# Rose-STL-Lab/dyffusion

Measured on AMD Instinct MI355X. Metric: sampled fields/sec (h-step rollout), higher is better.
Workload: dtype bf16; 1 GPU; BASELINE configs[1]: Navier-Stokes 221x42, C=3+2 static ch, unet_simple dim 64 @256^2, DYffusion h=16 cold sampling + refine, interpolator MC dropout p=0.15, hipGraph rollout; rows_per_gpu=80, total_rows=80, net_forwards_per_rollout=60, parallelism=ensemble-sharded dp1

## Files before the change

### dyffusion_amd/_lib.py

```python
import ctypes as C
import os

_HERE = os.path.dirname(os.path.abspath(__file__))
LIB_PATH = os.environ.get("DYF_LIB") or os.path.join(_HERE, "lib", "libdyffusion_hip.so")
LIB_PATH_F16 = os.environ.get("DYF_LIB_F16") or os.path.join(_HERE, "lib", "libdyffusion_hip_f16.so")
DTYPES = {"bf16": 0, "bfloat16": 0, "fp16": 1, "float16": 1, "half": 1}
FP32_NAMES = ("fp32", "float32", "32")
BF16X3_NAMES = ("bf16x3", "48")


def canonical_dtype(dtype) -> str:
    key = str(dtype).lower()
    if key in FP32_NAMES:
        return "fp32"
    if key in BF16X3_NAMES:
        return "bf16x3"
    if key not in DTYPES:
        raise ValueError(f"dtype {dtype!r}: expected one of {sorted(DTYPES) + list(FP32_NAMES) + list(BF16X3_NAMES)}")
    return "fp16" if DTYPES[key] else "bf16"


def storage_dtype(dtype) -> str:
    d = canonical_dtype(dtype)
    return "bf16" if d in ("fp32", "bf16x3") else d
# ... 16 lines not shown
DYF_TRAIN_PRECISION_BF16X3 = 48
DYF_SAMPLE_PRECISION_BF16X3 = 48
DYF_OK, DYF_ERR_INVALID_ARGUMENT, DYF_ERR_UNSUPPORTED, DYF_ERR_HIP, DYF_ERR_STATE = range(5)
NET_FORECASTER, NET_INTERPOLATOR = 0, 1
ARCH_UNET_SIMPLE, ARCH_UNET_RESNET = 0, 1
ARCH_SIMPLE_CONV_NET = 2
FCOND = {"none": 0, "data": 1, "data+noise": 2}


class NetConfig(C.Structure):
    _fields_ = [("arch", C.c_int32), ("in_channels", C.c_int32), ("cond_channels", C.c_int32),
                ("out_channels", C.c_int32), ("dim", C.c_int32), ("with_time_emb", C.c_int32),
                ("upsample_h", C.c_int32), ("upsample_w", C.c_int32), ("dropout", C.c_float),
                ("input_dropout", C.c_float), ("n_mults", C.c_int32), ("dim_mults", C.c_int32 * 6),
                ("block_dropout1", C.c_float), ("attn_dropout", C.c_float), ("groups", C.c_int32),
                ("init_kernel_size", C.c_int32), ("init_padding", C.c_int32), ("outer_nearest", C.c_int32),
                ("keep_spatial_dims", C.c_int32), ("single_conv_layer", C.c_int32), ("learned_sinusoidal_dim", C.c_int32)]


class EngineConfig(C.Structure):
    _fields_ = [("abi_version", C.c_int32), ("device", C.c_int32), ("height", C.c_int32), ("width", C.c_int32),
                ("max_batch", C.c_int32), ("use_graph", C.c_int32), ("enable_mfma", C.c_int32), ("dtype", C.c_int32),
                ("batch_invariant", C.c_int32), ("net", NetConfig * 2)]


class PlanStep(C.Structure):
    _fields_ = [("forecaster_time", C.c_float), ("tau", C.c_float), ("i_next", C.c_float), ("i_cur", C.c_float),
                ("is_last", C.c_int32), ("out_slot", C.c_int32)]


class Plan(C.Structure):
    _fields_ = [("n_steps", C.c_int32), ("steps", C.POINTER(PlanStep)), ("sampling_cold", C.c_int32),
                ("cold_for_last_step", C.c_int32), ("forward_conditioning", C.c_int32), ("n_refine", C.c_int32),
                ("refine_times", C.POINTER(C.c_float)), ("refine_slots", C.POINTER(C.c_int32)),
                ("n_out_slots", C.c_int32), ("interpolator_dropout", C.c_int32), ("forecaster_dropout", C.c_int32)]


class BcArgs(C.Structure):
    _fields_ = [("kind", C.c_int32), ("n_fields", C.c_int32), ("rows", C.c_int32), ("channels", C.c_int32),
                ("height", C.c_int32), ("width", C.c_int32), ("n_meta", C.c_int32), ("row_meta_dev", C.c_void_p),
                ("time_factor_dev", C.c_void_p), ("times_per_meta", C.c_int32), ("fixed_mask_dev", C.c_void_p),
                ("in_velocity_dev", C.c_void_p), ("vertex_y_dev", C.c_void_p), ("boundary_dev", C.c_void_p)]


class ConvEx(C.Structure):
    _fields_ = [("x1_dev", C.c_void_p), ("residual_dev", C.c_void_p), ("y_f32_dev", C.c_void_p), ("mask_dev", C.c_void_p),
                ("c1", C.c_int32), ("coef_div", C.c_int32), ("n_sel", C.c_int32), ("drop_mode", C.c_int32),
                ("drop_p", C.c_float), ("drop_site", C.c_int32), ("drop_row_offset", C.c_uint32), ("drop_forward", C.c_uint32)]


BC_NAVIER_STOKES, BC_SPRING_MESH = 0, 1
COMM_ID_BYTES = 128
TRAIN_BATCH_STATS, TRAIN_DROPOUT = 1, 2


class TrainOp(C.Structure):
    _fields_ = [(k, C.c_int32) for k in ("op", "nb", "h", "w", "c", "c2", "k", "stride", "pad", "groups", "flags")] + [("p", C.c_float)]


TRAIN_OPS = {"conv": 0, "gn_act": 1, "layernorm": 2, "linattn": 3, "attention": 4, "linear": 5, "learned_sinu": 6, "dropout": 7,
             "gelu": 8, "add": 9, "cat": 10, "up2_nearest": 11, "norm_act": 12, "up2_bilinear": 13, "resize": 14, "convt": 15,
             "attention_stream": 16}
TOP_WS, TOP_BIAS, TOP_PRE, TOP_FILM, TOP_SAME = 1, 2, 4, 8, 16
TOP_RUNNING, TOP_MASK, TOP_LEAKY, TOP_RELU, TOP_NEAREST, TOP_GRAD_IN = 32, 64, 128, 256, 512, 1024
TOP_ACT_GELU, TOP_RESIDUAL = 2048, 4096
TOP_SAMPLE = 8192


class SampleOp(C.Structure):
    _fields_ = [(k, C.c_int32) for k in ("op", "nb", "h", "w", "c", "c2", "k", "pad", "groups", "act", "flags", "film_stride", "film_div",
                                         "part_slots", "nsrc")] + [("ch", C.c_int32 * 4), ("drop_mode", C.c_int32), ("drop_p", C.c_float),
                                                                   ("drop_site", C.c_int32), ("drop_row_offset", C.c_uint32), ("drop_forward", C.c_uint32)] + \
               [(k, C.c_int32) for k in ("oh", "ow", "nearest", "src_rows", "iw_store")] + [("tau", C.c_float)]


class SampleTensors(C.Structure):
    _fields_ = [("x", C.c_void_p * 4), ("residual", C.c_void_p), ("film_a", C.c_void_p), ("film_c", C.c_void_p), ("part", C.c_void_p),
                ("mask", C.c_void_p), ("y", C.c_void_p), ("col_map", C.c_void_p), ("y2", C.c_void_p), ("y3", C.c_void_p)]


SAMPLE_OPS = {"gn_act": 0, "layernorm_c": 1, "head": 2, "up2_nearest": 3, "drop16": 4, "stem_conv": 5, "groupnorm_f32": 6, "up2_bilinear": 7,
              "up2_epilogue": 8, "readout": 9, "readout_tables": 10, "stem": 11, "stem16": 12, "rng_begin": 13, "rng_clone": 14, "time_mlp": 15,
              "film": 16, "cold_update": 17, "noisy_condition": 18}
SOP_NO_STATS, SOP_NO_TABLES, SOP_FOLD_RNG, SOP_COUNTERS_ONLY = 1, 2, 4, 8
RNG_STATE_WORDS = 8
ACTS = {"none": 0, "relu": 1, "leaky": 2, "silu": 3, "gelu": 4}


class OptimConfig(C.Structure):
    _fields_ = [("beta1", C.c_double), ("beta2", C.c_double), ("eps", C.c_double), ("weight_decay", C.c_double),
                ("max_grad_norm", C.c_double), ("ema", C.c_int32)]


OPTIM_WEIGHT, OPTIM_GRAD, OPTIM_EXP_AVG, OPTIM_EXP_AVG_SQ, OPTIM_EMA, OPTIM_WEIGHT_FWD = range(6)

_P = C.c_void_p
SYMBOLS = [
    ("dyf_engine_create", C.c_int, [C.POINTER(EngineConfig), C.POINTER(_P)]),
    ("dyf_engine_destroy", None, [_P]),
    ("dyf_last_error", C.c_char_p, [_P]),
    ("dyf_abi_version", C.c_int32, []),
    ("dyf_dtype", C.c_int32, []),
    ("dyf_load_weights", C.c_int, [_P, C.c_int32, C.c_int32, C.POINTER(C.c_char_p), C.POINTER(_P), C.POINTER(_P),
                                   C.POINTER(C.c_int32)]),
    ("dyf_train_load_weights", C.c_int, [_P, C.c_int32, C.c_int32, C.POINTER(C.c_char_p), C.POINTER(_P), C.POINTER(_P),
                                         C.POINTER(C.c_int32)]),
    ("dyf_train_load_weights_dev", C.c_int, [_P, C.c_int32, C.c_int32, C.POINTER(C.c_char_p), C.POINTER(_P), C.POINTER(_P),
                                             C.POINTER(C.c_int32)]),
    ("dyf_train_export_dev", C.c_int, [_P, C.c_int32, C.c_int32, C.POINTER(C.c_char_p), C.POINTER(_P)]),
    ("dyf_net_forward", C.c_int, [_P, C.c_int32, _P, _P, _P, _P, C.c_int32, C.c_int32, C.POINTER(_P), _P]),
    ("dyf_set_plan", C.c_int, [_P, C.POINTER(Plan)]),
    ("dyf_sample", C.c_int, [_P, _P, _P, _P, C.c_int32, C.POINTER(_P), _P, _P]),
    ("dyf_seed", C.c_int, [_P, C.c_uint64]),
    ("dyf_set_row_offset", C.c_int, [_P, C.c_uint32]),
    ("dyf_set_log_intermediates", C.c_int, [_P, C.c_int32]),
    ("dyf_get_log", C.c_int, [_P, C.c_int32, C.c_int32, _P, C.c_int32, _P]),
    ("dyf_set_row_groups", C.c_int, [_P, C.c_int32]),
    ("dyf_row_groups", C.c_int32, [_P]),
    ("dyf_comm_unique_id", C.c_int, [_P]),
    ("dyf_comm_init", C.c_int, [_P, _P, C.c_int32, C.c_int32]),
    ("dyf_comm_destroy", C.c_int, [_P]),
    ("dyf_comm_count", C.c_int, [_P, _P]),
    ("dyf_sample_gather", C.c_int, [_P, _P, _P, _P, C.c_int32, C.c_int32, _P]),
    ("dyf_get_sampler_state", C.c_int, [_P, C.c_int32, _P, C.c_int32, _P]),
    ("dyf_plan_forward_counts", C.c_int, [_P, C.POINTER(C.c_int32), C.POINTER(C.c_int32)]),
    ("dyf_net_flops", C.c_int, [_P, C.c_int32, C.POINTER(C.c_double)]),
    ("dyf_net_flops_executed", C.c_int, [_P, C.c_int32, C.POINTER(C.c_double)]),
    ("dyf_time_conv_layer", C.c_int, [_P, C.c_int32, C.c_int32, C.c_int32, C.c_int32, _P, C.POINTER(C.c_double),
                                      C.POINTER(C.c_double), C.POINTER(C.c_double)]),
    ("dyf_ensemble_metrics", C.c_int, [_P, _P, _P, C.c_int32, C.c_int64, C.POINTER(C.c_double), _P]),
    ("dyf_time_layer_in_rollout", C.c_int, [_P, C.c_int32, C.c_int32, _P, C.POINTER(C.c_double), C.POINTER(C.c_int32)]),
    ("dyf_time_kernel_in_rollout", C.c_int, [_P, C.c_int32, C.c_int32, _P, C.POINTER(C.c_double), C.POINTER(C.c_int32),
                                             C.POINTER(C.c_double), C.POINTER(C.c_double)]),
    ("dyf_op_conv2d", C.c_int, [_P, _P, _P] + [C.c_int32] * 9 + [_P, _P, C.c_int32, C.c_int32, _P, _P]),
    ("dyf_op_conv2d_ex", C.c_int, [_P, _P, _P] + [C.c_int32] * 9 + [_P, _P, C.c_int32, C.c_int32, _P, C.POINTER(ConvEx), _P]),
    ("dyf_op_upconv2d", C.c_int, [_P, _P, _P] + [C.c_int32] * 5 + [_P, _P, C.c_int32, _P, _P]),
    ("dyf_op_linear_attention", C.c_int, [_P, _P, C.c_int32, C.c_int32, _P, _P]),
    ("dyf_op_linear_attention_fused", C.c_int, [_P, _P, _P, C.c_int32, C.c_int32, C.c_int32, _P, _P, _P, _P, _P]),
    ("dyf_op_attention", C.c_int, [_P, _P, C.c_int32, C.c_int32, _P, _P]),
    ("dyf_op_attention_dropout", C.c_int, [_P, _P, C.c_int32, C.c_int32, C.c_float, _P, _P]),
    ("dyf_op_attention_f32", C.c_int, [_P, _P, C.c_int32, C.c_int32, C.c_float, _P, C.c_int32, _P, _P]),
    ("dyf_op_train_f32", C.c_int, [_P, C.POINTER(TrainOp), C.POINTER(_P), C.POINTER(_P), _P, _P, C.POINTER(_P), C.POINTER(_P), _P]),
    ("dyf_op_sample16", C.c_int, [_P, C.POINTER(SampleOp), C.POINTER(SampleTensors), C.POINTER(_P), _P]),
    ("dyf_criterion", C.c_int, [_P, _P, _P, C.c_int64, C.c_int32, _P, _P]),
    ("dyf_train_forward", C.c_int, [_P, C.c_int32, C.c_int32, _P, _P, _P, _P, C.c_int32, C.c_int32, _P]),
    ("dyf_train_backward", C.c_int, [_P, C.c_int32, _P, _P, C.c_int32, _P]),
    ("dyf_train_zero_grads", C.c_int, [_P, C.c_int32]),
    ("dyf_train_set_precision", C.c_int, [_P, C.c_int32]),
    ("dyf_train_precision", C.c_int32, [_P]),
    ("dyf_train_set_deterministic", C.c_int, [_P, C.c_int32]),
    ("dyf_train_deterministic", C.c_int32, [_P]),
    ("dyf_set_sample_precision", C.c_int, [_P, C.c_int32]),
    ("dyf_sample_precision", C.c_int32, [_P]),
    ("dyf_set_attention_dropout", C.c_int, [_P, C.c_int32]),
    ("dyf_attention_dropout", C.c_int32, [_P]),
    ("dyf_train_export", C.c_int, [_P, C.c_int32, C.c_int32, C.POINTER(C.c_char_p), C.POINTER(_P)]),
    ("dyf_optim_create", C.c_int, [_P, C.c_int32, C.POINTER(OptimConfig)]),
    ("dyf_optim_destroy", C.c_int, [_P, C.c_int32]),
    ("dyf_optim_step", C.c_int, [_P, C.c_int32, C.c_double, C.c_double, _P]),
    ("dyf_optim_last", C.c_int, [_P, C.c_int32, C.POINTER(C.c_double), C.POINTER(C.c_int32)]),
    ("dyf_optim_get_step", C.c_int, [_P, C.c_int32, C.POINTER(C.c_int64)]),
    ("dyf_optim_set_step", C.c_int, [_P, C.c_int32, C.c_int64]),
    ("dyf_optim_export", C.c_int, [_P, C.c_int32, C.c_int32, C.c_int32, C.POINTER(C.c_char_p), C.POINTER(_P), C.c_int32]),
    ("dyf_optim_import", C.c_int, [_P, C.c_int32, C.c_int32, C.c_int32, C.POINTER(C.c_char_p), C.POINTER(_P), C.c_int32]),
    ("dyf_optim_swap_ema", C.c_int, [_P, C.c_int32, _P]),
    ("dyf_criterion_grad", C.c_int, [_P, _P, _P, C.c_int64, C.c_int32, C.c_float, _P, _P]),
    ("dyf_train_conv_check", C.c_int, [_P] + [C.c_int32] * 9 + [C.c_uint32, C.POINTER(C.c_float)]),
# ... 61 lines not shown
```

### dyffusion_amd/csrc/conv.h

```cpp
#pragma once
#include "common.h"
#include "gn_fused.h"

#include <string>
#include <vector>

void dyf_form_log_enable(bool on);
std::string dyf_form_log_text();
void dyf_form_set(const char* key, const char* value);
std::string dyf_form_text();
void dyf_prof_arm(const char* name);
void dyf_prof_collect(double* total_ms, double* total_bytes, int* launches);

struct ConvArgs {
    const el16_t* src0;
    const el16_t* src1;
    int c0, c1;
    int pix_pitch0;
    int n, h, w;
    int ho, wo;
    int kh, kw, stride, pad;
    int cout;
    const el16_t* wpk;
    const el16_t* wpk_frag;
    int up2x;
    const el16_t* wpk_up;
    const el16_t* wpk_up_frag;
    const int16_t* up_cols;
    const int16_t* up_cbase;
    const int16_t* up_cidx;
    int up_ntiles, up_npad, up_nvalid0, up_nvalid1;
    int up_mix[3];
    int up_sh_off, up_sh_cb;
    int up_wo_store;
    const float* coef_a;
    const float* coef_c;
    int coef_stride;
    int coef_div;
    int act;
    DropSpec drop;
    int up_nearest;
    const el16_t* residual;
    el16_t* out_el16;
    float* out_f32;
    const el16_t* zero_page;
    float* up_border;
    float* splitk_ws;
    long long splitk_cap;
    int splitk;
    int n_sel;
    float* gn_part;
    int gn_slots;
    GnFuse gnf;
};
inline size_t conv_up_border_floats(int n, int h, int w, int cout) { return (size_t)n * (4 * (size_t)w + 4 * (size_t)h - 4) * cout; }

enum class HaloOrder { None, Halo3_256 , Halo3_64 , S2 ,
                       Enc0Stem  };
struct ConvW {
    const el16_t* wpk = nullptr;
    const el16_t* frag = nullptr;
    const el16_t* halo = nullptr;
    HaloOrder halo_order = HaloOrder::None;
    const el16_t* frag64 = nullptr;
};

hipError_t conv_init();
bool conv_mfma_supported(const ConvArgs& a);
enum class ConvForm { Invalid , None , Direct, Igemm128, Igemm256x64, UpHalo,
                      Halo3, Rows3, Halo5, HaloS2, Enc0Stem, Igemm2, Skinny, Gn16 };
enum class ConvWant { Plain, Stats , GnFused };
struct ConvChoice {
    ConvForm form;
    const el16_t* frag;
    int gn_slots;
    int bm;
};
ConvChoice conv_choose_form(const ConvArgs& a, const ConvW& w, int path, ConvWant want);
hipError_t launch_conv(const ConvArgs& a, const ConvW& w, int path, hipStream_t stream);
hipError_t launch_conv_stats(const ConvArgs& a, const ConvW& w, int path, hipStream_t stream, int* gn_slots);
hipError_t launch_conv_gn_fused(const ConvArgs& a, const ConvW& w, int path, hipStream_t stream, bool* fused);
int conv_gn_fused_max_slots(int h, int w);
bool conv_plain3x3_takes_halo5(const ConvArgs& a, const ConvW& w);

hipError_t launch_conv_direct(const ConvArgs& a, hipStream_t stream);
hipError_t launch_conv_igemm(const ConvArgs& a, hipStream_t stream);
void pack_up2x_weights(const float* w, int cout, int cin, el16_t* out);
hipError_t launch_conv_splitk_finish4(const ConvArgs& a, long long M, hipStream_t stream);
bool conv_up_halo_supported(const ConvArgs& a);
hipError_t conv_up_halo_init();
hipError_t launch_conv_up_halo(const ConvArgs& a, hipStream_t stream);
void pack_up2x_frag(const el16_t* wpk_up, int cout, int cin, el16_t* out);
bool plan_up_sparse_columns(const std::vector<uint8_t>& needed, int w, std::vector<int16_t>& cols, std::vector<int16_t>& cbase,
                            std::vector<int16_t>& cidx, std::vector<int16_t>& col_map, int& ntiles, int& nvalid0, int& nvalid1,
                            int slots = 16);
int conv_halo_rows_slots();
int conv_halo_rows_sparse_halo_w();
int conv_halo_rows_sparse_halo_w_shape(int shape);
bool plan_up_sparse_columns_mixed(const std::vector<uint8_t>& needed, int w, int h, std::vector<int16_t>& cols, std::vector<int16_t>& cbase,
                                  std::vector<int16_t>& cidx, std::vector<int16_t>& col_map, int mix[3], int& nvalid0, int& nvalid1);
bool conv_halo_rows_up_supported(const ConvArgs& a);
bool conv_halo_rows3_supported(const ConvArgs& a);
hipError_t conv_halo_rows_init();
hipError_t launch_conv_halo_rows_up(const ConvArgs& a, hipStream_t stream);
hipError_t launch_conv_halo_rows3(const ConvArgs& a, hipStream_t stream);
bool conv_halo3_supported(const ConvArgs& a);
hipError_t launch_conv_halo3(const ConvArgs& a, hipStream_t stream);
void pack_halo3_frag(const el16_t* wpk, int cout, int cin, el16_t* out);
bool conv_halo_s2_supported(const ConvArgs& a);
hipError_t launch_conv_halo_s2(const ConvArgs& a, hipStream_t stream);
void pack_halo_s2_frag(const el16_t* wpk, int cout, int cin, el16_t* out);
bool conv_halo5_supported(const ConvArgs& a);
int conv_halo5_gn_slots(int h, int w);
hipError_t launch_conv_halo5(const ConvArgs& a, hipStream_t stream);
void pack_halo3_frag64(const el16_t* wpk, int cout, int cin, el16_t* out);
bool conv_gn16_supported(const ConvArgs& a);
int conv_gn16_slots(int h, int w);
hipError_t launch_conv_gn16(const ConvArgs& a, hipStream_t stream);
bool conv_enc0_stem_supported(const ConvArgs& a);
hipError_t conv_enc0_stem_init();
hipError_t launch_conv_enc0_stem(const ConvArgs& a, const el16_t* wfrag, hipStream_t stream);
void pack_enc0_stem_frag(const el16_t* wpk, int cout, el16_t* out);
bool conv_igemm2_supported(const ConvArgs& a);
hipError_t conv_igemm2_init();
hipError_t launch_conv_igemm2(const ConvArgs& a, hipStream_t stream);
void pack_conv_frag(const el16_t* wpk, int cout, int taps, int cin, el16_t* out);
bool conv_igemm2_tile2d(int ho, int wo);
int conv_igemm2_gn_slots(int ho, int wo);
int conv_igemm2_gn_slots_bm128(int ho, int wo);
bool conv_skinny_supported(const ConvArgs& a);
hipError_t launch_conv_skinny(const ConvArgs& a, hipStream_t stream);
```

### dyffusion_amd/csrc/conv_dispatch.hip

```cpp
#include "conv.h"

#include <algorithm>
#include <initializer_list>

namespace {

long long form_rows(const ConvArgs& a) { return a.n_sel > 0 ? a.n_sel : a.n; }
ConvArgs with_up_frag(ConvArgs a, const el16_t* f) { a.wpk_up_frag = f; return a; }
ConvArgs with_frag(ConvArgs a, const ConvW& w) { a.wpk_frag = w.frag; return a; }
const el16_t* halo_of(const ConvW& w, HaloOrder order) { return w.halo_order == order ? w.halo : nullptr; }
bool halo3_on() { return dyf_form_int("DYF_HALO3", 1) != 0; }
bool igemm2_on() { return dyf_form_int("DYF_IGEMM2", 1) != 0; }

bool up_halo_admits(const ConvArgs& a) {
    const int halo_min = dyf_form_int("DYF_HALO_MIN_PLANE", 32);
    return a.up2x && dyf_form_int("DYF_UP_HALO", 1) != 0 && a.h >= halo_min && a.w >= halo_min && conv_up_halo_supported(a);
}

const el16_t* halo3_admits(const ConvArgs& a, const ConvW& w) {
    if (!(!a.up2x && a.kh == 3 && a.kw == 3 && a.cout % 256 == 0 && a.out_f32 == nullptr && a.residual == nullptr) || !halo3_on()) return nullptr;
    const ConvArgs b = with_up_frag(a, halo_of(w, HaloOrder::Halo3_256));
    const long long tiles3 = (form_rows(a) * a.h * a.w / 128) * (a.cout / 256);
    return b.wpk_up_frag && tiles3 >= dyf_form_int("DYF_HALO3_MIN_TILES", 80) && conv_halo3_supported(b) ? b.wpk_up_frag : nullptr;
}

const el16_t* halo5_admits(const ConvArgs& a, const ConvW& w) {
    if (!(!a.up2x && a.kh == 3 && a.kw == 3 && a.stride == 1 && a.cout % 64 == 0 && a.cout % 256 != 0 && a.out_f32 == nullptr)) return nullptr;
    if (dyf_form_int("DYF_HALO5", 1) == 0) return nullptr;
    const ConvArgs b = with_up_frag(a, halo_of(w, HaloOrder::Halo3_64));
    const long long ty = (a.h + 15) / 16, tx = (a.w + 31) / 32;
    const long long tiles5 = form_rows(a) * ty * tx * (a.cout / 64);
    const bool covers = 10ll * a.h * a.w >= 6ll * ty * 16 * tx * 32;
    return b.wpk_up_frag && covers && tiles5 >= dyf_form_int("DYF_HALO5_MIN_TILES", 64) && conv_halo5_supported(b) ? b.wpk_up_frag : nullptr;
}

const el16_t* enc0_stem_admits(const ConvArgs& a, const ConvW& w) {
    return a.pix_pitch0 == 16 && conv_enc0_stem_supported(a) ? halo_of(w, HaloOrder::Enc0Stem) : nullptr;
}

const el16_t* halo_s2_admits(const ConvArgs& a, const ConvW& w) {
    if (!(!a.up2x && a.kh == 4 && a.kw == 4 && a.stride == 2 && a.cout % 128 == 0 && a.c1 == 0 && a.out_f32 == nullptr &&
          a.residual == nullptr && a.pix_pitch0 == 0) || !halo3_on())
        return nullptr;
    const ConvArgs b = with_up_frag(a, halo_of(w, HaloOrder::S2));
    const long long min_tiles3 = dyf_form_int("DYF_HALO_S2_MIN_TILES", dyf_form_int("DYF_HALO3_MIN_TILES", 80));
    const long long pix = form_rows(a) * a.ho * a.wo;
    const long long tiles3 = a.cout % 256 == 0 ? (pix / 128) * (a.cout / 256) : (pix / 256) * (a.cout / 128);
    return b.wpk_up_frag && tiles3 >= min_tiles3 && conv_halo_s2_supported(b) ? b.wpk_up_frag : nullptr;
}

long long igemm2_tiles(const ConvArgs& a) {
    return ((form_rows(a) * a.ho * a.wo + 255) / 256) * (a.cout % 128 == 0 ? a.cout / 128 : a.cout / 64);
}

const el16_t* igemm2_admits(const ConvArgs& a, const ConvW& w) {
    if (!(!a.up2x && igemm2_on() && a.cout % 64 == 0)) return nullptr;
    const ConvArgs b = with_frag(a, w);
    return igemm2_tiles(a) >= dyf_form_int("DYF_IGEMM2_MIN_TILES", 384) && conv_igemm2_supported(b) ? b.wpk_frag : nullptr;
}

const el16_t* skinny_admits(const ConvArgs& a, const ConvW& w) {
    if (!(!a.up2x && a.cout % 128 == 0) || dyf_form_int("DYF_SKINNY", 1) == 0) return nullptr;
    const long long tiles128 = ((form_rows(a) * a.ho * a.wo + 127) / 128) * (a.cout / 128);
    const ConvArgs b = with_frag(a, w);
    return tiles128 <= dyf_form_int("DYF_SKINNY_MAX_TILES", 64) && conv_skinny_supported(b) ? b.wpk_frag : nullptr;
}

const int GN_FUSE_MAX_SLOTS = 64;
bool gn_slots_fit(int slots, int max_slots) { return slots <= GN_FUSE_MAX_SLOTS && slots <= max_slots; }

const el16_t* gn16_admits(const ConvArgs& a, const ConvW& w, bool c256) {
    if (dyf_form_int("DYF_GN16", 1) == 0 || (c256 && dyf_form_int("DYF_GN16_C256", 1) == 0)) return nullptr;
    const ConvArgs b = with_up_frag(a, c256 ? w.frag64 : halo_of(w, HaloOrder::Halo3_64));
    const int slots16 = conv_gn16_slots(a.h, a.w);
    const long long tiles16 = form_rows(a) * slots16 * (a.cout / 64);
    const bool covers16 = 10ll * a.h * a.w >= 6ll * slots16 * 256 || dyf_form_int("DYF_GN16_ANY_PLANE", 0) != 0;
    const bool plane_ok = !c256 || (long long)a.h * a.w <= dyf_form_int("DYF_GN16_C256_MAX_PLANE", 1024);
    return b.wpk_up_frag && covers16 && plane_ok && tiles16 >= dyf_form_int("DYF_GN16_MIN_TILES", 64) &&
                   gn_slots_fit(slots16, a.gnf.max_slots) && conv_gn16_supported(b) ? b.wpk_up_frag : nullptr;
}

const el16_t* igemm2_fused_admits(const ConvArgs& a, const ConvW& w, ConvChoice* c) {
    const GnFuse& G = a.gnf;
    if (!(igemm2_on() && a.cout % 128 == 0)) return nullptr;
    const ConvArgs b = with_frag(a, w);
    if (!conv_igemm2_supported(b)) return nullptr;
    const long long tiles2 = igemm2_tiles(a);
    const long long min_tiles = dyf_form_int("DYF_IGEMM2_MIN_TILES", dyf_form_int("DYF_GN_FUSE_MIN_TILES", 32));
    const bool position_free = conv_igemm2_tile2d(a.ho, a.wo) || (a.ho * a.wo) % 128 == 0;
    if (G.invariant && !position_free) return nullptr;
    const long long bm128_below = dyf_form_int("DYF_IGEMM2_BM128_BELOW", 224);
    const int slots128 = conv_igemm2_gn_slots_bm128(a.ho, a.wo), slots = conv_igemm2_gn_slots(a.ho, a.wo);
    const bool free128 = (a.wo % 16 == 0 && a.ho % 8 == 0) || (a.ho * a.wo) % 64 == 0;
    if (tiles2 >= min_tiles && tiles2 < bm128_below && slots128 > 0 && gn_slots_fit(slots128, G.max_slots) && (!G.invariant || free128))
        c->gn_slots = slots128, c->bm = 128;
    else if (tiles2 >= min_tiles && slots > 0 && gn_slots_fit(slots, G.max_slots))
        c->gn_slots = slots, c->bm = 256;
    else
        return nullptr;
    return b.wpk_frag;
}

ConvChoice choose_plain(const ConvArgs& a, const ConvW& w, bool mfma, bool stats) {
    const ConvChoice invalid{ConvForm::Invalid, nullptr, 0, 0};
    const el16_t* const h5 = mfma && a.residual == nullptr ? halo5_admits(a, w) : nullptr;
    if (a.up_nearest && !(h5 && a.h % 2 == 0 && a.w % 2 == 0 && a.c1 == 0)) return invalid;
    if (!mfma) return a.up2x ? invalid : ConvChoice{ConvForm::Direct, nullptr, 0, 0};
    if (a.up2x && a.up_cols) return conv_up_halo_supported(a) ? ConvChoice{ConvForm::UpHalo, nullptr, 0, 0} : invalid;
    if (up_halo_admits(a)) return {ConvForm::UpHalo, nullptr, 0, 0};
    if (const el16_t* f = halo3_admits(a, w))
        return {dyf_form_int("DYF_HALO_ROWS", 1) != 0 && conv_halo_rows3_supported(a) ? ConvForm::Rows3 : ConvForm::Halo3, f, 0, 0};
    if (h5)
        return {ConvForm::Halo5, h5, stats && a.act == ACT_NONE && a.drop.mode == 0 ? conv_halo5_gn_slots(a.h, a.w) : 0, 0};
    if (const el16_t* f = enc0_stem_admits(a, w)) return {ConvForm::Enc0Stem, f, 0, 0};
    if (const el16_t* f = halo_s2_admits(a, w)) return {ConvForm::HaloS2, f, 0, 0};
    if (const el16_t* f = igemm2_admits(a, w)) return {ConvForm::Igemm2, f, 0, 0};
    if (const el16_t* f = skinny_admits(a, w)) return {ConvForm::Skinny, f, 0, 0};
    return {a.cout % 128 == 0 ? ConvForm::Igemm128 : ConvForm::Igemm256x64, nullptr, 0, 0};
}

ConvChoice choose_gn_fused(const ConvArgs& a, const ConvW& w, bool mfma) {
    ConvChoice c{ConvForm::None, nullptr, 0, 0};
    const GnFuse& G = a.gnf;
    if (!mfma || G.gran == nullptr || G.epoch == nullptr || a.act != ACT_SILU || a.drop.mode == 2 || a.out_el16 == nullptr ||
        a.out_f32 != nullptr || a.up2x)
        return c;
    const int cpg = G.groups > 0 ? a.cout / G.groups : 0;
    if (cpg < 8 || cpg % 8 != 0 || 64 % cpg != 0 || cpg * G.groups != a.cout) return c;
    const bool conv3 = a.kh == 3 && a.kw == 3 && a.stride == 1 && a.pad == 1;
    if (conv3 && a.cout % 64 == 0) {
        if (const el16_t* f = gn16_admits(a, w, a.cout % 256 == 0)) return {ConvForm::Gn16, f, conv_gn16_slots(a.h, a.w), 0};
        const int slots = conv_halo5_gn_slots(a.h, a.w);
        if (const el16_t* f = gn_slots_fit(slots, G.max_slots) ? halo5_admits(a, w) : nullptr) return {ConvForm::Halo5, f, slots, 0};
    }
    if ((c.frag = igemm2_fused_admits(a, w, &c))) c.form = ConvForm::Igemm2;
    return c;
}

hipError_t launch_chosen(ConvArgs& a, const ConvChoice& c, hipStream_t stream) {
    switch (c.form) {
    case ConvForm::Invalid: return hipErrorInvalidValue;
    case ConvForm::None: return hipSuccess;
    case ConvForm::Direct: return launch_conv_direct(a, stream);
    case ConvForm::Igemm128:
    case ConvForm::Igemm256x64: return launch_conv_igemm(a, stream);
    case ConvForm::UpHalo: return launch_conv_up_halo(a, stream);
    case ConvForm::Halo3: a.wpk_up_frag = c.frag; return launch_conv_halo3(a, stream);
    case ConvForm::Rows3: a.wpk_up_frag = c.frag; return launch_conv_halo_rows3(a, stream);
    case ConvForm::Halo5: a.wpk_up_frag = c.frag; return launch_conv_halo5(a, stream);
    case ConvForm::HaloS2: a.wpk_up_frag = c.frag; return launch_conv_halo_s2(a, stream);
    case ConvForm::Gn16: a.wpk_up_frag = c.frag; return launch_conv_gn16(a, stream);
    case ConvForm::Enc0Stem: return launch_conv_enc0_stem(a, c.frag, stream);
    case ConvForm::Igemm2: a.wpk_frag = c.frag; return launch_conv_igemm2(a, stream);
    case ConvForm::Skinny: a.wpk_frag = c.frag; return launch_conv_skinny(a, stream);
    }
    return hipErrorInvalidValue;
}

}

ConvChoice conv_choose_form(const ConvArgs& a, const ConvW& w, int path, ConvWant want) {
    const bool mfma = path == 1 && conv_mfma_supported(a);
    return want == ConvWant::GnFused ? choose_gn_fused(a, w, mfma) : choose_plain(a, w, mfma, want == ConvWant::Stats);
}

bool conv_plain3x3_takes_halo5(const ConvArgs& a, const ConvW& w) {
    return a.gn_part == nullptr && a.gnf.gran == nullptr && conv_choose_form(a, w, 1, ConvWant::Plain).form == ConvForm::Halo5;
}

int conv_gn_fused_max_slots(int h, int w) {
    int best = 0;
    for (int s : {conv_halo5_gn_slots(h, w), conv_gn16_slots(h, w), conv_igemm2_gn_slots(h, w), conv_igemm2_gn_slots_bm128(h, w)})
        if (gn_slots_fit(s, GN_FUSE_MAX_SLOTS)) best = std::max(best, s);
    return best;
}

hipError_t launch_conv(const ConvArgs& a, const ConvW& w, int path, hipStream_t stream) {
    return launch_conv_stats(a, w, path, stream, nullptr);
}

hipError_t launch_conv_stats(const ConvArgs& a_in, const ConvW& w, int path, hipStream_t stream, int* gn_slots) {
    if (gn_slots) *gn_slots = 0;
    ConvArgs a = a_in;
    a.wpk = w.wpk;
    a.gn_part = nullptr;
    a.gn_slots = 0;
    const bool stats = gn_slots != nullptr && a_in.gn_part != nullptr;
    const ConvChoice c = conv_choose_form(a, w, path, stats ? ConvWant::Stats : ConvWant::Plain);
    if (c.gn_slots > 0) {
        a.gn_part = a_in.gn_part;
        a.gn_slots = c.gn_slots;
        *gn_slots = c.gn_slots;
    }
    return launch_chosen(a, c, stream);
}

hipError_t launch_conv_gn_fused(const ConvArgs& a_in, const ConvW& w, int path, hipStream_t stream, bool* fused) {
    ConvArgs a = a_in;
    a.wpk = w.wpk;
    a.gn_part = nullptr;
    a.gn_slots = 0;
    const ConvChoice c = conv_choose_form(a, w, path, ConvWant::GnFused);
    *fused = c.form != ConvForm::None;
    a.gnf.slots = c.gn_slots;
    if (c.bm) a.gnf.bm = c.bm;
    return launch_chosen(a, c, stream);
}
```

### dyffusion_amd/csrc/conv_enc0_stem.hip

```cpp
#include "conv.h"

#include <type_traits>
typedef __attribute__((ext_vector_type(16))) float f32x16;

namespace {
constexpr int E0_KSTEPS = 16;
constexpr int E0_WAVES = 8, E0_THREADS = E0_WAVES * 64;
constexpr int e0_lds_bytes(int nt) { return E0_KSTEPS * nt * 1024 + E0_WAVES * 2 * nt * 32 * 4 + E0_WAVES * 32 * (nt * 64 + 16); }
}

template <int NT>
__global__ __launch_bounds__(512) void conv_enc0_stem_kernel(ConvArgs a, const el16_t* __restrict__ wfrag, int tiles, int tiles_per_wg) {
#if defined(__gfx950__)
    extern __shared__ __attribute__((aligned(16))) unsigned char e0_smem[];
    uint4* wl = (uint4*)e0_smem;
    const int tid = threadIdx.x, lane = tid & 63, wave = __builtin_amdgcn_readfirstlane(tid >> 6), l31 = lane & 31, hi = lane >> 5;
    for (int i = tid; i < E0_KSTEPS * NT * 64; i += E0_THREADS) wl[i] = ((const uint4*)wfrag)[i];
    __syncthreads();
    float* coefl = (float*)(e0_smem + E0_KSTEPS * NT * 1024) + wave * (2 * NT * 32);
    int coef_row = -1;
    constexpr int OROW = NT * 64 + 16;
    unsigned char* ostage = e0_smem + E0_KSTEPS * NT * 1024 + E0_WAVES * 2 * NT * 32 * 4 + wave * (32 * OROW);
    const int segs = a.wo >> 5;
    const int plane = a.ho * a.wo;
    const int t0 = blockIdx.x * tiles_per_wg, t1 = min(t0 + tiles_per_wg, tiles);
    const int cout = NT * 32;

    auto load = [&](int t, uint4 (&xf)[E0_KSTEPS]) {
        const int row = t / segs, seg = t - row * segs;
        const int n = row / a.ho, oy = row - n * a.ho;
        const el16_t* p = a.src0 + ((size_t)(n * a.h + 2 * oy) * a.w + 2 * (seg * 32 + l31)) * 16 + 8 * hi;
#pragma unroll
        for (int kh = 0; kh < 4; ++kh)
#pragma unroll
            for (int kw = 0; kw < 4; ++kw) xf[kh * 4 + kw] = *(const uint4*)(p + ((size_t)kh * a.w + kw) * 16);
        __builtin_amdgcn_sched_barrier(0);
    };

    auto tile = [&](int t, const uint4 (&xf)[E0_KSTEPS], auto act_c, auto mode_c) {
        constexpr int ACT = decltype(act_c)::value, MODE = decltype(mode_c)::value;
        f32x16 acc[NT];
#pragma unroll
        for (int nt = 0; nt < NT; ++nt)
#pragma unroll
            for (int r = 0; r < 16; ++r) acc[nt][r] = 0.0f;
#pragma unroll
        for (int s = 0; s < E0_KSTEPS; ++s) {
            int wlane = lane;
            asm volatile("" : "+v"(wlane));
            const el16x8_t xb = __builtin_bit_cast(el16x8_t, xf[s]);
#pragma unroll
            for (int nt = 0; nt < NT; ++nt)
                acc[nt] = DYF_MFMA_32x32x16(__builtin_bit_cast(el16x8_t, wl[(s * NT + nt) * 64 + wlane]), xb, acc[nt], 0, 0, 0);
        }
        const int m = t * 32 + l31;
        const int n_img = m / plane;
        const uint32_t ob = (uint32_t)m * (uint32_t)cout;
        const RngKey key = drop_row_key(a.drop, n_img);
        const uint32_t row0 = (uint32_t)n_img * (uint32_t)(plane * cout);
        const int crow = __builtin_amdgcn_readfirstlane(a.coef_div > 1 ? n_img / a.coef_div : n_img);
        if (crow != coef_row) {
            coef_row = crow;
            const float ps = drop_prescale<ACT, MODE>(a.drop);
            if (lane < NT * 8) {
                float4 ca = *(const float4*)(a.coef_a + (size_t)crow * a.coef_stride + lane * 4);
                float4 cc = *(const float4*)(a.coef_c + (size_t)crow * a.coef_stride + lane * 4);
                ca.x *= ps; ca.y *= ps; ca.z *= ps; ca.w *= ps;
                cc.x *= ps; cc.y *= ps; cc.z *= ps; cc.w *= ps;
                *(float4*)(coefl + lane * 4) = ca;
                *(float4*)(coefl + NT * 32 + lane * 4) = cc;
            }
        }
#pragma unroll
        for (int nt = 0; nt < NT; ++nt) {
            uint4 o2[2];
#pragma unroll
            for (int g2 = 0; g2 < 2; ++g2) {
                const int cg0 = nt * 32 + 16 * g2;
                const float4 ca0 = *(const float4*)(coefl + cg0 + 4 * hi), ca1 = *(const float4*)(coefl + cg0 + 4 * hi + 8);
                const float4 cc0 = *(const float4*)(coefl + NT * 32 + cg0 + 4 * hi), cc1 = *(const float4*)(coefl + NT * 32 + cg0 + 4 * hi + 8);
                const float ca[8] = {ca0.x, ca0.y, ca0.z, ca0.w, ca1.x, ca1.y, ca1.z, ca1.w};
                const float cc[8] = {cc0.x, cc0.y, cc0.z, cc0.w, cc1.x, cc1.y, cc1.z, cc1.w};
                const uint32_t e0 = ob + cg0 + 4 * hi;
                float v[8];
#pragma unroll
                for (int i = 0; i < 8; ++i) v[i] = fmaf(acc[nt][8 * g2 + i], ca[i], cc[i]);
                act_drop_fixed<4, ACT, MODE, true>(v, e0, row0, a.drop, key);
                act_drop_fixed<4, ACT, MODE, true>(v + 4, e0 + 8, row0, a.drop, key);
                const uint32_t p0 = pack_el16x2(v[0], v[1]), p1 = pack_el16x2(v[2], v[3]);
                const uint32_t q0 = pack_el16x2(v[4], v[5]), q1 = pack_el16x2(v[6], v[7]);
                const auto s0 = __builtin_amdgcn_permlane32_swap(p0, q0, false, false);
                const auto s1 = __builtin_amdgcn_permlane32_swap(p1, q1, false, false);
                o2[g2].x = s0[0]; o2[g2].y = s1[0]; o2[g2].z = s0[1]; o2[g2].w = s1[1];
            }
            *(uint4*)(ostage + l31 * OROW + (nt * 32 + 8 * hi) * 2) = o2[0];
            *(uint4*)(ostage + l31 * OROW + (nt * 32 + 16 + 8 * hi) * 2) = o2[1];
        }
        el16_t* tbase = a.out_el16 + (size_t)t * 32 * cout;
#pragma unroll
        for (int k = 0; k < NT * 2; ++k) {
            const int off = k * 1024 + lane * 16;
            const int px = off / (NT * 64), within = off - px * (NT * 64);
            const uint4 ov = *(const uint4*)(ostage + px * OROW + within);
            *(uint4*)((unsigned char*)tbase + off) = ov;
        }
    };

    auto run = [&](auto act_c, auto mode_c) {
        uint4 xa[E0_KSTEPS], xb[E0_KSTEPS];
        int t = t0 + wave;
        if (t >= t1) return;
        load(t, xa);
        for (; t < t1; t += 2 * E0_WAVES) {
            load(t + E0_WAVES, xb);
            tile(t, xa, act_c, mode_c);
            load(t + 2 * E0_WAVES < t1 ? t + 2 * E0_WAVES : t, xa);
            tile(t + E0_WAVES, xb, act_c, mode_c);
        }
    };
    auto by_mode = [&](auto act_c) {
        if (a.drop.mode == 0) run(act_c, std::integral_constant<int, 0>{});
        else if (a.drop.mode == 1) run(act_c, std::integral_constant<int, 1>{});
        else run(act_c, std::integral_constant<int, 2>{});
    };
    if (a.act == ACT_RELU) by_mode(std::integral_constant<int, ACT_RELU>{});
    else if (a.act == ACT_LEAKY) by_mode(std::integral_constant<int, ACT_LEAKY>{});
    else if (a.act == ACT_SILU) by_mode(std::integral_constant<int, ACT_SILU>{});
    else by_mode(std::integral_constant<int, ACT_NONE>{});
#endif
}

void pack_enc0_stem_frag(const el16_t* wpk, int cout, el16_t* out) {
    const int nt_n = cout / 32;
    for (int s = 0; s < E0_KSTEPS; ++s)
        for (int nt = 0; nt < nt_n; ++nt)
            for (int lane = 0; lane < 64; ++lane)
                for (int j = 0; j < 8; ++j)
                    out[(((size_t)s * nt_n + nt) * 64 + lane) * 8 + j] = wpk[(size_t)(32 * nt + (lane & 31)) * 256 + 16 * s + 8 * (lane >> 5) + j];
}

bool conv_enc0_stem_supported(const ConvArgs& a) {
    const bool on = dyf_form_int("DYF_ENC0_STEM", 1) != 0;
    if (!on || a.pix_pitch0 != 16 || a.c0 != 64 || a.c1 != 0 || a.kh != 4 || a.kw != 1 || a.stride != 2 || a.pad != 0) return false;
    if (a.up2x || a.residual || a.out_f32 || !a.out_el16 || (a.cout != 64 && a.cout != 128)) return false;
    if (a.wo % 32 != 0 || (a.ho * (a.wo / 32)) % 16 != 0 || a.h != 2 * a.ho + 2 || a.w != 2 * a.wo + 2) return false;
    const long long nsel = a.n_sel > 0 ? a.n_sel : a.n;
    if (nsel * a.ho * (a.wo / 32) < 4096) return false;
    return (size_t)a.n * a.ho * a.wo * a.cout < 0xFFFFFFF0ull;
}

hipError_t conv_enc0_stem_init() {
    hipError_t e = hipFuncSetAttribute((const void*)conv_enc0_stem_kernel<4>, hipFuncAttributeMaxDynamicSharedMemorySize, e0_lds_bytes(4));
    if (e == hipSuccess) e = hipFuncSetAttribute((const void*)conv_enc0_stem_kernel<2>, hipFuncAttributeMaxDynamicSharedMemorySize, e0_lds_bytes(2));
    return e;
}

hipError_t launch_conv_enc0_stem(const ConvArgs& a, const el16_t* wfrag, hipStream_t stream) {
    const int tiles = a.n * a.ho * (a.wo / 32);
    int nwg = std::min(256, (tiles + 15) / 16);
    int per = (tiles + nwg - 1) / nwg;
    per = (per + 15) / 16 * 16;
    nwg = (tiles + per - 1) / per;
    dyf_form_note("conv_enc0_stem_kernel", a.n);
    if (a.cout == 128)
        hipLaunchKernelGGL(conv_enc0_stem_kernel<4>, dim3(nwg), dim3(E0_THREADS), e0_lds_bytes(4), stream, a, wfrag, tiles, per);
    else
        hipLaunchKernelGGL(conv_enc0_stem_kernel<2>, dim3(nwg), dim3(E0_THREADS), e0_lds_bytes(2), stream, a, wfrag, tiles, per);
    return hipGetLastError();
}
```

### dyffusion_amd/csrc/engine.hip

```cpp
#include "engine_internal.h"

#include <dlfcn.h>
#include <mutex>
#include <rccl/rccl.h>
#include "unet_kernels.h"
#include "../../include/dyffusion_hip_testing.h"

using namespace dyf;

namespace {

thread_local bool g_creating_group_child = false;

int default_row_groups(const dyf_engine* e) {
    if (e->cfg.net[0].arch != DYF_ARCH_UNET_RESNET || e->cfg.net[1].arch != DYF_ARCH_UNET_RESNET) return 1;
    if (e->cfg.batch_invariant) return 1;
    const long long plane = (long long)e->cfg.height * e->cfg.width;
    if (plane > 128 * 128) return 1;
    const long long pix = plane * e->cfg.max_batch;
    if (pix >= 72ll * 60 * 60) return 3;
    return 1;
}

void layout_blocks(Net& n) {
// ... 5 lines not shown
    int off = 0;
    for (int i = 0; i < 12; ++i) {
        const int* s = i < 6 ? enc[i] : dec[i - 6];
        UBlock& b = n.blk[i];
        b.cin = s[0]; b.cout = s[1]; b.k = s[2]; b.stride = s[3]; b.pad = s[4];
        b.gn = (i == 5);
        b.transposed = i >= 6;
        b.act = i < 6 ? ACT_LEAKY : ACT_RELU;
        b.film_off = off;
        off += b.cout;
    }
    n.total_c = off;
}

std::string layout_geometry(Net& n, int H, int W) {
    n.uh = n.cfg.upsample_h > 0 ? n.cfg.upsample_h : H;
    n.uw = n.cfg.upsample_w > 0 ? n.cfg.upsample_w : W;
    int h = n.uh, w = n.uw;
    for (int i = 0; i < 6; ++i) {
        UBlock& b = n.blk[i];
        b.in_h = h; b.in_w = w;
        b.out_h = (h + 2 * b.pad - b.k) / b.stride + 1;
        b.out_w = (w + 2 * b.pad - b.k) / b.stride + 1;
        if (b.out_h < 1 || b.out_w < 1) return "resampled grid too small for six stride-2 encoder blocks";
        h = b.out_h; w = b.out_w;
    }
    for (int i = 6; i < 12; ++i) {
        UBlock& b = n.blk[i];
        b.in_h = 2 * h; b.in_w = 2 * w;
        b.out_h = b.in_h + 2 * b.pad - b.k + 1;
        b.out_w = b.in_w + 2 * b.pad - b.k + 1;
        h = b.out_h; w = b.out_w;
        if (i < 11) {
            const UBlock& skip = n.blk[10 - i];
            if (skip.out_h != h || skip.out_w != w)
                return "decoder/skip spatial sizes do not match (resampled grid must be divisible by 64)";
        }
    }
    double f = 2.0 * n.uh * n.uw * (double)n.cin_total * n.dim;
    for (int i = 0; i < 12; ++i) {
        const UBlock& b = n.blk[i];
        f += 2.0 * b.out_h * b.out_w * (double)b.cout * b.cin * b.k * b.k;
    }
    f += 2.0 * h * w * (double)n.dim * n.cfg.out_channels * 16;
    if (n.cfg.with_time_emb) {
        f += 2.0 * ((double)n.dim * n.tdim + (double)n.tdim * n.tdim);
        f += 2.0 * (double)n.tdim * 2 * n.total_c;
    }
    n.flops_per_sample = f;
    return "";
}

DropSpec make_drop(const dyf_engine* e, const Net& n, const FwdOpts& o, int layer) {
    DropSpec d{};
    const float p = n.cfg.dropout;
    d.mode = (p > 0.0f) ? o.dropout_mode : 0;
    d.scale = 1.0f / (1.0f - p);
    d.thresh16 = keep_threshold16(p);
    d.salt = rng_layer_salt((uint32_t)layer);
    d.row_keys = e->row_keys;
    d.mask = (d.mode == 2 && o.masks) ? o.masks[layer + (n.cfg.input_dropout > 0.0f ? 1 : 0)] : nullptr;
    if (d.mode == 2 && d.mask == nullptr) d.mode = 0;
    return d;
}

DropSpec make_input_drop(const dyf_engine* e, const Net& n, const FwdOpts& o) {
    DropSpec d{};
    const float p = n.cfg.input_dropout;
    d.mode = (p > 0.0f) ? o.dropout_mode : 0;
    d.scale = 1.0f / (1.0f - p);
    d.thresh16 = keep_threshold16(p);
    d.salt = rng_layer_salt(DYF_INPUT_DROP_SITE);
    d.row_keys = e->row_keys;
    d.mask = (d.mode == 2 && o.masks) ? o.masks[0] : nullptr;
    if (d.mode == 2 && d.mask == nullptr) d.mode = 0;
    return d;
}

dyf_status run_conv(dyf_engine* e, const ConvArgs& a, const ConvW& w, hipStream_t st) {
    HIP_TRY(e, launch_conv(a, w, conv_path(e, a), st));
    return DYF_OK;
}

const ConvW* fused_enc0_args(const dyf_engine* e, const Net& n, ConvArgs& a) {
    a.src0 = e->ws.stem16; a.c0 = 64; a.pix_pitch0 = 16;
    a.h = n.uh + 2; a.w = n.uw + 2;
    a.kh = 4; a.kw = 1; a.stride = 2; a.pad = 0;
    return &n.enc0_fused_w;
}

bool use_fused_up(const dyf_engine* e, const UBlock& b, const ConvArgs& f) {
    return e->cfg.enable_mfma && e->fuse_up2x && b.wpk_up != nullptr && f.h >= e->fuse_min_plane && f.w >= e->fuse_min_plane &&
           conv_mfma_supported(f);
}

ConvArgs block_conv_args(const dyf_engine* e, const Net& n, const UBlock& b, int nb) {
    ConvArgs a{};
    a.n = nb; a.h = b.in_h; a.w = b.in_w; a.ho = b.out_h; a.wo = b.out_w;
    a.kh = b.k; a.kw = b.k; a.stride = b.stride; a.pad = b.pad; a.cout = b.cout;
    a.act = b.act;
    a.zero_page = e->ws.zero_page;
    a.splitk_ws = e->ws.splitk; a.splitk_cap = DYF_SPLITK_FLOATS;
    a.n_sel = e->cfg.batch_invariant ? 2 * e->cfg.max_batch : 0;
    return a;
}

dyf_status net_forward(dyf_engine* e, int which, const Source* srcs, int nsrc, int nb, const FwdOpts& o, float* out_dev,
                       hipStream_t st) {
    Net& n = e->net[which];
    if (n.rn) return rn_forward(e, which, srcs, nsrc, nb, o, out_dev, st);
    if (n.sc) return sc_forward(e, which, srcs, nsrc, nb, o, out_dev, st);
    Workspace& ws = e->ws;
    const int H = e->cfg.height, W = e->cfg.width;
    const bool draws = o.dropout_mode == 1 && (n.cfg.dropout > 0.0f || n.cfg.input_dropout > 0.0f);
    const bool fold_rng = dyf_form_int("DYF_FOLD_RNG_BEGIN", 1) != 0;
    const bool rng_in_stem = draws && fold_rng && n.stem_fused && e->cfg.enable_mfma && e->fuse_stem && n.cfg.input_dropout == 0.0f;
    if (draws && !rng_in_stem)
        HIP_TRY(e, launch_rng_begin_forward(e->rng_state, e->row_keys, nb, o.src_rows > 0 ? o.src_rows : nb, st));
    StemArgs sa{};
    int ctot = 0;
    for (int i = 0; i < nsrc; ++i) {
        sa.src[i] = srcs[i].p;
        sa.ch[i] = srcs[i].ch;
        ctot += srcs[i].ch;
    }
    if (ctot != n.cin_total)
        return fail(e, DYF_ERR_INVALID_ARGUMENT, "channel count of the network inputs does not match its configuration");
    sa.nsrc = nsrc; sa.cin = ctot; sa.n = nb; sa.src_rows = o.src_rows; sa.h = H; sa.w = W; sa.uh = n.uh; sa.uw = n.uw;
    sa.resample = (n.uh != H || n.uw != W) ? 1 : 0;
    sa.nearest = n.cfg.outer_nearest;
    sa.wgt = n.stem_w; sa.bias = n.stem_b; sa.dim = n.dim;
    const bool fused_stem = n.stem_fused && e->cfg.enable_mfma && e->fuse_stem && n.cfg.input_dropout == 0.0f;
    sa.drop = make_input_drop(e, n, o);
    if (rng_in_stem) {
        sa.rng_state = e->rng_state; sa.rng_row_keys = e->row_keys; sa.rng_rows = nb; sa.rng_rows_per_fwd = o.src_rows > 0 ? o.src_rows : nb;
    }
    if (fused_stem) {
        sa.out = ws.stem16;
        HIP_TRY(e, launch_stem16(sa, st));
    } else {
        sa.out = ws.stem;
        HIP_TRY(e, launch_stem(sa, st));
    }
    const el16_t* x = ws.stem;
    for (int i = 0; i < 6; ++i) {
        const UBlock& b = n.blk[i];
        ConvArgs a = block_conv_args(e, n, b, nb);
        a.src0 = x; a.c0 = b.cin; a.src1 = nullptr; a.c1 = 0;
        const ConvW* w = &b.wpk;
        if (i == 0 && fused_stem) w = fused_enc0_args(e, n, a);
        if (!b.gn) {
            a.coef_a = o.coef_a + b.film_off; a.coef_c = o.coef_c + b.film_off; a.coef_stride = o.coef_stride;
            a.coef_div = o.coef_div;
            a.drop = make_drop(e, n, o, i);
            a.out_el16 = ws.enc[i];
            dyf_status s = run_conv(e, a, *w, st);
            if (s != DYF_OK) return s;
        } else {
            a.coef_a = b.static_a; a.coef_c = b.static_c; a.coef_stride = 0;
            a.act = ACT_NONE;
            a.drop = DropSpec{};
            a.out_f32 = ws.enc5_raw;
            dyf_status s = run_conv(e, a, *w, st);
            if (s != DYF_OK) return s;
            GroupNormArgs g{};
            g.x = ws.enc5_raw; g.n = nb; g.hw = b.out_h * b.out_w; g.c = b.cout; g.groups = 8;
            g.gamma = b.gamma; g.beta = b.beta;
            g.film_a = o.coef_a + b.film_off; g.film_c = o.coef_c + b.film_off; g.film_stride = o.coef_stride;
            g.film_div = o.coef_div;
            g.act = b.act; g.drop = make_drop(e, n, o, i); g.out = ws.enc[i];
            HIP_TRY(e, launch_groupnorm(g, st));
        }
        x = ws.enc[i];
    }
    const el16_t* skip = nullptr;
    int skip_c = 0;
    const UBlock* sparse_out = nullptr;
    int lh = n.blk[5].out_h, lw = n.blk[5].out_w;
    for (int i = 6; i < 12; ++i) {
        const UBlock& b = n.blk[i];
        ConvArgs a = block_conv_args(e, n, b, nb);
        a.coef_a = o.coef_a + b.film_off; a.coef_c = o.coef_c + b.film_off; a.coef_stride = o.coef_stride;
        a.coef_div = o.coef_div;
        a.drop = make_drop(e, n, o, i);
        a.out_el16 = ws.dec[i - 6];
        ConvArgs f = a;
        f.src0 = x; f.c0 = b.cin - skip_c; f.src1 = skip; f.c1 = skip_c; f.h = lh; f.w = lw;
        f.up2x = 1; f.wpk_up = b.wpk_up; f.wpk_up_frag = b.wpk_up_frag; f.up_border = ws.up_border;
        f.up_cols = b.up_cols; f.up_cbase = b.up_cbase; f.up_cidx = b.up_cidx; f.up_ntiles = b.up_ntiles; f.up_npad = b.up_npad;
        f.up_nvalid0 = b.up_nvalid0; f.up_nvalid1 = b.up_nvalid1; f.up_wo_store = b.up_wo_store;
        f.up_mix[0] = b.up_mix[0]; f.up_mix[1] = b.up_mix[1]; f.up_mix[2] = b.up_mix[2];
        if (i == 11 && b.up_cols && e->poison_dec5)
            HIP_TRY(e, hipMemsetAsync(ws.dec[5], 0xFF, (size_t)nb * b.out_h * b.out_w * b.cout * sizeof(el16_t), st));
        if (f.up_cols && !(use_fused_up(e, b, f) && conv_up_halo_supported(f))) f.up_cols = nullptr;
        if (f.up_cols) sparse_out = &b;
        const bool prof = e->prof_layer == i && e->prof_ev.size() < 4096;
        hipEvent_t pe0 = nullptr, pe1 = nullptr;
        if (prof) {
            HIP_TRY(e, hipEventCreate(&pe0));
            HIP_TRY(e, hipEventCreate(&pe1));
        }
        const bool commute = dyf_form_int("DYF_DEC_COMMUTE", 1) != 0;
        const bool commuted = commute && b.k == 1 && b.stride == 1 && b.pad == 0 && e->cfg.enable_mfma && (b.cout & 3) == 0 &&
                              (size_t)nb * lh * lw * b.cout * sizeof(float) <= (size_t)nb * b.in_h * b.in_w * b.cin * sizeof(el16_t);
        if (use_fused_up(e, b, f)) {
            if (prof) HIP_TRY(e, hipEventRecord(pe0, st));
            HIP_TRY(e, launch_conv(f, b.wpk, 1, st));
            if (prof) HIP_TRY(e, hipEventRecord(pe1, st));
        } else if (commuted) {
            ConvArgs lo = a;
            lo.src0 = x; lo.c0 = b.cin - skip_c; lo.src1 = skip; lo.c1 = skip_c;
            lo.h = lh; lo.w = lw; lo.ho = lh; lo.wo = lw;
            lo.coef_a = ws.ones_f; lo.coef_c = ws.zeros_f; lo.coef_stride = 0; lo.coef_div = 0;
            lo.act = ACT_NONE; lo.drop = DropSpec{};
            lo.out_el16 = nullptr; lo.out_f32 = (float*)ws.up;
            if (prof) HIP_TRY(e, hipEventRecord(pe0, st));
            dyf_status s = run_conv(e, lo, b.wpk, st);
            if (s != DYF_OK) return s;
            Up2xEpiArgs u{};
            u.lo = (const float*)ws.up; u.n = nb; u.h = lh; u.w = lw; u.c = b.cout;
            u.coef_a = a.coef_a; u.coef_c = a.coef_c; u.coef_stride = a.coef_stride; u.coef_div = a.coef_div;
            u.act = a.act; u.drop = a.drop; u.out = a.out_el16;
            HIP_TRY(e, launch_up2x_epilogue(u, st));
            if (prof) HIP_TRY(e, hipEventRecord(pe1, st));
        } else {
            Up2xArgs u{};
            u.src0 = x; u.c0 = b.cin - skip_c; u.src1 = skip; u.c1 = skip_c; u.n = nb; u.h = lh; u.w = lw; u.out = ws.up;
            HIP_TRY(e, launch_up2x(u, st));
            a.src0 = ws.up; a.c0 = b.cin; a.src1 = nullptr; a.c1 = 0;
            if (prof) HIP_TRY(e, hipEventRecord(pe0, st));
            dyf_status s = run_conv(e, a, b.wpk, st);
            if (s != DYF_OK) return s;
            if (prof) HIP_TRY(e, hipEventRecord(pe1, st));
// ... 332 lines not shown
    if (n.sc) {
        dyf_status ss = sc_load_weights(e, n, sd);
        if (ss != DYF_OK || e->is_group_child) return ss;
        return train_store_params(e, which, sd);
    }
    if (n.rn) {
        dyf_status rs = rn_load_weights(e, n, sd);
        if (rs != DYF_OK) return rs;
        n.loaded = true;
        n.table_of_time.clear();
        n.ntables = 0;
        e->plan.set = false;
        if (e->is_group_child) return DYF_OK;
        return train_store_params(e, which, sd);
    }
    std::string missing;
    auto get = [&](const std::string& key, std::vector<int64_t> want) -> const TensorView* {
        auto it = sd.find(key);
        if (it == sd.end()) {
            if (missing.empty()) missing = "missing tensor '" + key + "' in state_dict";
            return nullptr;
        }
        if (it->second.shape != want) {
            if (missing.empty()) missing = "tensor '" + key + "' has an unexpected shape";
            return nullptr;
        }
        return &it->second;
    };
    auto vec = [](const TensorView* t) { return std::vector<float>(t->data, t->data + t->numel()); };
    const int64_t d = n.dim, td = n.tdim;
#define NEED(var, key, ...)                                              \
    const TensorView* var = get(key, std::vector<int64_t>{__VA_ARGS__}); \
    if (!var) return fail(e, DYF_ERR_INVALID_ARGUMENT, missing)
#define UP(dst, hostvec)                                  \
    do {                                                  \
        dyf_status _s = dev_upload(e, &(dst), (hostvec)); \
        if (_s != DYF_OK) return _s;                      \
    } while (0)

    if (n.cfg.with_time_emb) {
        NEED(w1, "time_emb_mlp.1.weight", td, d);
        NEED(b1, "time_emb_mlp.1.bias", td);
        NEED(w2, "time_emb_mlp.3.weight", td, td);
        NEED(b2, "time_emb_mlp.3.bias", td);
        UP(n.t_w1, vec(w1)); UP(n.t_b1, vec(b1)); UP(n.t_w2, vec(w2)); UP(n.t_b2, vec(b2));
    }
    {
        NEED(sw, "init_conv.weight", d, (int64_t)n.cin_total, 1, 1);
        NEED(sb, "init_conv.bias", d);
        UP(n.stem_w, vec(sw)); UP(n.stem_b, vec(sb));
    }
    std::vector<float> film_w((size_t)2 * n.total_c * n.tdim, 0.0f), film_b((size_t)2 * n.total_c, 0.0f);
    std::vector<float> norm_a(n.total_c, 1.0f), norm_c(n.total_c, 0.0f);
    std::vector<int> blk_of(n.total_c), blk_off(12), blk_cout(12);
    for (int i = 0; i < 12; ++i) {
        UBlock& b = n.blk[i];
        const std::string pre = (i < 6 ? "input_ops." + std::to_string(i) : "output_ops." + std::to_string(i - 6));
        const std::string conv = pre + ".ops." + (b.transposed ? "1" : "0");
        const std::string norm = pre + ".ops." + (b.transposed ? "2" : "1");
        NEED(cw, conv + ".weight", (int64_t)b.cout, (int64_t)b.cin, (int64_t)b.k, (int64_t)b.k);
        NEED(cb, conv + ".bias", (int64_t)b.cout);
        NEED(nw, norm + ".weight", (int64_t)b.cout);
        NEED(nbias, norm + ".bias", (int64_t)b.cout);
        blk_off[i] = b.film_off;
        blk_cout[i] = b.cout;
        for (int c = 0; c < b.cout; ++c) blk_of[b.film_off + c] = i;
        const int taps = b.k * b.k;
        { dyf_status _s = upload_conv_weights(e, &b.wpk, pack_conv(cw->data, b.cout, b.cin, taps), b.cout, taps, b.cin); if (_s != DYF_OK) return _s; }
        if (i == 0 && b.k == 4 && n.cin_total + 1 <= 16 && b.cout % 64 == 0 && n.uh % 2 == 0 && n.uw % 2 == 0) {
            const TensorView* sw = &sd["init_conv.weight"];
            const TensorView* sb = &sd["init_conv.bias"];
            std::vector<el16_t> fw((size_t)b.cout * 16 * 16);
            for (int co = 0; co < b.cout; ++co)
                for (int t = 0; t < 16; ++t)
                    for (int c = 0; c < 16; ++c) {
                        double v = 0.0;
                        if (c <= n.cin_total)
                            for (int d2 = 0; d2 < n.dim; ++d2) {
                                const double we = cw->data[((size_t)co * b.cin + d2) * 16 + t];
                                v += we * (c < n.cin_total ? (double)sw->data[(size_t)d2 * n.cin_total + c] : (double)sb->data[d2]);
                            }
                        fw[((size_t)co * 16 + t) * 16 + c] = f32_to_el16((float)v);
                    }
            { dyf_status _s = upload_conv_weights(e, &n.enc0_fused_w, fw, b.cout, 4, 64, true); if (_s != DYF_OK) return _s; }
            n.stem_fused = true;
        }
        if (b.transposed && b.k == 3) {
            std::vector<el16_t> pu((size_t)4 * b.cout * 16 * b.cin);
            pack_up2x_weights(cw->data, b.cout, b.cin, pu.data());
            UP(b.wpk_up, pu);
            if (b.cin % 64 == 0 && b.cout % 64 == 0) {
                std::vector<el16_t> pf(pu.size());
                pack_up2x_frag(pu.data(), b.cout, b.cin, pf.data());
                UP(b.wpk_up_frag, pf);
            }
            const bool sparse_ok = dyf_form_int("DYF_SPARSE_DEC5", 1) != 0;
            if (i == 11 && b.wpk_up_frag && sparse_ok) {
                const int iw = b.out_w, tw = 2 * iw, ow = e->cfg.width;
                std::vector<uint8_t> needed(iw, 0);
                for (int ox = 0; ox < ow; ++ox) {
                    double src = ((double)ox + 0.5) * ((double)tw / (double)ow) - 0.5;
                    if (src < 0.0) src = 0.0;
                    if (n.cfg.outer_nearest) src = (double)ox * ((double)tw / (double)ow);
                    for (double eps : {-1e-3, 1e-3}) {
                        int v0 = (int)std::floor(std::max(0.0, src + eps));
                        v0 = std::min(v0, tw - 1);
                        for (int v : {v0, std::min(v0 + 1, tw - 1)}) {
                            const int jh = (v + 1) >> 1;
                            for (int j : {jh, jh - 1})
                                if (j >= 0 && j < iw) needed[j] = 1;
                        }
                    }
                }
                std::vector<int16_t> cols, cbase, cidx, cmap;
                int nt = 0, nv0 = 0, nv1 = 0;
                const bool rows_env = dyf_form_int("DYF_HALO_ROWS", 1) != 0;
                int slots = rows_env && (b.out_h / 2) % 4 == 0 ? conv_halo_rows_slots() : 16;
                bool planned = false;
                int mix[3] = {0, 0, 0};
                const bool mixed_env = dyf_form_int("DYF_SPARSE_MIXED", 1) != 0;
                if (n.dim == 64 && n.cfg.out_channels <= 4 && mixed_env && slots == conv_halo_rows_slots() &&
                    plan_up_sparse_columns_mixed(needed, iw / 2, b.out_h / 2, cols, cbase, cidx, cmap, mix, nv0, nv1)) {
                    planned = true;
                    nt = mix[0] + mix[1] + mix[2];
                }
                if (!planned && n.dim == 64 && n.cfg.out_channels <= 4) {
                    mix[0] = mix[1] = mix[2] = 0;
                    planned = plan_up_sparse_columns(needed, iw / 2, cols, cbase, cidx, cmap, nt, nv0, nv1, slots);
                    if (!planned && slots != 16) {
                        slots = 16;
                        planned = plan_up_sparse_columns(needed, iw / 2, cols, cbase, cidx, cmap, nt, nv0, nv1, slots);
                    }
                }
                if (planned) {
                    UP(b.up_cols, cols);
                    UP(b.up_cbase, cbase);
                    UP(b.up_cidx, cidx);
                    UP(b.up_col_map, cmap);
                    b.up_ntiles = nt; b.up_npad = nt * slots; b.up_nvalid0 = nv0; b.up_nvalid1 = nv1;
                    b.up_mix[0] = mix[0]; b.up_mix[1] = mix[1]; b.up_mix[2] = mix[2];
                    if (mix[0] | mix[1] | mix[2]) b.up_npad = 32 * mix[0] + 16 * mix[1] + 4 * mix[2];
                    b.up_wo_store = nv0 + nv1;
                }
            }
        }
        if (!b.gn) {
            NEED(rm, norm + ".running_mean", (int64_t)b.cout);
            NEED(rv, norm + ".running_var", (int64_t)b.cout);
            for (int c = 0; c < b.cout; ++c) {
                const double a = (double)nw->data[c] / std::sqrt((double)rv->data[c] + 1e-5);
                norm_a[b.film_off + c] = (float)a;
                norm_c[b.film_off + c] = (float)((double)nbias->data[c] + ((double)cb->data[c] - (double)rm->data[c]) * a);
            }
        } else {
            UP(b.gamma, vec(nw)); UP(b.beta, vec(nbias));
            UP(b.static_a, std::vector<float>(b.cout, 1.0f));
            UP(b.static_c, vec(cb));
        }
        if (n.cfg.with_time_emb) {
            NEED(fw, pre + ".time_mlp.1.weight", (int64_t)2 * b.cout, td);
            NEED(fb, pre + ".time_mlp.1.bias", (int64_t)2 * b.cout);
            std::copy(fw->data, fw->data + fw->numel(), film_w.begin() + (size_t)2 * b.film_off * n.tdim);
            std::copy(fb->data, fb->data + fb->numel(), film_b.begin() + (size_t)2 * b.film_off);
        }
    }
    UP(n.film_w, film_w); UP(n.film_b, film_b); UP(n.norm_a, norm_a); UP(n.norm_c, norm_c);
    UP(n.blk_of, blk_of); UP(n.blk_off, blk_off); UP(n.blk_cout, blk_cout);
// ... 724 lines not shown
    if (!e || !out_full_dev) return fail(e, DYF_ERR_INVALID_ARGUMENT, "null argument");
    if (!e->comm) return fail(e, DYF_ERR_STATE, "dyf_comm_init has not been called");
    const int world = e->comm_world;
    if (total_rows < 1 || (long long)nb * world < total_rows || nb != (total_rows + world - 1) / world)
        return fail(e, DYF_ERR_INVALID_ARGUMENT, "every rank samples nb = ceil(total_rows / world) rows");
    e->poll_stream = (hipStream_t)stream;
    dyf_status r = sample_into_stack(e, initial_dev, static_dev, nb, nullptr, nullptr, stream);
    if (r != DYF_OK) return r;
    hipStream_t st = (hipStream_t)stream;
    const size_t row = (size_t)e->C * e->cfg.height * e->cfg.width, slots = (size_t)e->plan.hdr.n_out_slots;
    const size_t send = slots * nb * row;
    if (e->gather_recv_floats < send * world) {
        if (e->gather_recv) { HIP_TRY(e, hipDeviceSynchronize()); (void)hipFree(e->gather_recv); e->gather_recv = nullptr; }
        HIP_TRY(e, hipMalloc((void**)&e->gather_recv, send * world * sizeof(float)));
        e->gather_recv_floats = send * world;
    }
    RcclApi& api = rccl_api();
    ncclResult_t nr = api.AllGather(e->s_stack, e->gather_recv, send, ncclFloat, (ncclComm_t)e->comm, st);
    if (nr != ncclSuccess) return fail(e, DYF_ERR_HIP, std::string("ncclAllGather: ") + api.GetErrorString(nr));
    HIP_TRY(e, launch_gather_unpack(e->gather_recv, out_full_dev, world, (int)slots, nb, total_rows, (long long)row, st));
    return DYF_OK;
}

dyf_status dyf_get_sampler_state(dyf_engine* e, int32_t what, float* out_dev, int32_t nb, void* stream) {
    if (!e || !out_dev) return DYF_ERR_INVALID_ARGUMENT;
    if (!e->plan.set || !e->s_x0hat) return fail(e, DYF_ERR_STATE, "no sampling call has been made yet");
    if (nb < 1 || nb > e->cfg.max_batch) return fail(e, DYF_ERR_INVALID_ARGUMENT, "batch size outside [1, max_batch]");
    if (e->last_groups > 0) {
        if (nb != e->last_nb) return fail(e, DYF_ERR_INVALID_ARGUMENT, "batch size differs from the sampling call's");
        const size_t row = (size_t)e->C * e->cfg.height * e->cfg.width;
        for (int g = 0; g < e->last_groups; ++g) {
            dyf_engine* c = e->groups[g];
            dyf_status r = dyf_get_sampler_state(c, what, out_dev + (size_t)g * e->last_per * row,
                                                 std::min(e->last_per, nb - g * e->last_per), stream);
            if (r != DYF_OK) return fail(e, r, "row group: " + c->err);
        }
        return DYF_OK;
    }
    const float* src = nullptr;
    if (what == DYF_STATE_X0_HAT) src = e->s_x0hat;
    else if (what == DYF_STATE_X_S) src = e->s_xs;
    else if (what == DYF_STATE_X_NEXT) src = e->plan.steps.back().i_next >= 0.0f ? e->s_next : e->s_x0hat;
    else return fail(e, DYF_ERR_INVALID_ARGUMENT, "what must be a dyf_sampler_state");
    HIP_TRY(e, hipMemcpyAsync(out_dev, src, (size_t)nb * e->C * e->cfg.height * e->cfg.width * sizeof(float),
                              hipMemcpyDeviceToDevice, (hipStream_t)stream));
    return DYF_OK;
}

dyf_status dyf_set_log_intermediates(dyf_engine* e, int32_t enable) {
    if (!e) return DYF_ERR_INVALID_ARGUMENT;
    e->log_on = enable != 0;
    return DYF_OK;
}

dyf_status dyf_get_log(dyf_engine* e, int32_t step, int32_t what, float* out_dev, int32_t nb, void* stream) {
    if (!e || !out_dev) return DYF_ERR_INVALID_ARGUMENT;
    if (!e->s_log || e->log_has_cur.size() != e->plan.steps.size())
        return fail(e, DYF_ERR_STATE, "no sampling call has been logged (dyf_set_log_intermediates, then dyf_sample)");
    if (step < 0 || step >= (int)e->plan.steps.size() || what < 0 || what > 2 || nb != e->log_nb)
        return fail(e, DYF_ERR_INVALID_ARGUMENT, "step / what / batch size outside the logged call");
    if (what == 2 && !e->log_has_cur[step])
        return fail(e, DYF_ERR_STATE, "x_interpolated_s is not defined at this step (naive sampling, or a first step that is the last)");
    const size_t field = (size_t)nb * e->C * e->cfg.height * e->cfg.width;
    HIP_TRY(e, hipMemcpyAsync(out_dev, e->s_log + ((size_t)step * 3 + what) * field, field * sizeof(float), hipMemcpyDeviceToDevice,
                              (hipStream_t)stream));
    return DYF_OK;
}

dyf_status dyf_time_conv_layer(dyf_engine* e, int32_t which, int32_t layer, int32_t nb, int32_t iters, void* stream,
                               double* avg_ms, double* flops, double* algo_bytes) {
    if (!e || which < 0 || which > 1 || layer < 0 || layer > 11 || iters < 1 || !avg_ms)
        return fail(e, DYF_ERR_INVALID_ARGUMENT, "bad argument to dyf_time_conv_layer");
    Net& n = e->net[which];
    if (!n.loaded) return fail(e, DYF_ERR_STATE, "weights not loaded");
    if (n.rn || n.sc) return fail(e, DYF_ERR_UNSUPPORTED, "dyf_time_conv_layer addresses the 12 UNetBlocks of arch unet_simple");
    if (nb < 1 || nb > e->cfg.max_batch) return fail(e, DYF_ERR_INVALID_ARGUMENT, "batch size outside [1, max_batch]");
    HIP_TRY(e, hipSetDevice(e->cfg.device));
    hipStream_t st = (hipStream_t)stream;
    const UBlock& b = n.blk[layer];
    ConvArgs a = block_conv_args(e, n, b, nb);
    a.src0 = b.transposed ? e->ws.up : (layer == 0 ? e->ws.stem : e->ws.enc[layer - 1]);
    a.c0 = b.cin;
    const ConvW* w = &b.wpk;
    if (layer == 0 && n.stem_fused && e->cfg.enable_mfma && e->fuse_stem && n.cfg.input_dropout == 0.0f) w = fused_enc0_args(e, n, a);
    if (b.transposed && layer > 6) {
        ConvArgs f = a;
        const UBlock& skipb = n.blk[11 - layer];
        f.src0 = e->ws.dec[layer - 7]; f.c0 = b.cin - skipb.cout; f.src1 = e->ws.enc[11 - layer]; f.c1 = skipb.cout;
        f.h = b.in_h / 2; f.w = b.in_w / 2; f.up2x = 1; f.wpk_up = b.wpk_up; f.wpk_up_frag = b.wpk_up_frag; f.up_border = e->ws.up_border;
        f.up_cols = b.up_cols; f.up_cbase = b.up_cbase; f.up_cidx = b.up_cidx; f.up_ntiles = b.up_ntiles; f.up_npad = b.up_npad;
        f.up_nvalid0 = b.up_nvalid0; f.up_nvalid1 = b.up_nvalid1; f.up_wo_store = b.up_wo_store;
        f.up_mix[0] = b.up_mix[0]; f.up_mix[1] = b.up_mix[1]; f.up_mix[2] = b.up_mix[2];
        if (use_fused_up(e, b, f)) a = f;
    }
    const float* A = n.tables ? n.tables : e->ws.coef_a;
    const float* Cc = n.tables ? n.tables + n.total_c : e->ws.coef_c;
    a.coef_a = b.gn ? b.static_a : A + b.film_off;
    a.coef_c = b.gn ? b.static_c : Cc + b.film_off;
    a.coef_stride = 0;
    a.drop = DropSpec{};
    if (b.gn) { a.out_f32 = e->ws.enc5_raw; a.act = ACT_NONE; } else { a.out_el16 = b.transposed ? e->ws.dec[layer - 6] : e->ws.enc[layer]; }
    hipEvent_t ev0, ev1;
    HIP_TRY(e, hipEventCreate(&ev0));
    HIP_TRY(e, hipEventCreate(&ev1));
    for (int i = 0; i < 2; ++i) {
        dyf_status s = run_conv(e, a, *w, st);
        if (s != DYF_OK) return s;
    }
    HIP_TRY(e, hipEventRecord(ev0, st));
    for (int i = 0; i < iters; ++i) {
        dyf_status s = run_conv(e, a, *w, st);
        if (s != DYF_OK) return s;
    }
    HIP_TRY(e, hipEventRecord(ev1, st));
    HIP_TRY(e, hipEventSynchronize(ev1));
    float ms = 0.0f;
    HIP_TRY(e, hipEventElapsedTime(&ms, ev0, ev1));
    (void)hipEventDestroy(ev0);
    (void)hipEventDestroy(ev1);
    *avg_ms = (double)ms / iters;
    const bool sparse = a.up2x && a.up_cols != nullptr;
    const double M = (double)nb * b.out_h * (sparse ? (double)(a.up_nvalid0 + a.up_nvalid1) : (double)b.out_w);
    if (flops) *flops = 2.0 * M * b.cout * b.cin * b.k * b.k;
    if (algo_bytes) {
        const double in_px = a.up2x ? (double)a.h * a.w : (double)b.in_h * b.in_w;
        *algo_bytes = 2.0 * ((double)nb * in_px * b.cin + M * b.cout + (double)b.cout * b.cin * b.k * b.k);
    }
    return DYF_OK;
}

dyf_status dyf_ensemble_metrics(dyf_engine* e, const float* preds_dev, const float* targets_dev, int32_t n_members,
                                int64_t n_points, double* out_host, void* stream) {
    if (!e || !preds_dev || !targets_dev || !out_host) return fail(e, DYF_ERR_INVALID_ARGUMENT, "null argument");
    if (n_members < 1 || n_members > 15360) return fail(e, DYF_ERR_INVALID_ARGUMENT, "n_members outside [1, 15360]");
    if (n_points < 1) return fail(e, DYF_ERR_INVALID_ARGUMENT, "n_points must be positive");
    HIP_TRY(e, hipSetDevice(e->cfg.device));
    hipStream_t st = (hipStream_t)stream;
    if (!e->metric_sums) {
        dyf_status s = dev_alloc(e, &e->metric_sums, 4);
        if (s != DYF_OK) return s;
    }
    HIP_TRY(e, launch_ensemble_metrics(preds_dev, targets_dev, n_members, n_points, e->metric_sums, st));
    double h[3];
    HIP_TRY(e, hipMemcpyAsync(h, e->metric_sums, sizeof(h), hipMemcpyDeviceToHost, st));
    HIP_TRY(e, hipStreamSynchronize(st));
    const double mse = h[0] / (double)n_points;
    out_host[0] = mse;
    out_host[1] = std::sqrt(h[1] / (double)n_points) / std::sqrt(mse);
    out_host[2] = h[2] / (double)n_points;
    return DYF_OK;
}

dyf_status dyf_apply_boundary_conditions(dyf_engine* e, const dyf_bc_args* bc, float* preds_dev, void* stream) {
    if (!e || !bc || !preds_dev) return fail(e, DYF_ERR_INVALID_ARGUMENT, "null argument");
    if (bc->kind != DYF_BC_NAVIER_STOKES && bc->kind != DYF_BC_SPRING_MESH)
        return fail(e, DYF_ERR_UNSUPPORTED, "Boundary conditions are implemented for navier-stokes and spring-mesh");
    if (bc->n_fields < 1 || bc->rows < 1 || bc->channels < 1 || bc->height < 1 || bc->width < 1 || bc->n_meta < 1)
        return fail(e, DYF_ERR_INVALID_ARGUMENT, "boundary conditions: bad geometry");
    if (!bc->row_meta_dev || !bc->fixed_mask_dev) return fail(e, DYF_ERR_INVALID_ARGUMENT, "row_meta / fixed_mask must be given");
    if (bc->kind == DYF_BC_NAVIER_STOKES && (!bc->in_velocity_dev || !bc->vertex_y_dev || !bc->time_factor_dev))
        return fail(e, DYF_ERR_INVALID_ARGUMENT, "navier-stokes boundary conditions need in_velocity, vertex_y and time_factor");
    if (bc->kind == DYF_BC_SPRING_MESH && !bc->boundary_dev)
        return fail(e, DYF_ERR_INVALID_ARGUMENT, "spring-mesh boundary conditions need the boundary values");
    HIP_TRY(e, hipSetDevice(e->cfg.device));
    BcArgs a{};
    a.preds = preds_dev; a.kind = bc->kind; a.n_fields = bc->n_fields; a.rows = bc->rows; a.c = bc->channels; a.h = bc->height;
    a.w = bc->width; a.n_meta = bc->n_meta; a.row_meta = bc->row_meta_dev; a.time_factor = bc->time_factor_dev; a.times_per_meta = bc->times_per_meta;
// ... 309 lines not shown
    if (c != 64 && c != 128) return fail(e, DYF_ERR_UNSUPPORTED, "dyf_op_linear_attention_fused: dim 64 or 128");
    HIP_TRY(e, hipSetDevice(e->cfg.device));
    hipStream_t st = (hipStream_t)stream;
    std::vector<el16_t> fq((size_t)384 * c), fo((size_t)c * 128);
    linattn_fused_pack(wqkv_host, wout_host, c, fq.data(), fo.data());
    const size_t nblk = ((size_t)hw + 255) / 256;
    const size_t scratch_floats = (size_t)n * 4 * (nblk * 1088 + 1024);
    float *scratch = nullptr, *bo = nullptr;
    el16_t *dq = nullptr, *dout = nullptr;
    hipError_t err = hipMalloc((void**)&scratch, scratch_floats * sizeof(float));
    if (err == hipSuccess) err = hipMalloc((void**)&bo, (size_t)c * sizeof(float));
    if (err == hipSuccess) err = hipMalloc((void**)&dq, fq.size() * sizeof(el16_t));
    if (err == hipSuccess) err = hipMalloc((void**)&dout, fo.size() * sizeof(el16_t));
    if (err == hipSuccess) err = hipMemcpy(bo, bout_host, (size_t)c * sizeof(float), hipMemcpyHostToDevice);
    if (err == hipSuccess) err = hipMemcpy(dq, fq.data(), fq.size() * sizeof(el16_t), hipMemcpyHostToDevice);
    if (err == hipSuccess) err = hipMemcpy(dout, fo.data(), fo.size() * sizeof(el16_t), hipMemcpyHostToDevice);
    if (err == hipSuccess) {
        LinAttnFusedArgs f{};
        f.xn = xn_dev; f.xres = xres_dev; f.n = n; f.hw = hw; f.c = c; f.wqkv_frag = dq; f.wout_frag = dout; f.bout = bo;
        f.y = y_dev; f.scratch = scratch; f.scratch_floats = (long long)scratch_floats;
        err = launch_linear_attention_fused(f, st);
    }
    if (err == hipSuccess) err = hipStreamSynchronize(st);
    (void)hipFree(scratch); (void)hipFree(bo); (void)hipFree(dq); (void)hipFree(dout);
    if (err != hipSuccess) return fail(e, DYF_ERR_HIP, std::string("dyf_op_linear_attention_fused: ") + hipGetErrorString(err));
    return DYF_OK;
}

dyf_status dyf_op_attention(dyf_engine* e, const uint16_t* qkv_dev, int32_t n, int32_t hw, uint16_t* out_dev, void* stream) {
    return dyf_op_attention_dropout(e, qkv_dev, n, hw, 0.0f, out_dev, stream);
}

dyf_status dyf_op_attention_dropout(dyf_engine* e, const uint16_t* qkv_dev, int32_t n, int32_t hw, float p, uint16_t* out_dev, void* stream) {
    if (!e || !qkv_dev || !out_dev || n < 1 || hw < 1 || p < 0.0f || p >= 1.0f) return fail(e, DYF_ERR_INVALID_ARGUMENT, "dyf_op_attention: bad arguments");
    if (p > 0.0f && e->attn_dropout_exact && hw > ATTN_EXACT_MAX_TOKENS)
        return fail(e, DYF_ERR_UNSUPPORTED, "dyf_op_attention_dropout: the exact form of the probability dropout takes at most 32767 tokens");
    HIP_TRY(e, hipSetDevice(e->cfg.device));
    hipStream_t st = (hipStream_t)stream;
    AttnArgs a{};
    a.qkv = qkv_dev; a.n = n; a.hw = hw; a.heads = 4; a.out = out_dev; a.drop = DropSpec{};
    if (p > 0.0f) {
        if (n > 2 * e->cfg.max_batch) return fail(e, DYF_ERR_INVALID_ARGUMENT, "more rows than the engine's row-key table (2 max_batch)");
        HIP_TRY(e, launch_rng_begin_forward(e->rng_state, e->row_keys, n, n, st));
        a.drop.mode = 1;
        a.drop.scale = 1.0f / (1.0f - p);
        a.drop.thresh16 = keep_threshold16(p);
        a.drop.thresh8 = keep_threshold8(p);
        a.drop.scale8 = 256.0f / (float)a.drop.thresh8;
        a.drop.attn_exact = e->attn_dropout_exact ? 1u : 0u;
        a.drop.salt = rng_layer_salt(0u);
        a.drop.row_keys = e->row_keys;
    }
    hipError_t err = launch_attention(a, st);
    if (err == hipSuccess) err = hipStreamSynchronize(st);
    if (err != hipSuccess) return fail(e, DYF_ERR_HIP, std::string("dyf_op_attention: ") + hipGetErrorString(err));
    return DYF_OK;
}

dyf_status dyf_op_attention_f32(dyf_engine* e, const float* qkv_dev, int32_t n, int32_t hw, float p, const uint8_t* mask_dev, int32_t form,
                                float* out_dev, void* stream) {
    if (!e || !qkv_dev || !out_dev || n < 1 || hw < 1 || p < 0.0f || p >= 1.0f || (form != 0 && form != 1) || (mask_dev && p <= 0.0f))
        return fail(e, DYF_ERR_INVALID_ARGUMENT, "dyf_op_attention_f32: bad arguments");
    HIP_TRY(e, hipSetDevice(e->cfg.device));
    return f32_op_attention(e, qkv_dev, n, hw, p, mask_dev, form, out_dev, (hipStream_t)stream);
}

dyf_status dyf_op_train_f32(dyf_engine* e, const dyf_train_op* desc, const float* const* inputs_dev, const float* const* params_host,
                            const float* dout_dev, float* y_dev, float* const* dinputs_dev, float* const* dparams_host, void* stream) {
    if (!e || !desc || !inputs_dev || !dout_dev || !y_dev) return fail(e, DYF_ERR_INVALID_ARGUMENT, "dyf_op_train_f32: bad arguments");
    HIP_TRY(e, hipSetDevice(e->cfg.device));
    return f32_op_train(e, desc, inputs_dev, params_host, dout_dev, y_dev, dinputs_dev, dparams_host, (hipStream_t)stream);
}

static dyf_status sample_op_net(dyf_engine* e, const dyf_sample_op& d, const dyf_sample_tensors& t, const float* const* params_host, hipStream_t st) {
    const int op = d.op;
    auto bad = [&](const char* m) { return fail(e, DYF_ERR_INVALID_ARGUMENT, std::string("dyf_op_sample16: ") + m); };
    auto unsup = [&](const char* m) { return fail(e, DYF_ERR_UNSUPPORTED, std::string("dyf_op_sample16: ") + m); };
    const bool readout = op == DYF_SOP_READOUT, tables = op == DYF_SOP_READOUT_TABLES, stem = op == DYF_SOP_STEM, stem16 = op == DYF_SOP_STEM16;
    const bool begin = op == DYF_SOP_RNG_BEGIN, clone = op == DYF_SOP_RNG_CLONE, tmlp = op == DYF_SOP_TIME_MLP, film = op == DYF_SOP_FILM;
    const bool cold = op == DYF_SOP_COLD_UPDATE, noisy = op == DYF_SOP_NOISY_CONDITION;
    if (!t.y) return bad("null output");
    if (d.k || d.pad || d.groups || d.act || d.film_stride || d.film_div || d.part_slots || t.residual || t.film_a || t.film_c || t.part)
        return bad("k / pad / groups / act / FiLM rows / residual / part belong to the kernels between the convs");
    const int allowed = readout ? DYF_SOP_NO_TABLES : stem16 ? DYF_SOP_FOLD_RNG : clone ? DYF_SOP_COUNTERS_ONLY : 0;
    if (d.flags & ~allowed) return bad("a flag the op does not take");
    const bool fold = stem16 && (d.flags & DYF_SOP_FOLD_RNG);
    if (!stem && (d.drop_mode != 0 || t.mask || d.drop_p != 0.0f || d.drop_site != 0)) return bad("the op has no dropout");
    if (!(stem || fold || begin) && d.drop_forward != 0) return bad("drop_forward on an op that starts no forward");
    if (!(stem || fold || begin || clone || noisy) && d.drop_row_offset != 0) return bad("drop_row_offset on an op without batch rows of the generator");
    if (!(readout || tables || stem || stem16) && (d.oh || d.ow || d.nearest)) return bad("oh / ow / nearest on an op without a resample");
    if (!(readout || tables) && (d.iw_store || t.col_map)) return bad("iw_store / col_map belong to the readout");
    if (!(stem || stem16 || begin) && d.src_rows) return bad("src_rows on an op without source rows");
    if (!noisy && d.tau != 0.0f) return bad("tau belongs to NOISY_CONDITION");
    if (!(stem || stem16 || film) && (d.nsrc || d.ch[0] || d.ch[1] || d.ch[2] || d.ch[3])) return bad("nsrc / ch on an op without sources or blocks");
    if (!(stem16 || begin || tables || film || cold) && (t.y2 || t.y3)) return bad("y2 / y3 on an op with one output");
    if (d.nb < 1 || d.h < 0 || d.w < 0 || d.c < 0 || d.c2 < 0 || d.oh < 0 || d.ow < 0 || d.src_rows < 0 || d.iw_store < 0 || d.nsrc < 0 || d.nsrc > 4 ||
        (d.nearest != 0 && d.nearest != 1))
        return bad("bad geometry");
    const int nparams = (readout || stem) ? 2 : tmlp ? (d.c2 > 0 ? 5 : 4) : film ? 4 : 0;
    if (nparams && !params_host) return bad("the op takes parameters");
    for (int i = 0; i < nparams; ++i)
        if (!params_host[i]) return bad("null parameter");
    int ctot = 0;
    for (int i = 0; i < 4; ++i) {
        if ((stem || stem16 || film) && ((i < d.nsrc) != (d.ch[i] > 0))) return bad("nsrc and ch go together");
        ctot += d.ch[i];
    }
    const long long hw = (long long)d.h * d.w;
    if (readout || tables) {
        if (d.h < 1 || d.w < 1 || d.oh < 1 || d.ow < 1) return bad("READOUT: (h, w) -> (oh, ow)");
        if ((d.iw_store > 0) != (t.col_map != nullptr) || d.iw_store > d.w) return bad("READOUT: iw_store (1..w) and col_map go together");
        if (tables ? (d.nb != 1 || d.c || d.c2 || !t.y2 || t.y3 || t.x[0]) : (d.c < 1 || d.c2 < 1 || !t.x[0])) return bad("READOUT: channels / tensors");
        if (readout && d.c2 > DYF_MAX_OUT_CH) return unsup("more output channels than the readout takes");
        if (readout && (size_t)16 * d.c * d.c2 * sizeof(float) > 64 * 1024) return unsup("readout weights beyond the LDS of the VALU forms");
        const long long iws = d.iw_store > 0 ? d.iw_store : d.w;
        if ((long long)d.nb * d.oh * d.ow >= (1ll << 30) || (long long)d.nb * d.h * iws * std::max(d.c, 64) * 2 >= 0x7F000000ll)
            return unsup("tensor too large for the kernels' 32-bit indices");
    } else if (stem || stem16) {
        if (d.h < 1 || d.w < 1 || d.oh < 1 || d.ow < 1 || d.nsrc < 1 || ctot != d.c) return bad("STEM: (h, w) -> (oh, ow), c = sum of ch");
        for (int i = 0; i < 4; ++i)
            if ((i < d.nsrc) != (t.x[i] != nullptr)) return bad("STEM: sources and their channel counts go together");
        if (d.src_rows > d.nb) return bad("STEM: src_rows above nb");
        if (stem ? (d.c2 < 1 || d.c > DYF_MAX_IN_CH) : (d.c2 != 0 || d.c > 15)) return unsup("STEM: c2 = dim and c <= 32 (STEM); c <= 15 and no c2 (STEM16)");
        if ((long long)d.nb * (d.oh + 2) * (d.ow + 2) * std::max(d.c2, 16) >= 0x7F000000ll || hw * d.c * d.nb >= 0x7F000000ll)
            return unsup("tensor too large for the kernels' 32-bit indices");
        if (fold ? (!t.y2 || !t.y3) : (t.y2 || t.y3)) return bad("STEM16: y2 / y3 go with DYF_SOP_FOLD_RNG");
        if (fold && d.nb > 2 * e->cfg.max_batch) return bad("more rows than the engine's row-key table (2 max_batch)");
    } else if (begin) {
        if (!t.y2 || t.y3 || d.nb > 2 * e->cfg.max_batch || d.src_rows > d.nb || d.h || d.w || d.c || d.c2) return bad("RNG_BEGIN: nb <= 2 max_batch rows, y and y2");
    } else if (clone) {
        if (!t.x[0] || d.nb != 1 || d.h || d.w || d.c || d.c2) return bad("RNG_CLONE: source and destination state");
    } else if (tmlp) {
        if (!t.x[0] || d.h || d.w || d.c < 4 || d.c % 2 != 0 || d.c > 4096 || d.c2 > 4096) return bad("TIME_MLP: times, an even dim of 4 .. 4096");
    } else if (film) {
        if (d.h || d.w || d.c < 1 || d.c2 || d.nsrc < 1 || !t.y2 || t.y3 || d.nb > 65535) return bad("FILM: c = tdim, 1..4 blocks, y and y2");
    } else {
        if (!t.x[0] || d.h < 1 || d.w < 1 || d.c < 1 || d.c2 || t.y3 || hw * d.c >= 0x7F000000ll || (long long)d.nb * hw * d.c >= (1ll << 38))
            return bad("COLD_UPDATE / NOISY_CONDITION: (nb, h, w, c) floats");
        if (cold ? !t.x[1] : (t.y2 != nullptr)) return bad("COLD_UPDATE needs x_next; NOISY_CONDITION has one output");
    }
    dyf_status ds = DYF_OK;
    if (stem) { ds = op_drop_check(e, d.nb, d.drop_mode, d.drop_p, t.mask, d.drop_site); if (ds != DYF_OK) return ds; }
    std::vector<int16_t> cmap;
    if (t.col_map) {
        cmap.resize((size_t)d.w);
        HIP_TRY(e, hipMemcpy(cmap.data(), t.col_map, cmap.size() * sizeof(int16_t), hipMemcpyDeviceToHost));
        for (int16_t v : cmap)
            if (v < -1 || v >= d.iw_store) return bad("READOUT: col_map entry outside the stored columns");
    }
    std::vector<void*> tmp;
    dyf_status rs = DYF_OK;
    hipError_t le = hipSuccess;
    {
        AllocScope scope(e, &tmp);
        auto upf = [&](const float** dst, const float* host, size_t n) {
            float* p = nullptr;
            const dyf_status us = dev_upload(e, &p, std::vector<float>(host, host + n));
            *dst = p;
            return us;
        };
        auto upi = [&](const int** dst, const std::vector<int>& host) {
            int* p = nullptr;
            const dyf_status us = dev_upload(e, &p, host);
            *dst = p;
            return us;
        };
        auto set_counters = [&](bool forward_too) -> dyf_status {
            const uint32_t words[2] = {d.drop_forward, d.drop_row_offset};
            HIP_TRY(e, hipDeviceSynchronize());
            if (forward_too) {
                HIP_TRY(e, hipMemcpy(e->rng_state + 2, words, sizeof(words), hipMemcpyHostToDevice));
            } else {
                HIP_TRY(e, hipMemcpy(e->rng_state + 3, words + 1, sizeof(uint32_t), hipMemcpyHostToDevice));
            }
            e->row_offset = d.drop_row_offset;
            e->row_offset_known = true;
            return DYF_OK;
        };
        if (readout || tables) {
            ReadoutArgs a{};
            a.x = (const el16_t*)t.x[0]; a.n = d.nb; a.ih = d.h; a.iw = d.w; a.cin = d.c; a.cout = d.c2; a.oh = d.oh; a.ow = d.ow;
            a.nearest = d.nearest; a.iw_store = d.iw_store > 0 ? d.iw_store : d.w; a.col_map = t.col_map; a.out = (float*)t.y;
            if (tables) {
                a.row_tab = (const uint4*)t.y; a.col_tab = (const uint4*)t.y2;
                le = launch_readout_tables(a, st);
            } else {
                const std::vector<float> pk = pack_readout_weights(params_host[0], d.c, d.c2);
                rs = upf(&a.wgt, pk.data(), pk.size());
                if (rs == DYF_OK) rs = upf(&a.bias, params_host[1], (size_t)d.c2);
                if (rs == DYF_OK && d.c == 64 && d.c2 <= 4) {
                    el16_t* wf = nullptr;
                    rs = dev_upload(e, &wf, pack_readout_frag(pk, d.c2));
                    a.wfrag = wf;
                    if (rs == DYF_OK && !(d.flags & DYF_SOP_NO_TABLES)) {
                        uint4 *rt = nullptr, *ct = nullptr;
                        rs = dev_alloc(e, &rt, (size_t)2 * d.oh);
                        if (rs == DYF_OK) rs = dev_alloc(e, &ct, (size_t)2 * d.ow);
                        a.row_tab = rt; a.col_tab = ct;
                        if (rs == DYF_OK) le = launch_readout_tables(a, st);
                    }
                }
                if (rs == DYF_OK && le == hipSuccess) {
                    le = launch_readout(a, st);
                    if (le == hipErrorInvalidValue && a.col_map) rs = unsup("launch_readout refuses a compact input without fragments");
                }
            }
        } else if (stem || stem16) {
            StemArgs a{};
            for (int i = 0; i < d.nsrc; ++i) { a.src[i] = (const float*)t.x[i]; a.ch[i] = d.ch[i]; }
            a.nsrc = d.nsrc; a.cin = d.c; a.n = d.nb; a.src_rows = d.src_rows; a.h = d.h; a.w = d.w; a.uh = d.oh; a.uw = d.ow;
            a.resample = (d.oh != d.h || d.ow != d.w) ? 1 : 0;
            a.nearest = d.nearest; a.dim = d.c2; a.out = (el16_t*)t.y;
            if (stem) {
                rs = upf(&a.wgt, params_host[0], (size_t)d.c2 * d.c);
                if (rs == DYF_OK) rs = upf(&a.bias, params_host[1], (size_t)d.c2);
                if (rs == DYF_OK) rs = op_drop_arm(e, d.nb, d.drop_mode, d.drop_p, t.mask, d.drop_site, d.drop_row_offset, d.drop_forward, st, &a.drop);
                if (rs == DYF_OK) le = launch_stem(a, st);
            } else {
                if (fold) {
                    rs = set_counters(true);
                    a.rng_state = e->rng_state; a.rng_row_keys = e->row_keys; a.rng_rows = d.nb; a.rng_rows_per_fwd = d.src_rows > 0 ? d.src_rows : d.nb;
                }
                if (rs == DYF_OK) le = launch_stem16(a, st);
            }
        } else if (begin) {
            rs = set_counters(true);
            if (rs == DYF_OK) le = launch_rng_begin_forward(e->rng_state, e->row_keys, d.nb, d.src_rows > 0 ? d.src_rows : d.nb, st);
        } else if (clone) {
            le = launch_rng_clone((uint32_t*)t.y, (const uint32_t*)t.x[0], d.drop_row_offset, (d.flags & DYF_SOP_COUNTERS_ONLY) != 0, st);
        } else if (tmlp) {
            TimeMlpArgs a{};
            const size_t td = (size_t)2 * d.c, nfeat = d.c2 > 0 ? (size_t)2 * d.c2 + 1 : (size_t)d.c;
            a.time = (const float*)t.x[0]; a.rows = d.nb; a.dim = d.c; a.silu_out = (float*)t.y;
            rs = upf(&a.w1, params_host[0], td * nfeat);
            if (rs == DYF_OK) rs = upf(&a.b1, params_host[1], td);
            if (rs == DYF_OK) rs = upf(&a.w2, params_host[2], td * td);
            if (rs == DYF_OK) rs = upf(&a.b2, params_host[3], td);
            if (rs == DYF_OK && d.c2 > 0) { rs = upf(&a.learned_w, params_host[4], (size_t)d.c2); a.learned_half = d.c2; }
            if (rs == DYF_OK) le = launch_time_mlp(a, st);
        } else if (film) {
            FilmArgs a{};
            a.silu = (const float*)t.x[0]; a.rows = d.nb; a.tdim = d.c; a.total_c = ctot; a.coef_a = (float*)t.y; a.coef_c = (float*)t.y2;
            std::vector<int> blk_of((size_t)ctot), blk_off((size_t)d.nsrc), blk_cout((size_t)d.nsrc);
            for (int i = 0, off = 0; i < d.nsrc; off += d.ch[i], ++i) {
                blk_off[i] = off;
                blk_cout[i] = d.ch[i];
                for (int c = 0; c < d.ch[i]; ++c) blk_of[off + c] = i;
            }
            rs = upf(&a.wf, params_host[0], (size_t)2 * ctot * d.c);
            if (rs == DYF_OK) rs = upf(&a.bf, params_host[1], (size_t)2 * ctot);
            if (rs == DYF_OK) rs = upf(&a.norm_a, params_host[2], (size_t)ctot);
            if (rs == DYF_OK) rs = upf(&a.norm_c, params_host[3], (size_t)ctot);
            if (rs == DYF_OK) rs = upi(&a.blk_of, blk_of);
            if (rs == DYF_OK) rs = upi(&a.blk_off, blk_off);
            if (rs == DYF_OK) rs = upi(&a.blk_cout, blk_cout);
            if (rs == DYF_OK) le = launch_film(a, st);
        } else if (cold) {
            le = launch_cold_update((float*)t.y, (const float*)t.x[0], (const float*)t.x[1], (long long)d.nb * hw * d.c, st, (float*)t.y2);
        } else {
            if (!t.x[1]) rs = set_counters(false);
            if (rs == DYF_OK)
                le = launch_noisy_condition((float*)t.y, (const float*)t.x[0], (const float*)t.x[1], d.tau, (long long)d.nb * hw * d.c, (int)(hw * d.c),
                                            e->rng_state, st);
        }
    }
    if (rs == DYF_OK) {
        if (le == hipSuccess) le = hipStreamSynchronize(st);
        if (le == hipSuccess && (fold || begin)) {
            le = hipMemcpy(fold ? t.y2 : t.y, e->row_keys, (size_t)2 * d.nb * sizeof(uint32_t), hipMemcpyDeviceToDevice);
            if (le == hipSuccess) le = hipMemcpy(fold ? t.y3 : t.y2, e->rng_state, DYF_RNG_STATE_WORDS * sizeof(uint32_t), hipMemcpyDeviceToDevice);
        }
        if (le != hipSuccess) rs = fail(e, DYF_ERR_HIP, std::string("dyf_op_sample16: ") + hipGetErrorString(le));
    } else {
        (void)hipDeviceSynchronize();
    }
    release_allocs(tmp);
    return rs;
}

dyf_status dyf_op_sample16(dyf_engine* e, const dyf_sample_op* desc, const dyf_sample_tensors* t, const float* const* params_host, void* stream) {
    if (e && desc && t && desc->op >= DYF_SOP_READOUT && desc->op <= DYF_SOP_NOISY_CONDITION) {
        HIP_TRY(e, hipSetDevice(e->cfg.device));
        return sample_op_net(e, *desc, *t, params_host, (hipStream_t)stream);
    }
    if (!e || !desc || !t || !t->x[0] || !t->y) return fail(e, DYF_ERR_INVALID_ARGUMENT, "dyf_op_sample16: null argument");
    const dyf_sample_op& d = *desc;
    if (d.op < DYF_SOP_GN_ACT || d.op > DYF_SOP_UP2_EPILOGUE) return fail(e, DYF_ERR_INVALID_ARGUMENT, "dyf_op_sample16: unknown op");
    if (d.oh || d.ow || d.nearest || d.src_rows || d.iw_store || d.tau != 0.0f || t->col_map || t->y2 || t->y3)
        return fail(e, DYF_ERR_INVALID_ARGUMENT, "dyf_op_sample16: oh / ow / nearest / src_rows / iw_store / tau / col_map / y2 / y3 belong to the launchers around the networks");
    if (d.nb < 1 || d.h < 1 || d.w < 1 || d.c < 1 || d.c2 < 0 || d.k < 0 || d.pad < 0 || d.groups < 0 || d.film_stride < 0 || d.film_div < 0 ||
        d.part_slots < 0 || d.nsrc < 0 || (d.flags & ~DYF_SOP_NO_STATS))
        return fail(e, DYF_ERR_INVALID_ARGUMENT, "dyf_op_sample16: bad geometry or flags");
    const int op = d.op;
    const bool gn = op == DYF_SOP_GN_ACT, gnf = op == DYF_SOP_GROUPNORM_F32, epi = op == DYF_SOP_UP2_EPILOGUE, stem = op == DYF_SOP_STEM_CONV;
    const bool up = op == DYF_SOP_UP2_NEAREST || op == DYF_SOP_UP2_BILINEAR || epi;
// ... 133 lines not shown
```

### dyffusion_amd/csrc/engine_internal.h

```cpp
#pragma once
#include <algorithm>
#include <cmath>
#include <cstdio>
#include <cstdlib>
#include <cstring>
#include <map>
#include <string>
#include <vector>

#include "../../include/dyffusion_hip.h"
#include "conv.h"
#include "kernels.h"

#define DYF_SPLITK_FLOATS (32ll << 20)

namespace dyf {

struct TrainState;
struct RNet;
struct SNet;

inline thread_local std::string g_create_error;

struct UBlock {
    int cin = 0, cout = 0, k = 0, stride = 1, pad = 0;
    bool gn = false;
    bool transposed = false;
    int act = ACT_NONE;
    int film_off = 0;
    int in_h = 0, in_w = 0;
    int out_h = 0, out_w = 0;
    ConvW wpk;
    el16_t* wpk_up = nullptr;
    el16_t* wpk_up_frag = nullptr;
    int16_t* up_cols = nullptr;
    int16_t* up_cbase = nullptr;
    int16_t* up_cidx = nullptr;
    int16_t* up_col_map = nullptr;
    int up_wo_store = 0;
    int up_ntiles = 0, up_npad = 0, up_nvalid0 = 0, up_nvalid1 = 0;
    int up_mix[3] = {0, 0, 0};
    float* gamma = nullptr;
    float* beta = nullptr;
    float* static_a = nullptr;
    float* static_c = nullptr;
};

struct Net {
    dyf_net_config cfg{};
    bool loaded = false;
    int cin_total = 0, dim = 0, tdim = 0, total_c = 0;
    int uh = 0, uw = 0;
    UBlock blk[12];
    float *t_w1 = nullptr, *t_b1 = nullptr, *t_w2 = nullptr, *t_b2 = nullptr;
    float* t_learned = nullptr;
    float *stem_w = nullptr, *stem_b = nullptr;
    float *film_w = nullptr, *film_b = nullptr, *norm_a = nullptr, *norm_c = nullptr;
    int *blk_of = nullptr, *blk_off = nullptr, *blk_cout = nullptr;
    float *ro_w = nullptr, *ro_b = nullptr;
    el16_t* ro_wfrag = nullptr;
    uint4 *ro_row_tab = nullptr, *ro_col_tab = nullptr;
    bool ro_tab_sparse = false;
    ConvW enc0_fused_w;
    bool stem_fused = false;
    double flops_per_sample = 0.0;
    int n_drop_sites = 12;
    struct RNet* rn = nullptr;
    struct SNet* sc = nullptr;
    std::map<float, int> table_of_time;
    float* tables = nullptr;
    int ntables = 0;
};

struct Workspace {
    el16_t* stem = nullptr;
    el16_t* stem16 = nullptr;
    el16_t* enc[6] = {};
    float* enc5_raw = nullptr;
    el16_t* up = nullptr;
    el16_t* dec[6] = {};
    float* silu = nullptr;
    float* coef_a = nullptr;
    float* coef_c = nullptr;
    el16_t* zero_page = nullptr;
    float* up_border = nullptr;
    float* coef_pair = nullptr;
    float* splitk = nullptr;
    float* ones_f = nullptr;
    float* zeros_f = nullptr;
};

struct PlanHost {
    bool set = false;
    std::vector<dyf_plan_step> steps;
    std::vector<float> refine_times;
    std::vector<int> refine_slots;
    dyf_plan hdr{};
};

struct GraphEntry {
    hipGraph_t graph = nullptr;
    hipGraphExec_t exec = nullptr;
};

}

struct dyf_engine {
    dyf_engine_config cfg{};
    std::string err;
    dyf::Net net[2];
    dyf::Workspace ws;
    std::vector<void*> allocs;
    std::vector<void*> net_allocs[2];
    std::vector<void*> plan_allocs;
    std::vector<void*>* alloc_sink = nullptr;
    dyf::PlanHost plan;
    int C = 0, Cs = 0, wC = 0;
    float *s_init = nullptr, *s_static = nullptr, *s_xs = nullptr, *s_x0hat = nullptr, *s_next = nullptr,
          *s_cur = nullptr, *s_noisy = nullptr, *s_stack = nullptr;
    float* s_time = nullptr;
    uint32_t* rng_state = nullptr;
    uint32_t row_offset = 0;
    bool row_offset_known = false;
    uint32_t* row_keys = nullptr;
    int stack_slots = 0;
    std::map<int, dyf::GraphEntry> graphs;
    int sample_precision = 16;
    int attn_dropout_exact = 0;
    void* f32_arena = nullptr;
    size_t f32_bytes = 0, f32_used = 0;
    bool f32_forward = false;
    int fuse_min_plane = 32;
    bool fuse_stem = true;
    bool fuse_up2x = true;
    hipStream_t cap_stream = nullptr;
    double* metric_sums = nullptr;
    int prof_layer = -1;
    std::vector<std::pair<hipEvent_t, hipEvent_t>> prof_ev;
    std::vector<int> prof_rows;
    float* s_pair = nullptr;
    float* refine_coef = nullptr;
    float* pair_coef = nullptr;
    bool pair_interp = true;
    void* comm = nullptr;
    int comm_rank = 0, comm_world = 1;
    float* gather_recv = nullptr;
    size_t gather_recv_floats = 0;
    std::vector<dyf_engine*> groups;
    bool is_group_child = false;
    int train_precision = 0;
    int train_deterministic = 0;
    double* criterion_partials = nullptr;
    int form_rows_scale = 1;
    hipStream_t group_stream = nullptr;
    hipEvent_t group_done = nullptr;
    hipEvent_t group_fork = nullptr;
    int group_min_rows = 16;
    int last_groups = 0, last_per = 0, last_nb = 0;
    bool log_on = false;
// ... 16 lines not shown
namespace dyf {

struct ProfScope {
    dyf_engine* e;
    hipStream_t st;
    hipEvent_t e0 = nullptr, e1 = nullptr;
    ProfScope(dyf_engine* eng, bool match, int rows, hipStream_t s) : e(eng), st(s) {
        if (!match || e->prof_ev.size() >= 4096) return;
        if (hipEventCreate(&e0) != hipSuccess || hipEventCreate(&e1) != hipSuccess || hipEventRecord(e0, st) != hipSuccess) {
            e0 = e1 = nullptr;
            return;
        }
        e->prof_rows.push_back(rows);
    }
    ~ProfScope() {
        if (!e0) return;
        (void)hipEventRecord(e1, st);
        e->prof_ev.emplace_back(e0, e1);
    }
};
#define DYF_PROF_RESNET_BASE 100
#define DYF_PROF_RN_CONV3_L0 0
#define DYF_PROF_RN_ATTENTION 1
#define DYF_PROF_RN_GN_L0 2

inline dyf_status fail(dyf_engine* e, dyf_status st, const std::string& msg) {
    if (e) e->err = msg; else g_create_error = msg;
    return st;
}

#define HIP_TRY(e, expr)                                                                                   \
    do {                                                                                                   \
        hipError_t _err = (expr);                                                                          \
        if (_err != hipSuccess)                                                                            \
            return fail(e, DYF_ERR_HIP, std::string(#expr) + ": " + hipGetErrorString(_err));              \
    } while (0)

inline int conv_path(const dyf_engine* e, const ConvArgs& a) { return (e->cfg.enable_mfma && conv_mfma_supported(a)) ? 1 : 0; }
inline int conv_form_rows(const dyf_engine* e, int n) {
    if (e->cfg.batch_invariant) return 2 * e->cfg.max_batch;
    return e->form_rows_scale > 1 ? n * e->form_rows_scale : 0;
}

template <typename T>
dyf_status dev_alloc(dyf_engine* e, T** out, size_t count) {
    void* p = nullptr;
    size_t bytes = std::max<size_t>(count * sizeof(T), 256);
    HIP_TRY(e, hipMalloc(&p, bytes));
    HIP_TRY(e, hipMemset(p, 0, bytes));
    (e->alloc_sink ? *e->alloc_sink : e->allocs).push_back(p);
    *out = (T*)p;
    return DYF_OK;
}

struct AllocScope {
    dyf_engine* e;
    std::vector<void*>* prev;
    AllocScope(dyf_engine* eng, std::vector<void*>* list) : e(eng), prev(eng->alloc_sink) { e->alloc_sink = list; }
    ~AllocScope() { e->alloc_sink = prev; }
};

inline void release_allocs(std::vector<void*>& list) {
    for (void* p : list) (void)hipFree(p);
    list.clear();
}

template <typename T>
dyf_status dev_upload(dyf_engine* e, T** out, const std::vector<T>& host) {
    dyf_status st = dev_alloc(e, out, host.size());
    if (st != DYF_OK) return st;
    if (!host.empty()) HIP_TRY(e, hipMemcpy(*out, host.data(), host.size() * sizeof(T), hipMemcpyHostToDevice));
    return DYF_OK;
}

inline std::vector<el16_t> pack_conv(const float* w, int cout, int cin, int taps) {
    std::vector<el16_t> pk((size_t)cout * taps * cin);
    for (int co = 0; co < cout; ++co)
        for (int ci = 0; ci < cin; ++ci)
            for (int t = 0; t < taps; ++t) pk[((size_t)co * taps + t) * cin + ci] = f32_to_el16(w[((size_t)co * cin + ci) * taps + t]);
    return pk;
}

inline dyf_status upload_conv_weights(dyf_engine* e, ConvW* out, const std::vector<el16_t>& pk, int cout, int taps, int cin,
                                      bool enc0_stem = false) {
    *out = ConvW{};
    auto up = [&](const el16_t** dst, const std::vector<el16_t>& host) {
        el16_t* p = nullptr;
        const dyf_status st = dev_upload(e, &p, host);
        *dst = p;
        return st;
    };
    dyf_status st = up(&out->wpk, pk);
    if (st != DYF_OK || cout % 64 != 0 || cin % 64 != 0 || (size_t)cout * taps * cin != pk.size()) return st;
    std::vector<el16_t> pf;
    if (taps <= 32) {
        pf.assign(pk.size(), el16_t{});
        pack_conv_frag(pk.data(), cout, taps, cin, pf.data());
        if ((st = up(&out->frag, pf)) != DYF_OK) return st;
    }
    if (enc0_stem && (cout == 64 || cout == 128)) {
        pf.assign(pk.size(), el16_t{});
        pack_enc0_stem_frag(pk.data(), cout, pf.data());
        out->halo_order = HaloOrder::Enc0Stem;
    } else if (taps == 16 && cout % 128 == 0) {
        pf.assign((size_t)cout * 16 * 4 * cin, el16_t{});
        pack_halo_s2_frag(pk.data(), cout, cin, pf.data());
        out->halo_order = HaloOrder::S2;
    } else if (taps == 9 && cout % 256 != 0) {
        pf.assign((size_t)cout * 16 * cin, el16_t{});
        pack_halo3_frag64(pk.data(), cout, cin, pf.data());
        out->halo_order = HaloOrder::Halo3_64;
    } else if (taps == 9) {
        pf.assign((size_t)cout * 16 * cin, el16_t{});
        pack_halo3_frag(pk.data(), cout, cin, pf.data());
        out->halo_order = HaloOrder::Halo3_256;
    }
    if (out->halo_order != HaloOrder::None && (st = up(&out->halo, pf)) != DYF_OK) return st;
    if (out->halo_order == HaloOrder::Halo3_256) {
        pack_halo3_frag64(pk.data(), cout, cin, pf.data());
        st = up(&out->frag64, pf);
    }
    return st;
}

struct TensorView {
    const float* data;
    std::vector<int64_t> shape;
    int64_t numel() const {
        int64_t n = 1;
        for (auto s : shape) n *= s;
        return n;
    }
};


struct Source {
    const float* p;
    int ch;
};

struct FwdOpts {
    const float* coef_a;
    const float* coef_c;
    int coef_stride;
    int dropout_mode;
    const uint8_t* const* masks;
    int src_rows = 0;
    int coef_div = 0;
    const float* time_dev = nullptr;
    float time_value = 0.0f;
};


}

struct dyf_train_op;
namespace dyf {
dyf_status train_store_params(dyf_engine* e, int which, std::map<std::string, TensorView>& sd);
void train_destroy(dyf_engine* e);
dyf_status f32_net_forward(dyf_engine* e, int which, const Source* srcs, int nsrc, int nb, const FwdOpts& o, float* out_dev,
                           hipStream_t st);
dyf_status f32_prepare(dyf_engine* e);
void f32_destroy(dyf_engine* e);
dyf_status f32_op_attention(dyf_engine* e, const float* qkv, int nb, int N, float p, const uint8_t* mask, int form, float* out, hipStream_t st);
dyf_status f32_op_train(dyf_engine* e, const struct dyf_train_op* d, const float* const* inputs, const float* const* params, const float* dout,
                        float* y, float* const* dinputs, float* const* dparams, hipStream_t st);
inline size_t f32_arena_block(size_t bytes) { return (std::max<size_t>(bytes, 256) + 255) / 256 * 256; }
inline void* f32_arena_take(dyf_engine* e, size_t bytes) {
    const size_t b = f32_arena_block(bytes);
    if (!e->f32_arena || e->f32_used + b > e->f32_bytes) return nullptr;
    void* p = (char*)e->f32_arena + e->f32_used;
    e->f32_used += b;
    return p;
}
inline bool sample_f32_walk(const dyf_engine* e) { return e->sample_precision == 32 || e->sample_precision == 48; }
inline int graph_key(const dyf_engine* e, int nb) {
    return nb | (e->sample_precision == 32 ? 1 << 30 : 0) | (e->sample_precision == 48 ? 1 << 28 : 0) | (e->attn_dropout_exact ? 1 << 29 : 0);
}
}

namespace dyf {
std::string sc_configure(dyf_engine* e, Net& n);
dyf_status sc_alloc_workspace(dyf_engine* e);
dyf_status sc_load_weights(dyf_engine* e, Net& n, std::map<std::string, TensorView>& sd);
// ... 18 lines not shown
```

### dyffusion_amd/csrc/kernels.h

```cpp
#pragma once
#include "common.h"

#include <vector>

#define DYF_MAX_IN_CH 32
#define DYF_MAX_OUT_CH 8

struct TimeMlpArgs {
    const float* time;
    int rows, dim;
    const float* w1;
    const float* b1;
    const float* w2;
    const float* b2;
    float* silu_out;
    const float* learned_w = nullptr;
    int learned_half = 0;
};
hipError_t launch_time_mlp(const TimeMlpArgs& a, hipStream_t s);

struct FilmArgs {
    const float* silu;
    int rows, tdim, total_c;
    const float* wf;
    const float* bf;
    const int* blk_of;
    const int* blk_off;
    const int* blk_cout;
    const float* norm_a;
    const float* norm_c;
    float* coef_a;
    float* coef_c;
};
hipError_t launch_film(const FilmArgs& a, hipStream_t s);

struct StemArgs {
    const float* src[4];
    int ch[4];
    int nsrc, cin;
    int n, h, w;
    int src_rows;
    int uh, uw;
    int resample;
    int nearest;
    const float* wgt;
    const float* bias;
    int dim;
    el16_t* out;
    DropSpec drop;
    uint32_t* rng_state;
    uint32_t* rng_row_keys;
    int rng_rows, rng_rows_per_fwd;
};
hipError_t launch_stem(const StemArgs& a, hipStream_t s);
hipError_t launch_stem16(const StemArgs& a, hipStream_t s);

struct Up2xArgs {
    const el16_t* src0;
    const el16_t* src1;
    int c0, c1;
    int n, h, w;
    el16_t* out;
};
hipError_t launch_up2x(const Up2xArgs& a, hipStream_t s);

struct Up2xEpiArgs {
    const float* lo;
    int n, h, w, c;
    const float* coef_a;
    const float* coef_c;
    int coef_stride, coef_div;
    int act;
    DropSpec drop;
    el16_t* out;
};
hipError_t launch_up2x_epilogue(const Up2xEpiArgs& a, hipStream_t s);

struct GroupNormArgs {
    const float* x;
    int n, hw, c, groups;
    const float* gamma;
    const float* beta;
    const float* film_a;
    const float* film_c;
    int film_stride;
    int film_div;
    int act;
    DropSpec drop;
    el16_t* out;
};
hipError_t launch_groupnorm(const GroupNormArgs& a, hipStream_t s);

struct ReadoutArgs {
    const el16_t* x;
    int n, ih, iw, cin;
    int iw_store;
    const int16_t* col_map;
    const float* wgt;
    const el16_t* wfrag;
    const float* bias;
    int cout;
    int oh, ow;
    int nearest;
    float* out;
    const uint4* row_tab;
    const uint4* col_tab;
};
hipError_t launch_readout(const ReadoutArgs& a, hipStream_t s);
hipError_t launch_readout_tables(const ReadoutArgs& a, hipStream_t s);
inline std::vector<float> pack_readout_weights(const float* w, int cin, int cout) {
    std::vector<float> pk((size_t)16 * cin * cout);
    for (int ci = 0; ci < cin; ++ci)
        for (int co = 0; co < cout; ++co)
            for (int t = 0; t < 16; ++t) pk[((size_t)t * cin + ci) * cout + co] = w[((size_t)ci * cout + co) * 16 + t];
    return pk;
}
inline std::vector<el16_t> pack_readout_frag(const std::vector<float>& pk, int cout) {
    std::vector<el16_t> wf((size_t)16 * 2 * 64 * 8, 0);
    for (int t = 0; t < 16; ++t)
        for (int h2 = 0; h2 < 2; ++h2)
            for (int lane = 0; lane < 64; ++lane) {
                const int m = lane & 15, kg = lane >> 4;
                for (int el = 0; el < 8; ++el)
                    if (m < cout)
                        wf[(((size_t)t * 2 + h2) * 64 + lane) * 8 + el] = f32_to_el16(pk[((size_t)t * 64 + h2 * 32 + kg * 8 + el) * cout + m]);
            }
    return wf;
}

hipError_t launch_cold_update(float* x_s, const float* x_cur, const float* x_next, long long count, hipStream_t s, float* copy = nullptr);
hipError_t launch_noisy_condition(float* out, const float* cond, const float* noise, float tau, long long count,
                                  int row_elems, uint32_t* rng_state, hipStream_t s);
#define DYF_RNG_STATE_WORDS 8

struct BcArgs {
    float* preds;
    int kind;
    int n_fields, rows, c, h, w, n_meta;
// ... 22 lines not shown
```

### dyffusion_amd/csrc/kernels.hip

```cpp
#include "kernels.h"

#include <cstdlib>

__device__ __forceinline__ float wave_sum(float v) {
#pragma unroll
    for (int off = 32; off > 0; off >>= 1) v += __shfl_xor(v, off, 64);
    return v;
}

__device__ __forceinline__ float block_sum(float v, float* scratch ) {
    v = wave_sum(v);
    const int lane = threadIdx.x & 63, wave = threadIdx.x >> 6, nw = (blockDim.x + 63) >> 6;
    __syncthreads();
    if (lane == 0) scratch[wave] = v;
    __syncthreads();
    float t = 0.0f;
    for (int i = 0; i < nw; ++i) t += scratch[i];
    return t;
}

__global__ void time_mlp_kernel(TimeMlpArgs a) {
    extern __shared__ float sh[];
    const int row = blockIdx.x, tdim = 2 * a.dim, half = a.dim / 2;
    const int dim = a.learned_w ? 2 * a.learned_half + 1 : a.dim;
// ... 76 lines not shown
        const int n = (int)(pix / ((long long)a.uh * a.uw));
        const int rem = (int)(pix % ((long long)a.uh * a.uw));
        const int y = rem / a.uw, x = rem % a.uw;
        int y0 = y, y1 = y, x0 = x, x1 = x;
        float ly = 0.0f, lx = 0.0f;
        if (a.resample) {
            bilinear_coord(y, (float)a.h / (float)a.uh, a.h, y0, y1, ly, a.nearest != 0);
            bilinear_coord(x, (float)a.w / (float)a.uw, a.w, x0, x1, lx, a.nearest != 0);
        }
        int cbase = 0;
        for (int s = 0; s < a.nsrc; ++s) {
            const float* src = a.src[s] + (size_t)(a.src_rows > 0 ? n % a.src_rows : n) * a.ch[s] * a.h * a.w;
            for (int c = 0; c < a.ch[s]; ++c) {
                const float* p = src + (size_t)c * a.h * a.w;
                const float v00 = p[y0 * a.w + x0], v01 = p[y0 * a.w + x1];
                const float v10 = p[y1 * a.w + x0], v11 = p[y1 * a.w + x1];
                const float top = v00 * (1.0f - lx) + v01 * lx;
                const float bot = v10 * (1.0f - lx) + v11 * lx;
                vals[(cbase + c) * 256 + tid] = top * (1.0f - ly) + bot * ly;
            }
            cbase += a.ch[s];
        }
    }
    __syncthreads();
    if (!live) return;
    el16_t* out = a.out + (size_t)pix * a.dim;
    const int n_row = (int)(pix / ((long long)a.uh * a.uw));
    const RngKey dkey = drop_row_key(a.drop, n_row);
    const uint32_t row0 = (uint32_t)n_row * (uint32_t)(a.uh * a.uw * a.dim);
    for (int d0 = 0; d0 < a.dim; d0 += 8) {
        float acc[8];
#pragma unroll
        for (int t = 0; t < 8; ++t) acc[t] = (d0 + t < a.dim) ? a.bias[d0 + t] : 0.0f;
        for (int c = 0; c < a.cin; ++c) {
            const float v = vals[c * 256 + tid];
#pragma unroll
            for (int t = 0; t < 8; ++t)
                if (d0 + t < a.dim) acc[t] = fmaf(a.wgt[(size_t)(d0 + t) * a.cin + c], v, acc[t]);
        }
        if (a.drop.mode != 0) {
#pragma unroll
            for (int t = 0; t < 8; ++t)
                if (d0 + t < a.dim) acc[t] = drop_apply(acc[t], (uint32_t)(pix * a.dim + d0 + t), row0, a.drop, dkey);
        }
        if ((a.dim & 7) == 0) {
            uint4 o;
            o.x = pack_el16x2(acc[0], acc[1]);
            o.y = pack_el16x2(acc[2], acc[3]);
            o.z = pack_el16x2(acc[4], acc[5]);
            o.w = pack_el16x2(acc[6], acc[7]);
            *(uint4*)(out + d0) = o;
        } else {
#pragma unroll
            for (int t = 0; t < 8; ++t)
                if (d0 + t < a.dim) out[d0 + t] = f32_to_el16(acc[t]);
        }
    }
}

hipError_t launch_stem(const StemArgs& a, hipStream_t s) {
    const long long total = (long long)a.n * a.uh * a.uw;
    dyf_form_note("stem_kernel", a.n);
    hipLaunchKernelGGL(stem_kernel, dim3((unsigned)((total + 255) / 256)), dim3(256), (size_t)a.cin * 256 * sizeof(float),
                       s, a);
    return hipGetLastError();
}

__device__ __forceinline__ void stem_rng_begin(const StemArgs& a) {
    if (a.rng_state == nullptr || blockIdx.x != 0) return;
    const uint32_t lo = a.rng_state[0], hi = a.rng_state[1], fwd0 = a.rng_state[2], row0 = a.rng_state[3];
    for (int r = threadIdx.x; r < a.rng_rows; r += blockDim.x) {
        const RngKey k = rng_row_key(lo, hi, fwd0 + (uint32_t)(r / a.rng_rows_per_fwd), row0 + (uint32_t)(r % a.rng_rows_per_fwd));
        a.rng_row_keys[2 * r] = k.k0;
        a.rng_row_keys[2 * r + 1] = k.k1;
    }
    __syncthreads();
    if (threadIdx.x == 0) a.rng_state[2] = fwd0 + (uint32_t)((a.rng_rows + a.rng_rows_per_fwd - 1) / a.rng_rows_per_fwd);
}

__global__ __launch_bounds__(256) void stem16_kernel(StemArgs a) {
    stem_rng_begin(a);
    const long long idx = (long long)blockIdx.x * 256 + threadIdx.x;
    const int ph = a.uh + 2, pw = a.uw + 2;
    const long long total = (long long)a.n * ph * pw;
    if (idx >= total) return;
    const int n = (int)(idx / ((long long)ph * pw));
    const int rem = (int)(idx % ((long long)ph * pw));
    const int y = rem / pw - 1, x = rem % pw - 1;
    uint32_t w[8] = {0, 0, 0, 0, 0, 0, 0, 0};
    if ((unsigned)y < (unsigned)a.uh && (unsigned)x < (unsigned)a.uw) {
        int y0 = y, y1 = y, x0 = x, x1 = x;
        float ly = 0.0f, lx = 0.0f;
        if (a.resample) {
            bilinear_coord(y, (float)a.h / (float)a.uh, a.h, y0, y1, ly, a.nearest != 0);
            bilinear_coord(x, (float)a.w / (float)a.uw, a.w, x0, x1, lx, a.nearest != 0);
        }
        const int e0 = a.ch[0], e1 = e0 + (a.nsrc > 1 ? a.ch[1] : 0), e2 = e1 + (a.nsrc > 2 ? a.ch[2] : 0);
        const int nrow = a.src_rows > 0 ? n % a.src_rows : n;
        const int o00 = y0 * a.w + x0, o01 = y0 * a.w + x1, o10 = y1 * a.w + x0, o11 = y1 * a.w + x1;
        const size_t plane = (size_t)a.h * a.w;
        float v[16];
#pragma unroll
        for (int k = 0; k < 16; ++k) {
            float val = 0.0f;
            if (k < a.cin) {
                const int si = k < e0 ? 0 : (k < e1 ? 1 : (k < e2 ? 2 : 3));
                const int cl = k - (si == 0 ? 0 : (si == 1 ? e0 : (si == 2 ? e1 : e2)));
                const float* p = a.src[si] + ((size_t)nrow * a.ch[si] + cl) * plane;
                const float top = p[o00] * (1.0f - lx) + p[o01] * lx;
                const float bot = p[o10] * (1.0f - lx) + p[o11] * lx;
                val = top * (1.0f - ly) + bot * ly;
            } else if (k == a.cin) {
                val = 1.0f;
            }
            v[k] = val;
        }
#pragma unroll
        for (int k = 0; k < 8; ++k) w[k] = pack_el16x2(v[2 * k], v[2 * k + 1]);
    }
    uint4* o = (uint4*)(a.out + (size_t)idx * 16);
    o[0] = make_uint4(w[0], w[1], w[2], w[3]);
    o[1] = make_uint4(w[4], w[5], w[6], w[7]);
}

constexpr int ST_ROWS = 8;
template <int CP>
__global__ __launch_bounds__(512) void stem16_rows_kernel(StemArgs a, int nblk) {
    extern __shared__ __attribute__((aligned(16))) float st_rows[];
    stem_rng_begin(a);
    const int ph = a.uh + 2, pw = a.uw + 2;
    const int n = blockIdx.x / nblk, rb = blockIdx.x - n * nblk;
    const int py0 = rb * ST_ROWS, py1 = min(py0 + ST_ROWS, ph);
    const int ya = max(py0 - 1, 0), yb = min(py1 - 2, a.uh - 1);
    const float ys = (float)a.h / (float)a.uh, xs = (float)a.w / (float)a.uw;
    int sbase = 0;
    if (ya <= yb) {
        int s0 = ya, s1 = yb, t0, t1;
        float l;
        if (a.resample) {
            bilinear_coord(ya, ys, a.h, s0, t0, l, a.nearest != 0);
            bilinear_coord(yb, ys, a.h, t1, s1, l, a.nearest != 0);
        }
        sbase = s0;
        const int nsrc_rows = s1 - s0 + 1;
        const int nrow = a.src_rows > 0 ? n % a.src_rows : n;
        const size_t plane = (size_t)a.h * a.w;
        const int per_row = a.cin * a.w;
        for (int j = threadIdx.x; j < per_row; j += 512) {
            const int k = j / a.w, x = j - k * a.w;
            int si = 0, cl = k;
            while (cl >= a.ch[si]) cl -= a.ch[si++];
            const float* sp = a.src[si] + ((size_t)nrow * a.ch[si] + cl) * plane + (size_t)s0 * a.w + x;
            float* dp = st_rows + (size_t)x * CP + k;
            float tmp[ST_ROWS + 2];
#pragma unroll
            for (int r = 0; r < ST_ROWS + 2; ++r) tmp[r] = r < nsrc_rows ? sp[(size_t)r * a.w] : 0.0f;
#pragma unroll
            for (int r = 0; r < ST_ROWS + 2; ++r)
                if (r < nsrc_rows) dp[(size_t)r * a.w * CP] = tmp[r];
        }
    }
    int4* xtab = (int4*)(st_rows + (size_t)(ST_ROWS + 2) * a.w * CP);
    int4* ytab = xtab + pw;
    for (int px = threadIdx.x; px < pw + ST_ROWS; px += 512) {
        if (px < pw) {
            const int x = px - 1;
            int x0 = x, x1 = x;
            float lx = 0.0f;
            const bool ok = (unsigned)x < (unsigned)a.uw;
            if (ok && a.resample) bilinear_coord(x, xs, a.w, x0, x1, lx, a.nearest != 0);
            xtab[px] = make_int4(ok ? x0 * CP : 0, ok ? x1 * CP : 0, __float_as_int(lx), ok);
        } else {
            const int r = px - pw, y = py0 + r - 1;
            int y0 = y, y1 = y;
            float ly = 0.0f;
            const bool ok = (unsigned)y < (unsigned)a.uh && py0 + r < py1;
            if (ok && a.resample) bilinear_coord(y, ys, a.h, y0, y1, ly, a.nearest != 0);
            ytab[r] = make_int4(ok ? (y0 - sbase) * a.w * CP : 0, ok ? (y1 - sbase) * a.w * CP : 0, __float_as_int(ly), ok);
        }
    }
    __syncthreads();
    uint4* oblk = (uint4*)(a.out + (((size_t)n * ph + py0) * pw) * 16);
    if (a.cin <= 8 && (a.uw & 63) == 0) {
        const int lane = threadIdx.x & 63, wave = threadIdx.x >> 6;
        unsigned char* stg = (unsigned char*)(ytab + ST_ROWS) + wave * 2048;
        const uint4 zero4 = make_uint4(0, 0, 0, 0);
        const uint4 half1 = a.cin == 8 ? make_uint4(pack_el16x2(1.0f, 0.0f), 0, 0, 0) : zero4;
        for (int i = threadIdx.x; i < (py1 - py0) * 4; i += 512) {
            const int rr = i >> 2, q = i & 3;
            oblk[(size_t)rr * 2 * pw + (q < 2 ? q : 2 * pw - 4 + q)] = zero4;
        }
        const int total_in = (py1 - py0) * a.uw;
        int r = 0, j = threadIdx.x;
        while (j >= a.uw) { j -= a.uw; ++r; }
        for (int i = threadIdx.x; i < total_in; i += 512) {
            const int4 xt = xtab[j + 1], yt = ytab[r];
            uint4 w = zero4;
            if (yt.w) {
                const int x0 = xt.x, x1 = xt.y;
                const float lx = __int_as_float(xt.z), ly = __int_as_float(yt.z);
                const float* r0 = st_rows + yt.x;
                const float* r1 = st_rows + yt.y;
                float v[8];
#pragma unroll
                for (int q = 0; q < 2; ++q) {
                    float t00[4] = {0, 0, 0, 0}, t01[4] = {0, 0, 0, 0}, t10[4] = {0, 0, 0, 0}, t11[4] = {0, 0, 0, 0};
                    if (4 * q < CP) {
                        const float4 p00 = *(const float4*)(r0 + x0 + 4 * q), p01 = *(const float4*)(r0 + x1 + 4 * q);
                        const float4 p10 = *(const float4*)(r1 + x0 + 4 * q), p11 = *(const float4*)(r1 + x1 + 4 * q);
                        t00[0] = p00.x; t00[1] = p00.y; t00[2] = p00.z; t00[3] = p00.w;
                        t01[0] = p01.x; t01[1] = p01.y; t01[2] = p01.z; t01[3] = p01.w;
                        t10[0] = p10.x; t10[1] = p10.y; t10[2] = p10.z; t10[3] = p10.w;
                        t11[0] = p11.x; t11[1] = p11.y; t11[2] = p11.z; t11[3] = p11.w;
                    }
#pragma unroll
                    for (int e = 0; e < 4; ++e) {
                        const int k = 4 * q + e;
                        const float top = t00[e] * (1.0f - lx) + t01[e] * lx;
                        const float bot = t10[e] * (1.0f - lx) + t11[e] * lx;
                        float val = top * (1.0f - ly) + bot * ly;
                        if (k >= a.cin) val = k == a.cin ? 1.0f : 0.0f;
                        v[k] = val;
                    }
                }
                w = make_uint4(pack_el16x2(v[0], v[1]), pack_el16x2(v[2], v[3]), pack_el16x2(v[4], v[5]), pack_el16x2(v[6], v[7]));
            }
            *(uint4*)(stg + lane * 32) = w;
            *(uint4*)(stg + lane * 32 + 16) = yt.w ? half1 : zero4;
            uint4* dst = oblk + (size_t)r * 2 * pw + 2 * (1 + j - lane) + lane;
            dst[0] = *(const uint4*)(stg + lane * 16);
            dst[64] = *(const uint4*)(stg + 1024 + lane * 16);
            j += 512;
            while (j >= a.uw) { j -= a.uw; ++r; }
        }
        return;
    }
    const int total = (py1 - py0) * 2 * pw;
    int r = 0, j = threadIdx.x;
    for (int i = threadIdx.x; i < total; i += 512) {
        const int px = j >> 1, half = j & 1;
        const int4 xt = xtab[px], yt = ytab[r];
        uint32_t w[4] = {0, 0, 0, 0};
        if (xt.w && yt.w) {
            const int x0 = xt.x, x1 = xt.y;
            const float lx = __int_as_float(xt.z), ly = __int_as_float(yt.z);
            const float* r0 = st_rows + yt.x;
            const float* r1 = st_rows + yt.y;
            float v[8];
#pragma unroll
            for (int q2 = 0; q2 < 2; ++q2) {
                const int q = 2 * half + q2;
                float t00[4] = {0, 0, 0, 0}, t01[4] = {0, 0, 0, 0}, t10[4] = {0, 0, 0, 0}, t11[4] = {0, 0, 0, 0};
                if (4 * q < CP) {
                    const float4 p00 = *(const float4*)(r0 + x0 + 4 * q), p01 = *(const float4*)(r0 + x1 + 4 * q);
                    const float4 p10 = *(const float4*)(r1 + x0 + 4 * q), p11 = *(const float4*)(r1 + x1 + 4 * q);
                    t00[0] = p00.x; t00[1] = p00.y; t00[2] = p00.z; t00[3] = p00.w;
                    t01[0] = p01.x; t01[1] = p01.y; t01[2] = p01.z; t01[3] = p01.w;
                    t10[0] = p10.x; t10[1] = p10.y; t10[2] = p10.z; t10[3] = p10.w;
                    t11[0] = p11.x; t11[1] = p11.y; t11[2] = p11.z; t11[3] = p11.w;
                }
#pragma unroll
                for (int e = 0; e < 4; ++e) {
                    const int k = 4 * q + e;
                    const float top = t00[e] * (1.0f - lx) + t01[e] * lx;
                    const float bot = t10[e] * (1.0f - lx) + t11[e] * lx;
                    float val = top * (1.0f - ly) + bot * ly;
                    if (k >= a.cin) val = k == a.cin ? 1.0f : 0.0f;
                    v[4 * q2 + e] = val;
                }
            }
#pragma unroll
            for (int k = 0; k < 4; ++k) w[k] = pack_el16x2(v[2 * k], v[2 * k + 1]);
        }
        oblk[i] = make_uint4(w[0], w[1], w[2], w[3]);
        j += 512;
        if (j >= 2 * pw) { j -= 2 * pw; ++r; }
    }
}

hipError_t launch_stem16(const StemArgs& a, hipStream_t s) {
    const int cp = (a.cin + 3) / 4 * 4;
    const size_t lds = (size_t)(ST_ROWS + 2) * a.w * cp * sizeof(float) + (size_t)(a.uw + 2 + ST_ROWS) * 16 + 8 * 2048;
    const bool rows = dyf_form_int("DYF_STEM16_ROWS", 1) != 0;
    if (rows && lds <= 48 * 1024 && cp <= 16 && a.h <= a.uh && 2 * (a.uw + 2) >= 512) {
        const int nblk = (a.uh + 2 + ST_ROWS - 1) / ST_ROWS;
        const dim3 grid((unsigned)(a.n * nblk)), block(512);
        dyf_form_note("stem16_rows_kernel", a.n);
        KernelProf kp("stem16_rows_kernel", s, (double)(a.src_rows ? a.src_rows : a.n) * a.h * a.w * a.cin * 4.0 + (double)a.n * (a.uh + 2) * (a.uw + 2) * 16 * 2.0);
        if (cp == 4) hipLaunchKernelGGL(stem16_rows_kernel<4>, grid, block, lds, s, a, nblk);
        else if (cp == 8) hipLaunchKernelGGL(stem16_rows_kernel<8>, grid, block, lds, s, a, nblk);
        else if (cp == 12) hipLaunchKernelGGL(stem16_rows_kernel<12>, grid, block, lds, s, a, nblk);
        else hipLaunchKernelGGL(stem16_rows_kernel<16>, grid, block, lds, s, a, nblk);
        return hipGetLastError();
    }
    const long long total = (long long)a.n * (a.uh + 2) * (a.uw + 2);
    dyf_form_note("stem16_kernel", a.n);
    hipLaunchKernelGGL(stem16_kernel, dim3((unsigned)((total + 255) / 256)), dim3(256), 0, s, a);
    return hipGetLastError();
}

template <int VEC>
__global__ __launch_bounds__(256) void up2x_kernel(Up2xArgs a, long long total) {
    const long long idx = (long long)blockIdx.x * 256 + threadIdx.x;
    if (idx >= total) return;
    const int c = a.c0 + a.c1;
    const int groups = c / VEC;
    const int g = (int)(idx % groups);
    const long long pix = idx / groups;
    const int ow = 2 * a.w, oh = 2 * a.h;
    const int n = (int)(pix / ((long long)oh * ow));
    const int rem = (int)(pix % ((long long)oh * ow));
    const int y = rem / ow, x = rem % ow;
    int y0, y1, x0, x1;
    float ly, lx;
    bilinear_coord(y, 0.5f, a.h, y0, y1, ly);
    bilinear_coord(x, 0.5f, a.w, x0, x1, lx);
    int ch = g * VEC;
    const el16_t* src = a.src0;
    int cs = a.c0;
    if (ch >= a.c0) {
        src = a.src1;
        cs = a.c1;
        ch -= a.c0;
    }
    const size_t base = (size_t)n * a.h * a.w;
    const el16_t* p00 = src + ((base + (size_t)y0 * a.w + x0) * cs + ch);
    const el16_t* p01 = src + ((base + (size_t)y0 * a.w + x1) * cs + ch);
    const el16_t* p10 = src + ((base + (size_t)y1 * a.w + x0) * cs + ch);
    const el16_t* p11 = src + ((base + (size_t)y1 * a.w + x1) * cs + ch);
    el16_t* o = a.out + ((size_t)pix * c + g * VEC);
    if (VEC == 8) {
        const uint4 q00 = *(const uint4*)p00, q01 = *(const uint4*)p01, q10 = *(const uint4*)p10, q11 = *(const uint4*)p11;
        const uint32_t* w00 = (const uint32_t*)&q00;
        const uint32_t* w01 = (const uint32_t*)&q01;
        const uint32_t* w10 = (const uint32_t*)&q10;
        const uint32_t* w11 = (const uint32_t*)&q11;
        uint32_t r[4];
#pragma unroll
        for (int t = 0; t < 4; ++t) {
            float lo, hi;
            {
                const float a00 = el16_lo(w00[t]), a01 = el16_lo(w01[t]);
                const float a10 = el16_lo(w10[t]), a11 = el16_lo(w11[t]);
                const float top = a00 * (1.0f - lx) + a01 * lx, bot = a10 * (1.0f - lx) + a11 * lx;
                lo = top * (1.0f - ly) + bot * ly;
            }
            {
                const float a00 = el16_hi(w00[t]), a01 = el16_hi(w01[t]);
                const float a10 = el16_hi(w10[t]), a11 = el16_hi(w11[t]);
                const float top = a00 * (1.0f - lx) + a01 * lx, bot = a10 * (1.0f - lx) + a11 * lx;
                hi = top * (1.0f - ly) + bot * ly;
            }
            r[t] = pack_el16x2(lo, hi);
        }
        *(uint4*)o = make_uint4(r[0], r[1], r[2], r[3]);
    } else {
        const float a00 = el16_to_f32(*p00), a01 = el16_to_f32(*p01), a10 = el16_to_f32(*p10), a11 = el16_to_f32(*p11);
        const float top = a00 * (1.0f - lx) + a01 * lx, bot = a10 * (1.0f - lx) + a11 * lx;
        *o = f32_to_el16(top * (1.0f - ly) + bot * ly);
    }
}

__global__ __launch_bounds__(256) void up2x_quad_kernel(Up2xArgs a, long long total) {
    const long long idx = (long long)blockIdx.x * 256 + threadIdx.x;
    if (idx >= total) return;
    const int c = a.c0 + a.c1, groups = c >> 3;
    const int g = (int)(idx % groups);
    const int pix = (int)(idx / groups);
    const int plane = a.h * a.w;
    const int n = pix / plane, rem = pix - n * plane;
    const int i = rem / a.w, j = rem - i * a.w;
    int ch = g * 8;
    const el16_t* src = a.src0;
    int cs = a.c0;
    if (ch >= a.c0) {
        src = a.src1;
        cs = a.c1;
        ch -= a.c0;
// ... 1108 lines not shown
```

### dyffusion_amd/engine.py

```python
import ctypes as C
from typing import Dict, List, Optional, Sequence

import numpy as np
import torch

from . import _lib as L


class EngineError(RuntimeError):
    pass


def _raise(status: int, msg: str):
    if status == L.DYF_ERR_INVALID_ARGUMENT:
        raise ValueError(msg)
    if status == L.DYF_ERR_UNSUPPORTED:
        raise NotImplementedError(msg)
    raise EngineError(msg)


def net_config(*, in_channels: int, cond_channels: int, out_channels: int, dim: int, with_time_emb: bool = True,
               upsample_dims: Optional[Sequence[int]] = (256, 256), dropout: float = 0.0,
               input_dropout: float = 0.0, outer_sample_mode: str = "bilinear") -> L.NetConfig:
    uh, uw = (0, 0) if upsample_dims is None else (int(upsample_dims[0]), int(upsample_dims[1]))
# ... 832 lines not shown
            if t.dtype != (torch.float32 if f32_in else dt) or not t.is_cuda or not t.is_contiguous() or t.dim() != 4:
                raise ValueError(f"{op}: inputs are contiguous 4-d device tensors of dtype {torch.float32 if f32_in else dt}")
        if not 1 <= len(xs) <= (4 if op == "stem_conv" else 2 if op == "up2_bilinear" else 1):
            raise ValueError(f"{op}: {len(xs)} inputs")
        x = xs[0]
        ps = [np.ascontiguousarray(t.detach().to("cpu", torch.float32).numpy()) for t in params]
        desc, tens = L.SampleOp(), L.SampleTensors()
        desc.op, desc.groups, desc.act, desc.film_div = L.SAMPLE_OPS[op], int(groups), L.ACTS[act], int(film_div)
        desc.flags = 0 if stats else L.SOP_NO_STATS
        if op == "stem_conv":
            nb, _, h, w = x.shape
            c = sum(t.shape[1] for t in xs)
            desc.nsrc, desc.k, desc.pad = len(xs), int(k), int(pad)
            for i, t in enumerate(xs):
                if (t.shape[0], t.shape[2], t.shape[3]) != (nb, h, w):
                    raise ValueError("stem_conv: the sources share (nb, h, w)")
                desc.ch[i] = t.shape[1]
            if len(ps) != 2 or ps[0].shape[1:] != (c, k, k) or ps[1].shape != (ps[0].shape[0],):
                raise ValueError("stem_conv: params are weight (dim, cin, k, k) and bias (dim)")
            desc.c2 = ps[0].shape[0]
            out_shape, out_dt = (nb, h, w, desc.c2), dt
        else:
            nb, h, w, c = x.shape
            want = {"gn_act": [(c,), (c,)], "groupnorm_f32": [(c,), (c,)], "layernorm_c": [(c,)]}.get(op, [])
            out_shape, out_dt = (nb, h, w, c), dt
            if op == "head":
                if len(ps) != 2 or ps[0].ndim != 2 or ps[0].shape[1] != c:
                    raise ValueError("head: params are weight (cout, c) and bias (cout)")
                desc.c2 = ps[0].shape[0]
                want = [(desc.c2, c), (desc.c2,)]
                out_shape, out_dt = (nb, desc.c2, h, w), torch.float32
            elif op == "up2_bilinear":
                if len(xs) == 2:
                    if xs[1].shape[:3] != x.shape[:3]:
                        raise ValueError("up2_bilinear: the sources share (nb, h, w)")
                    desc.c2 = xs[1].shape[3]
                out_shape = (nb, 2 * h, 2 * w, c + desc.c2)
            elif op in ("up2_nearest", "up2_epilogue"):
                out_shape = (nb, 2 * h, 2 * w, c)
            if len(ps) != len(want) or any(t.size != int(np.prod(sh)) for t, sh in zip(ps, want)):
                raise ValueError(f"{op}: parameters must have the shapes {want}")
        desc.nb, desc.h, desc.w, desc.c = nb, h, w, c
        for i, t in enumerate(xs):
            tens.x[i] = t.data_ptr()
        keep = []
        if (film_a is None) != (film_c is None):
            raise ValueError("film_a and film_c go together")
        if film_a is not None:
            film_a, film_c = _f32c(film_a, "film_a"), _f32c(film_c, "film_c")
            rows = -(-nb // film_div) if film_div > 1 else nb
            if film_a.dim() != 2 or film_a.shape != film_c.shape or film_a.shape[0] != rows or film_a.shape[1] < c:
                raise ValueError(f"film rows must be ({rows}, >= {c}) fp32")
            desc.film_stride = film_a.shape[1]
            tens.film_a, tens.film_c = film_a.data_ptr(), film_c.data_ptr()
            keep += [film_a, film_c]
        if residual is not None:
            if residual.dtype != dt or not residual.is_cuda or not residual.is_contiguous() or tuple(residual.shape) != tuple(x.shape):
                raise ValueError("residual: a contiguous 16-bit device tensor of the input's shape")
            tens.residual = residual.data_ptr()
        if part is not None:
            part = _f32c(part, "part")
            if part.dim() != 4 or part.shape[0] != nb or part.shape[2] * 8 != c or part.shape[3] != 2:
                raise ValueError("part: fp32 (nb, slots, c / 8, 2)")
            desc.part_slots = part.shape[1]
            tens.part = part.data_ptr()
            keep.append(part)
        desc.drop_p = float(p)
        if mask is not None and rng_site is not None:
            raise ValueError("mask or rng_site, not both")
        if mask is not None:
            if mask.dtype != torch.uint8 or not mask.is_cuda or not mask.is_contiguous() or tuple(mask.shape) != out_shape:
                raise ValueError("mask: a contiguous uint8 device tensor of the output's shape")
            desc.drop_mode, tens.mask = 2, mask.data_ptr()
        elif rng_site is not None:
            desc.drop_mode, desc.drop_site, desc.drop_row_offset, desc.drop_forward = 1, int(rng_site), int(rng_row_offset), int(rng_forward)
        y = torch.empty(out_shape, dtype=out_dt, device=x.device)
        tens.y = y.data_ptr()
        arr = (C.c_void_p * max(len(ps), 1))(*[t.ctypes.data for t in ps])
        self._check(self._lib.dyf_op_sample16(self._h, C.byref(desc), C.byref(tens), arr, self._stream()))
        return y

    def _op_sample_net(self, op, xs, params, *, mask=None, p=0.0, rng_site=None, rng_row_offset=0, rng_forward=0, out_hw=None, in_hw=None,
                       nearest=False, src_rows=0, nb=None, col_map=None, tables=True, fold_rng=False, counters_only=False, dst=None, tau=0.0,
                       blocks=(), copy=False, iw_store=None):
        given = {k for k, v, d in (("mask", mask, None), ("p", p, 0.0), ("rng_site", rng_site, None), ("rng_row_offset", rng_row_offset, 0),
                                   ("rng_forward", rng_forward, 0), ("out_hw", out_hw, None), ("in_hw", in_hw, None), ("nearest", nearest, False),
                                   ("src_rows", src_rows, 0), ("nb", nb, None), ("col_map", col_map, None), ("tables", tables, True),
                                   ("fold_rng", fold_rng, False), ("counters_only", counters_only, False), ("dst", dst, None), ("tau", tau, 0.0),
                                   ("blocks", blocks, ()), ("copy", copy, False), ("iw_store", iw_store, None)) if v is not d and v != d}
        takes = {"readout": {"out_hw", "nearest", "col_map", "tables"}, "readout_tables": {"in_hw", "out_hw", "nearest", "col_map", "iw_store"},
                 "stem": {"out_hw", "nearest", "src_rows", "nb", "mask", "p", "rng_site", "rng_row_offset", "rng_forward"},
                 "stem16": {"out_hw", "nearest", "src_rows", "nb", "fold_rng", "rng_row_offset", "rng_forward"},
                 "rng_begin": {"nb", "src_rows", "rng_row_offset", "rng_forward"}, "rng_clone": {"dst", "rng_row_offset", "counters_only"},
                 "time_mlp": set(), "film": {"blocks", "nb"}, "cold_update": {"copy"}, "noisy_condition": {"tau", "rng_row_offset"}}[op]
        if given - takes:
            raise ValueError(f"{op}: does not take {sorted(given - takes)}")
        dev = torch.device("cuda", self.device)
        ps = [np.ascontiguousarray(t.detach().to("cpu", torch.float32).numpy()) for t in params]
        desc, tens = L.SampleOp(), L.SampleTensors()
        desc.op = L.SAMPLE_OPS[op]
        for t in xs:
            if not t.is_cuda or not t.is_contiguous():
                raise ValueError(f"{op}: inputs are contiguous device tensors")
        dt = self.torch_dtype
        i32 = lambda *shape: torch.zeros(shape, dtype=torch.int32, device=dev)
        f32 = lambda *shape: torch.empty(shape, dtype=torch.float32, device=dev)
        want = lambda t, d, n: t.dtype == d and t.dim() == n
        outs = None
        if op in ("readout", "readout_tables"):
            desc.oh, desc.ow, desc.nearest = int(out_hw[0]), int(out_hw[1]), int(bool(nearest))
            if col_map is not None:
                if col_map.dtype != torch.int16 or not col_map.is_cuda or not col_map.is_contiguous() or col_map.dim() != 1:
                    raise ValueError(f"{op}: col_map is a contiguous int16 device vector")
                tens.col_map = col_map.data_ptr()
            if op == "readout":
                if len(xs) != 1 or not want(xs[0], dt, 4) or len(ps) != 2 or ps[0].ndim != 4 or ps[0].shape[0] != xs[0].shape[3] or ps[0].shape[2:] != (4, 4):
                    raise ValueError("readout: x 16-bit (nb, ih, iw_store, cin), weight (cin, cout, 4, 4), bias (cout)")
                desc.nb, desc.h, iws, desc.c = xs[0].shape
                desc.c2 = ps[0].shape[1]
                desc.w = iws if col_map is None else col_map.numel()
                desc.iw_store = 0 if col_map is None else iws
                desc.flags = 0 if tables else L.SOP_NO_TABLES
                outs = [f32(desc.nb, desc.c2, desc.oh, desc.ow)]
            else:
                desc.nb, desc.h, desc.w = 1, int(in_hw[0]), int(in_hw[1])
                desc.iw_store = 0 if col_map is None else int(iw_store)
                outs = [i32(desc.oh, 8), i32(desc.ow, 8)]
        elif op in ("stem", "stem16"):
            if not 1 <= len(xs) <= 4 or any(not want(t, torch.float32, 4) or t.shape[0] != xs[0].shape[0] or t.shape[2:] != xs[0].shape[2:] for t in xs):
                raise ValueError(f"{op}: 1..4 fp32 NCHW sources of one (rows, h, w)")
            rows, _, desc.h, desc.w = xs[0].shape
            desc.nb = rows if nb is None else int(nb)
            desc.src_rows = int(src_rows)
            if (desc.src_rows if desc.src_rows > 0 else desc.nb) != rows:
                raise ValueError(f"{op}: the sources hold src_rows (or nb) rows")
            desc.nsrc, desc.c = len(xs), sum(t.shape[1] for t in xs)
            for i, t in enumerate(xs):
                desc.ch[i] = t.shape[1]
            desc.oh, desc.ow, desc.nearest = int(out_hw[0]), int(out_hw[1]), int(bool(nearest))
            if op == "stem":
                if len(ps) != 2 or ps[0].ndim != 2 or ps[0].shape[1] != desc.c or ps[1].shape != (ps[0].shape[0],):
                    raise ValueError("stem: params are weight (dim, cin) and bias (dim)")
                desc.c2 = ps[0].shape[0]
                outs = [torch.empty((desc.nb, desc.oh, desc.ow, desc.c2), dtype=dt, device=dev)]
                desc.drop_p = float(p)
                if mask is not None and rng_site is not None:
                    raise ValueError("mask or rng_site, not both")
                if mask is not None:
                    if mask.dtype != torch.uint8 or not mask.is_cuda or not mask.is_contiguous() or tuple(mask.shape) != tuple(outs[0].shape):
                        raise ValueError("mask: a contiguous uint8 device tensor of the output's shape")
                    desc.drop_mode, tens.mask = 2, mask.data_ptr()
                elif rng_site is not None:
                    desc.drop_mode, desc.drop_site, desc.drop_row_offset, desc.drop_forward = 1, int(rng_site), int(rng_row_offset), int(rng_forward)
            else:
                outs = [torch.empty((desc.nb, desc.oh + 2, desc.ow + 2, 16), dtype=dt, device=dev)]
                if fold_rng:
                    desc.flags, desc.drop_row_offset, desc.drop_forward = L.SOP_FOLD_RNG, int(rng_row_offset), int(rng_forward)
                    outs += [i32(desc.nb, 2), i32(L.RNG_STATE_WORDS)]
        elif op == "rng_begin":
            desc.nb, desc.src_rows, desc.drop_row_offset, desc.drop_forward = int(nb), int(src_rows), int(rng_row_offset), int(rng_forward)
            outs = [i32(desc.nb, 2), i32(L.RNG_STATE_WORDS)]
        elif op == "rng_clone":
            if len(xs) != 1 or dst is None or any(t.dtype != torch.int32 or tuple(t.shape) != (L.RNG_STATE_WORDS,) for t in (xs[0], dst)):
                raise ValueError("rng_clone: source and destination states are int32 (8,)")
            desc.nb, desc.drop_row_offset, desc.flags = 1, int(rng_row_offset), L.SOP_COUNTERS_ONLY if counters_only else 0
            outs = [dst.clone()]
        elif op == "time_mlp":
            if len(xs) != 1 or not want(xs[0], torch.float32, 1) or len(ps) not in (4, 5) or ps[2].ndim != 2:
                raise ValueError("time_mlp: times fp32 (rows,), params w1, b1, w2, b2 (, learned weights)")
            desc.nb, desc.c = xs[0].shape[0], ps[2].shape[0] // 2
            desc.c2 = ps[4].size if len(ps) == 5 else 0
            nfeat = 2 * desc.c2 + 1 if desc.c2 else desc.c
            if [t.shape for t in ps[:4]] != [(2 * desc.c, nfeat), (2 * desc.c,), (2 * desc.c, 2 * desc.c), (2 * desc.c,)]:
                raise ValueError("time_mlp: parameter shapes")
            outs = [f32(desc.nb, 2 * desc.c)]
        elif op == "film":
            total = sum(blocks)
            if len(ps) != 4 or ps[0].ndim != 2 or [t.shape for t in ps] != [(2 * total, ps[0].shape[1]), (2 * total,), (total,), (total,)] or not 1 <= len(blocks) <= 4:
                raise ValueError("film: params wf (2 total, tdim), bf, norm_a, norm_c; 1..4 blocks")
            desc.c = ps[0].shape[1]
            if xs and (len(xs) != 1 or not want(xs[0], torch.float32, 2) or xs[0].shape[1] != desc.c):
                raise ValueError("film: SiLU rows fp32 (rows, tdim)")
            desc.nb = xs[0].shape[0] if xs else int(nb)
            desc.nsrc = len(blocks)
            for i, c in enumerate(blocks):
                desc.ch[i] = int(c)
            outs = [f32(desc.nb, total), f32(desc.nb, total)]
        elif op == "cold_update":
            if len(xs) != 3 or any(not want(t, torch.float32, 4) or t.shape != xs[0].shape for t in xs):
                raise ValueError("cold_update: x_s, x_cur, x_next fp32 of one 4-d shape")
            desc.nb, desc.c, desc.h, desc.w = xs[0].shape
            outs = [xs[0].clone()] + ([torch.empty_like(xs[0])] if copy else [])
            xs = xs[1:]
        elif op == "noisy_condition":
            if not 1 <= len(xs) <= 2 or any(not want(t, torch.float32, 4) or t.shape != xs[0].shape for t in xs):
                raise ValueError("noisy_condition: cond (and noise) fp32 (nb, c, h, w)")
            desc.nb, desc.c, desc.h, desc.w = xs[0].shape
            desc.tau, desc.drop_row_offset = float(tau), int(rng_row_offset)
            outs = [torch.empty_like(xs[0])]
        for i, t in enumerate(xs):
            tens.x[i] = t.data_ptr()
        tens.y = outs[0].data_ptr()
        if len(outs) > 1:
            tens.y2 = outs[1].data_ptr()
        if len(outs) > 2:
            tens.y3 = outs[2].data_ptr()
        arr = (C.c_void_p * max(len(ps), 1))(*[t.ctypes.data for t in ps])
        self._check(self._lib.dyf_op_sample16(self._h, C.byref(desc), C.byref(tens), arr, self._stream()))
        if op == "cold_update":
            return outs[0], (outs[1] if copy else None)
        return outs[0] if len(outs) == 1 else tuple(outs)

    def op_upconv2d(self, x_nhwc_bf16: torch.Tensor, weight: torch.Tensor, scale: Optional[torch.Tensor] = None,
                    shift: Optional[torch.Tensor] = None, act: int = 0) -> torch.Tensor:
        assert x_nhwc_bf16.dtype == torch.bfloat16 and x_nhwc_bf16.is_cuda and x_nhwc_bf16.is_contiguous()
        n, h, w, cin = x_nhwc_bf16.shape
        cout = weight.shape[0]
        wh = np.ascontiguousarray(weight.detach().to("cpu", torch.float32).numpy())
        y = torch.empty((n, 2 * h, 2 * w, cout), dtype=torch.bfloat16, device=x_nhwc_bf16.device)
        if scale is not None:
            scale, shift = _f32c(scale, "scale"), _f32c(shift, "shift")
        self._check(self._lib.dyf_op_upconv2d(self._h, x_nhwc_bf16.data_ptr(), wh.ctypes.data, n, h, w, cin, cout,
                                              None if scale is None else scale.data_ptr(),
                                              None if shift is None else shift.data_ptr(), act, y.data_ptr(),
                                              self._stream()))
        return y


class EngineLoss(torch.autograd.Function):

    @staticmethod
    def forward(ctx, anchor, owner, value):
        ctx.owner = owner
        ctx.step_id = owner._train_state["step_id"]
        return anchor.new_tensor(value)

    @staticmethod
    def backward(ctx, grad_out):
        st = getattr(ctx.owner, "_train_state", None)
        eng = None if st is None else st.get("eng")
# ... 81 lines not shown
```

### include/dyffusion_hip_testing.h

```cpp
#ifndef DYFFUSION_HIP_TESTING_H
#define DYFFUSION_HIP_TESTING_H

#include "dyffusion_hip.h"

#ifdef __cplusplus
extern "C" {
#endif

dyf_status dyf_time_conv_layer(dyf_engine* engine, int32_t net, int32_t layer, int32_t nb, int32_t iters,
                               void* stream, double* avg_ms, double* flops, double* algorithmic_bytes);

dyf_status dyf_time_layer_in_rollout(dyf_engine* engine, int32_t layer, int32_t nb, void* stream, double* avg_ms,
                                     int32_t* launches);

dyf_status dyf_time_kernel_in_rollout(dyf_engine* engine, int32_t kind, int32_t nb, void* stream, double* avg_ms,
                                      int32_t* launches, double* flops, double* algorithmic_bytes);

dyf_status dyf_time_named_kernel_in_rollout(dyf_engine* engine, const char* kernel, int32_t nb, void* stream, double* total_ms,
                                            int32_t* launches, double* total_bytes);

dyf_status dyf_op_conv2d(dyf_engine* engine, const uint16_t* x_dev, const float* w_host, int32_t n, int32_t h,
                         int32_t w, int32_t cin, int32_t cout, int32_t kh, int32_t kw, int32_t stride, int32_t pad,
                         const float* scale_dev, const float* shift_dev, int32_t act, int32_t path, uint16_t* y_dev,
                         void* stream);

typedef struct {
    const uint16_t* x1_dev;
    const uint16_t* residual_dev;
    float* y_f32_dev;
    const uint8_t* mask_dev;
    int32_t c1;
    int32_t coef_div;
    int32_t n_sel;
    int32_t drop_mode;
    float drop_p;
    int32_t drop_site;
    uint32_t drop_row_offset;
    uint32_t drop_forward;
} dyf_conv_ex;
dyf_status dyf_op_conv2d_ex(dyf_engine* engine, const uint16_t* x_dev, const float* w_host, int32_t n, int32_t h,
                            int32_t w, int32_t cin, int32_t cout, int32_t kh, int32_t kw, int32_t stride, int32_t pad,
                            const float* scale_dev, const float* shift_dev, int32_t act, int32_t path, uint16_t* y_dev,
                            const dyf_conv_ex* ex, void* stream);

dyf_status dyf_op_upconv2d(dyf_engine* engine, const uint16_t* x_dev, const float* w_host, int32_t n, int32_t h,
                           int32_t w, int32_t cin, int32_t cout, const float* scale_dev, const float* shift_dev,
                           int32_t act, uint16_t* y_dev, void* stream);

dyf_status dyf_op_linear_attention(dyf_engine* engine, const uint16_t* qkv_dev, int32_t n, int32_t hw, uint16_t* out_dev,
                                   void* stream);

dyf_status dyf_op_linear_attention_fused(dyf_engine* engine, const uint16_t* xn_dev, const uint16_t* xres_dev, int32_t n,
                                         int32_t hw, int32_t c, const float* wqkv_host, const float* wout_host,
                                         const float* bout_host, uint16_t* y_dev, void* stream);

dyf_status dyf_op_attention(dyf_engine* engine, const uint16_t* qkv_dev, int32_t n, int32_t hw, uint16_t* out_dev,
                            void* stream);
dyf_status dyf_op_attention_dropout(dyf_engine* engine, const uint16_t* qkv_dev, int32_t n, int32_t hw, float p, uint16_t* out_dev,
                                    void* stream);
dyf_status dyf_op_attention_f32(dyf_engine* engine, const float* qkv_dev, int32_t n, int32_t hw, float p, const uint8_t* mask_dev,
                                int32_t form, float* out_dev, void* stream);

dyf_status dyf_train_conv_check(dyf_engine* engine, int32_t kind, int32_t n, int32_t h, int32_t w, int32_t cin, int32_t cout,
                                int32_t k, int32_t s, int32_t p, uint32_t seed, float* out_host);

typedef enum dyf_train_op_kind {
    DYF_TOP_CONV = 0, DYF_TOP_GN_ACT = 1, DYF_TOP_LAYERNORM = 2, DYF_TOP_LINATTN = 3, DYF_TOP_ATTENTION = 4, DYF_TOP_LINEAR = 5,
    DYF_TOP_LEARNED_SINU = 6, DYF_TOP_DROPOUT = 7, DYF_TOP_GELU = 8, DYF_TOP_ADD = 9, DYF_TOP_CAT = 10, DYF_TOP_UP2_NEAREST = 11,
    DYF_TOP_NORM_ACT = 12, DYF_TOP_UP2_BILINEAR = 13, DYF_TOP_RESIZE = 14, DYF_TOP_CONVT = 15, DYF_TOP_ATTENTION_STREAM = 16
} dyf_train_op_kind;
#define DYF_TOP_WS 1
#define DYF_TOP_BIAS 2
#define DYF_TOP_PRE 4
#define DYF_TOP_FILM 8
#define DYF_TOP_SAME 16
#define DYF_TOP_RUNNING 32
#define DYF_TOP_MASK 64
#define DYF_TOP_LEAKY 128
#define DYF_TOP_RELU 256
#define DYF_TOP_NEAREST 512
#define DYF_TOP_GRAD_IN 1024
#define DYF_TOP_ACT_GELU 2048
#define DYF_TOP_RESIDUAL 4096
#define DYF_TOP_SAMPLE 8192
typedef struct dyf_train_op {
    int32_t op, nb, h, w, c, c2, k, stride, pad, groups, flags;
    float p;
} dyf_train_op;
dyf_status dyf_op_train_f32(dyf_engine* engine, const dyf_train_op* desc, const float* const* inputs_dev, const float* const* params_host,
                            const float* dout_dev, float* y_dev, float* const* dinputs_dev, float* const* dparams_host, void* stream);

typedef enum dyf_sample_op_kind {
    DYF_SOP_GN_ACT = 0, DYF_SOP_LAYERNORM_C = 1, DYF_SOP_HEAD = 2, DYF_SOP_UP2_NEAREST = 3, DYF_SOP_DROP16 = 4, DYF_SOP_STEM_CONV = 5,
    DYF_SOP_GROUPNORM_F32 = 6, DYF_SOP_UP2_BILINEAR = 7, DYF_SOP_UP2_EPILOGUE = 8, DYF_SOP_READOUT = 9, DYF_SOP_READOUT_TABLES = 10,
    DYF_SOP_STEM = 11, DYF_SOP_STEM16 = 12, DYF_SOP_RNG_BEGIN = 13, DYF_SOP_RNG_CLONE = 14, DYF_SOP_TIME_MLP = 15, DYF_SOP_FILM = 16,
    DYF_SOP_COLD_UPDATE = 17, DYF_SOP_NOISY_CONDITION = 18
} dyf_sample_op_kind;
#define DYF_SOP_NO_STATS 1
#define DYF_SOP_NO_TABLES 2
#define DYF_SOP_FOLD_RNG 4
#define DYF_SOP_COUNTERS_ONLY 8
typedef struct dyf_sample_op {
    int32_t op, nb, h, w, c, c2, k, pad, groups, act, flags;
    int32_t film_stride, film_div, part_slots;
    int32_t nsrc, ch[4];
    int32_t drop_mode;
    float drop_p;
    int32_t drop_site;
    uint32_t drop_row_offset, drop_forward;
    int32_t oh, ow, nearest, src_rows, iw_store;
    float tau;
} dyf_sample_op;
typedef struct dyf_sample_tensors {
    const void* x[4];
    const uint16_t* residual;
    const float* film_a;
    const float* film_c;
    const float* part;
    const uint8_t* mask;
    void* y;
    const int16_t* col_map;
    void* y2;
    void* y3;
} dyf_sample_tensors;
dyf_status dyf_op_sample16(dyf_engine* engine, const dyf_sample_op* desc, const dyf_sample_tensors* t, const float* const* params_host,
                           void* stream);

dyf_status dyf_debug_read_block_output(dyf_engine* engine, int32_t net, int32_t layer, int32_t nb, float* out_dev,
                                       void* stream);

dyf_status dyf_debug_gn_fuse(dyf_engine* engine, uint32_t timeout_ticks, int32_t force_timeout);

void dyf_debug_form_log(int32_t enable);
int32_t dyf_debug_form_log_read(char* buf, int32_t cap);

void dyf_debug_set_form(const char* key, const char* value);
int32_t dyf_debug_forms(char* buf, int32_t cap);

#ifdef __cplusplus
}
#endif
#endif
```

Measured before the change: 8609 fields/s.

## Write stem16 once per distinct row and optionally use 8-channel pitch

The fused stem16 upsample kernel now writes only the src_rows distinct input rows (pair_once) instead of every batch row. The enc0 stem conv kernel reads each distinct row and emits multiple output copies (COPIES=2) with their own FiLM coefficients. An optional 8-channel pixel pitch halves stem buffer traffic; the constant-one channel is synthesized in-kernel as an extra K-step with a repacked weight fragment. This cuts the stem buffer's write and read bandwidth, at the cost of more template variants and extra per-copy epilogue work.

After: 8749 fields/s (median of 6 runs). +1.6%, better.

```diff
diff --git a/dyffusion_amd/_lib.py b/dyffusion_amd/_lib.py
--- a/dyffusion_amd/_lib.py
+++ b/dyffusion_amd/_lib.py
@@ -122,7 +122,7 @@
 SAMPLE_OPS = {"gn_act": 0, "layernorm_c": 1, "head": 2, "up2_nearest": 3, "drop16": 4, "stem_conv": 5, "groupnorm_f32": 6, "up2_bilinear": 7,
               "up2_epilogue": 8, "readout": 9, "readout_tables": 10, "stem": 11, "stem16": 12, "rng_begin": 13, "rng_clone": 14, "time_mlp": 15,
               "film": 16, "cold_update": 17, "noisy_condition": 18}
-SOP_NO_STATS, SOP_NO_TABLES, SOP_FOLD_RNG, SOP_COUNTERS_ONLY = 1, 2, 4, 8
+SOP_NO_STATS, SOP_NO_TABLES, SOP_FOLD_RNG, SOP_COUNTERS_ONLY, SOP_PAIR_ONCE, SOP_STEM_PITCH8 = 1, 2, 4, 8, 16, 32
 RNG_STATE_WORDS = 8
 ACTS = {"none": 0, "relu": 1, "leaky": 2, "silu": 3, "gelu": 4}
 
diff --git a/dyffusion_amd/csrc/conv.h b/dyffusion_amd/csrc/conv.h
--- a/dyffusion_amd/csrc/conv.h
+++ b/dyffusion_amd/csrc/conv.h
@@ -18,6 +18,7 @@
     int c0, c1;
     int pix_pitch0;
     int n, h, w;
+    int src0_rows;
     int ho, wo;
     int kh, kw, stride, pad;
     int cout;
@@ -63,6 +64,7 @@
     const el16_t* halo = nullptr;
     HaloOrder halo_order = HaloOrder::None;
     const el16_t* frag64 = nullptr;
+    const el16_t* enc0_p8 = nullptr;
 };
 
 hipError_t conv_init();
@@ -121,6 +123,7 @@
 hipError_t conv_enc0_stem_init();
 hipError_t launch_conv_enc0_stem(const ConvArgs& a, const el16_t* wfrag, hipStream_t stream);
 void pack_enc0_stem_frag(const el16_t* wpk, int cout, el16_t* out);
+void pack_enc0_stem_frag8(const el16_t* wpk, int cout, int cin, el16_t* out);
 bool conv_igemm2_supported(const ConvArgs& a);
 hipError_t conv_igemm2_init();
 hipError_t launch_conv_igemm2(const ConvArgs& a, hipStream_t stream);
diff --git a/dyffusion_amd/csrc/conv_dispatch.hip b/dyffusion_amd/csrc/conv_dispatch.hip
--- a/dyffusion_amd/csrc/conv_dispatch.hip
+++ b/dyffusion_amd/csrc/conv_dispatch.hip
@@ -35,7 +35,8 @@
 }
 
 const el16_t* enc0_stem_admits(const ConvArgs& a, const ConvW& w) {
-    return a.pix_pitch0 == 16 && conv_enc0_stem_supported(a) ? halo_of(w, HaloOrder::Enc0Stem) : nullptr;
+    if (!conv_enc0_stem_supported(a) || !halo_of(w, HaloOrder::Enc0Stem)) return nullptr;
+    return a.pix_pitch0 == 8 ? w.enc0_p8 : w.halo;
 }
 
 const el16_t* halo_s2_admits(const ConvArgs& a, const ConvW& w) {
@@ -161,7 +162,9 @@
 
 ConvChoice conv_choose_form(const ConvArgs& a, const ConvW& w, int path, ConvWant want) {
     const bool mfma = path == 1 && conv_mfma_supported(a);
-    return want == ConvWant::GnFused ? choose_gn_fused(a, w, mfma) : choose_plain(a, w, mfma, want == ConvWant::Stats);
+    const ConvChoice c = want == ConvWant::GnFused ? choose_gn_fused(a, w, mfma) : choose_plain(a, w, mfma, want == ConvWant::Stats);
+    if (((a.src0_rows > 0 && a.src0_rows != a.n) || a.pix_pitch0 == 8) && c.form != ConvForm::Enc0Stem) return {ConvForm::Invalid, nullptr, 0, 0};
+    return c;
 }
 
 bool conv_plain3x3_takes_halo5(const ConvArgs& a, const ConvW& w) {
diff --git a/dyffusion_amd/csrc/conv_enc0_stem.hip b/dyffusion_amd/csrc/conv_enc0_stem.hip
--- a/dyffusion_amd/csrc/conv_enc0_stem.hip
+++ b/dyffusion_amd/csrc/conv_enc0_stem.hip
@@ -5,39 +5,53 @@
 
 namespace {
 constexpr int E0_KSTEPS = 16;
+constexpr int e0_xsteps(bool p8) { return p8 ? 8 : 16; }
+constexpr int e0_wsteps(bool p8) { return p8 ? 9 : 16; }
 constexpr int E0_WAVES = 8, E0_THREADS = E0_WAVES * 64;
-constexpr int e0_lds_bytes(int nt) { return E0_KSTEPS * nt * 1024 + E0_WAVES * 2 * nt * 32 * 4 + E0_WAVES * 32 * (nt * 64 + 16); }
-}
-
-template <int NT>
+constexpr int E0_MAX_COPIES = 2;
+constexpr int e0_lds_bytes(int nt, int copies, bool p8) { return e0_wsteps(p8) * nt * 1024 + copies * E0_WAVES * 2 * nt * 32 * 4 + E0_WAVES * 32 * (nt * 64 + 16); }
+}
+
+template <int NT, int COPIES, bool P8>
 __global__ __launch_bounds__(512) void conv_enc0_stem_kernel(ConvArgs a, const el16_t* __restrict__ wfrag, int tiles, int tiles_per_wg) {
 #if defined(__gfx950__)
     extern __shared__ __attribute__((aligned(16))) unsigned char e0_smem[];
+    constexpr int XS = e0_xsteps(P8), WS = e0_wsteps(P8);
     uint4* wl = (uint4*)e0_smem;
     const int tid = threadIdx.x, lane = tid & 63, wave = __builtin_amdgcn_readfirstlane(tid >> 6), l31 = lane & 31, hi = lane >> 5;
-    for (int i = tid; i < E0_KSTEPS * NT * 64; i += E0_THREADS) wl[i] = ((const uint4*)wfrag)[i];
+    for (int i = tid; i < WS * NT * 64; i += E0_THREADS) wl[i] = ((const uint4*)wfrag)[i];
     __syncthreads();
-    float* coefl = (float*)(e0_smem + E0_KSTEPS * NT * 1024) + wave * (2 * NT * 32);
-    int coef_row = -1;
+    float* coefl_w = (float*)(e0_smem + WS * NT * 1024) + wave * (COPIES * 2 * NT * 32);
+    int coef_row[COPIES];
+#pragma unroll
+    for (int j = 0; j < COPIES; ++j) coef_row[j] = -1;
     constexpr int OROW = NT * 64 + 16;
-    unsigned char* ostage = e0_smem + E0_KSTEPS * NT * 1024 + E0_WAVES * 2 * NT * 32 * 4 + wave * (32 * OROW);
+    unsigned char* ostage = e0_smem + WS * NT * 1024 + COPIES * E0_WAVES * 2 * NT * 32 * 4 + wave * (32 * OROW);
     const int segs = a.wo >> 5;
     const int plane = a.ho * a.wo;
     const int t0 = blockIdx.x * tiles_per_wg, t1 = min(t0 + tiles_per_wg, tiles);
     const int cout = NT * 32;
 
-    auto load = [&](int t, uint4 (&xf)[E0_KSTEPS]) {
+    auto load = [&](int t, uint4 (&xf)[XS]) {
         const int row = t / segs, seg = t - row * segs;
         const int n = row / a.ho, oy = row - n * a.ho;
-        const el16_t* p = a.src0 + ((size_t)(n * a.h + 2 * oy) * a.w + 2 * (seg * 32 + l31)) * 16 + 8 * hi;
-#pragma unroll
-        for (int kh = 0; kh < 4; ++kh)
-#pragma unroll
-            for (int kw = 0; kw < 4; ++kw) xf[kh * 4 + kw] = *(const uint4*)(p + ((size_t)kh * a.w + kw) * 16);
+        if constexpr (P8) {
+            const el16_t* p = a.src0 + ((size_t)(n * a.h + 2 * oy) * a.w + 2 * (seg * 32 + l31) + hi) * 8;
+#pragma unroll
+            for (int kh = 0; kh < 4; ++kh)
+#pragma unroll
+                for (int kp = 0; kp < 2; ++kp) xf[kh * 2 + kp] = *(const uint4*)(p + ((size_t)kh * a.w + 2 * kp) * 8);
+        } else {
+            const el16_t* p = a.src0 + ((size_t)(n * a.h + 2 * oy) * a.w + 2 * (seg * 32 + l31)) * 16 + 8 * hi;
+#pragma unroll
+            for (int kh = 0; kh < 4; ++kh)
+#pragma unroll
+                for (int kw = 0; kw < 4; ++kw) xf[kh * 4 + kw] = *(const uint4*)(p + ((size_t)kh * a.w + kw) * 16);
+        }
         __builtin_amdgcn_sched_barrier(0);
     };
 
-    auto tile = [&](int t, const uint4 (&xf)[E0_KSTEPS], auto act_c, auto mode_c) {
+    auto tile = [&](int td, const uint4 (&xf)[XS], auto act_c, auto mode_c) {
         constexpr int ACT = decltype(act_c)::value, MODE = decltype(mode_c)::value;
         f32x16 acc[NT];
 #pragma unroll
@@ -45,22 +59,42 @@
 #pragma unroll
             for (int r = 0; r < 16; ++r) acc[nt][r] = 0.0f;
 #pragma unroll
-        for (int s = 0; s < E0_KSTEPS; ++s) {
+        for (int s = 0; s < WS; ++s) {
             int wlane = lane;
             asm volatile("" : "+v"(wlane));
-            const el16x8_t xb = __builtin_bit_cast(el16x8_t, xf[s]);
+            uint4 xs;
+            if constexpr (P8) {
+                if (s < XS) {
+                    xs = xf[s];
+                } else {
+                    const int row = td / segs, seg = td - row * segs;
+                    const int oy = row % a.ho, ox = seg * 32 + l31;
+                    const int py = 2 * oy + 2 * hi, px = 2 * ox;
+                    const bool r0 = py >= 1 && py <= a.h - 2, r1 = py + 1 <= a.h - 2;
+                    const float c0 = px >= 1 ? 1.0f : 0.0f, c3 = px + 3 <= a.w - 2 ? 1.0f : 0.0f;
+                    const uint32_t w01 = pack_el16x2(c0, 1.0f), w23 = pack_el16x2(1.0f, c3);
+                    xs = make_uint4(r0 ? w01 : 0u, r0 ? w23 : 0u, r1 ? w01 : 0u, r1 ? w23 : 0u);
+                }
+            } else {
+                xs = xf[s];
+            }
+            const el16x8_t xb = __builtin_bit_cast(el16x8_t, xs);
 #pragma unroll
             for (int nt = 0; nt < NT; ++nt)
                 acc[nt] = DYF_MFMA_32x32x16(__builtin_bit_cast(el16x8_t, wl[(s * NT + nt) * 64 + wlane]), xb, acc[nt], 0, 0, 0);
         }
+#pragma unroll
+        for (int j = 0; j < COPIES; ++j) {
+        const int t = td + j * tiles;
+        float* coefl = coefl_w + j * (2 * NT * 32);
         const int m = t * 32 + l31;
         const int n_img = m / plane;
         const uint32_t ob = (uint32_t)m * (uint32_t)cout;
         const RngKey key = drop_row_key(a.drop, n_img);
         const uint32_t row0 = (uint32_t)n_img * (uint32_t)(plane * cout);
         const int crow = __builtin_amdgcn_readfirstlane(a.coef_div > 1 ? n_img / a.coef_div : n_img);
-        if (crow != coef_row) {
-            coef_row = crow;
+        if (crow != coef_row[j]) {
+            coef_row[j] = crow;
             const float ps = drop_prescale<ACT, MODE>(a.drop);
             if (lane < NT * 8) {
                 float4 ca = *(const float4*)(a.coef_a + (size_t)crow * a.coef_stride + lane * 4);
@@ -104,10 +138,11 @@
             const uint4 ov = *(const uint4*)(ostage + px * OROW + within);
             *(uint4*)((unsigned char*)tbase + off) = ov;
         }
+        }
     };
 
     auto run = [&](auto act_c, auto mode_c) {
-        uint4 xa[E0_KSTEPS], xb[E0_KSTEPS];
+        uint4 xa[XS], xb[XS];
         int t = t0 + wave;
         if (t >= t1) return;
         load(t, xa);
@@ -139,32 +174,73 @@
                     out[(((size_t)s * nt_n + nt) * 64 + lane) * 8 + j] = wpk[(size_t)(32 * nt + (lane & 31)) * 256 + 16 * s + 8 * (lane >> 5) + j];
 }
 
+void pack_enc0_stem_frag8(const el16_t* wpk, int cout, int cin, el16_t* out) {
+    const int nt_n = cout / 32;
+    for (int s = 0; s < 9; ++s)
+        for (int nt = 0; nt < nt_n; ++nt)
+            for (int lane = 0; lane < 64; ++lane)
+                for (int j = 0; j < 8; ++j) {
+                    const size_t co = (size_t)(32 * nt + (lane & 31)), hi = (size_t)(lane >> 5);
+                    el16_t v{};
+                    if (s == 8) v = wpk[co * 256 + (8 * hi + j) * 16 + cin];
+                    else if (j < cin) v = wpk[co * 256 + ((s >> 1) * 4 + 2 * (s & 1) + hi) * 16 + j];
+                    out[(((size_t)s * nt_n + nt) * 64 + lane) * 8 + j] = v;
+                }
+}
+
+static int e0_copies(const ConvArgs& a) {
+    if (a.src0_rows <= 0 || a.src0_rows == a.n) return 1;
+    return a.n % a.src0_rows == 0 ? a.n / a.src0_rows : 0;
+}
+
 bool conv_enc0_stem_supported(const ConvArgs& a) {
     const bool on = dyf_form_int("DYF_ENC0_STEM", 1) != 0;
-    if (!on || a.pix_pitch0 != 16 || a.c0 != 64 || a.c1 != 0 || a.kh != 4 || a.kw != 1 || a.stride != 2 || a.pad != 0) return false;
+    if (!on || (a.pix_pitch0 != 16 && a.pix_pitch0 != 8) || a.c0 != 64 || a.c1 != 0 || a.kh != 4 || a.kw != 1 || a.stride != 2 || a.pad != 0) return false;
     if (a.up2x || a.residual || a.out_f32 || !a.out_el16 || (a.cout != 64 && a.cout != 128)) return false;
     if (a.wo % 32 != 0 || (a.ho * (a.wo / 32)) % 16 != 0 || a.h != 2 * a.ho + 2 || a.w != 2 * a.wo + 2) return false;
-    const long long nsel = a.n_sel > 0 ? a.n_sel : a.n;
+    const int copies = e0_copies(a);
+    if (copies < 1 || copies > E0_MAX_COPIES) return false;
+    const long long nsel = (a.n_sel > 0 ? a.n_sel : a.n) / copies;
     if (nsel * a.ho * (a.wo / 32) < 4096) return false;
     return (size_t)a.n * a.ho * a.wo * a.cout < 0xFFFFFFF0ull;
 }
 
+namespace {
+template <int NT, int COPIES, bool P8>
+hipError_t e0_set_lds() {
+    return hipFuncSetAttribute((const void*)conv_enc0_stem_kernel<NT, COPIES, P8>, hipFuncAttributeMaxDynamicSharedMemorySize, e0_lds_bytes(NT, COPIES, P8));
+}
+template <int NT, int COPIES, bool P8>
+void e0_launch(const ConvArgs& a, const el16_t* wfrag, int nwg, int tiles, int per, hipStream_t stream) {
+    hipLaunchKernelGGL((conv_enc0_stem_kernel<NT, COPIES, P8>), dim3(nwg), dim3(E0_THREADS), e0_lds_bytes(NT, COPIES, P8), stream, a, wfrag, tiles, per);
+}
+template <int NT>
+void e0_launch_nt(const ConvArgs& a, const el16_t* wfrag, int copies, int nwg, int tiles, int per, hipStream_t stream) {
+    const bool p8 = a.pix_pitch0 == 8;
+    if (copies == 1 && !p8) e0_launch<NT, 1, false>(a, wfrag, nwg, tiles, per, stream);
+    else if (copies == 1) e0_launch<NT, 1, true>(a, wfrag, nwg, tiles, per, stream);
+    else if (!p8) e0_launch<NT, 2, false>(a, wfrag, nwg, tiles, per, stream);
+    else e0_launch<NT, 2, true>(a, wfrag, nwg, tiles, per, stream);
+}
+}
+
 hipError_t conv_enc0_stem_init() {
-    hipError_t e = hipFuncSetAttribute((const void*)conv_enc0_stem_kernel<4>, hipFuncAttributeMaxDynamicSharedMemorySize, e0_lds_bytes(4));
-    if (e == hipSuccess) e = hipFuncSetAttribute((const void*)conv_enc0_stem_kernel<2>, hipFuncAttributeMaxDynamicSharedMemorySize, e0_lds_bytes(2));
-    return e;
+    for (hipError_t e : {e0_set_lds<4, 1, false>(), e0_set_lds<2, 1, false>(), e0_set_lds<4, 2, false>(), e0_set_lds<2, 2, false>(),
+                         e0_set_lds<4, 1, true>(), e0_set_lds<2, 1, true>(), e0_set_lds<4, 2, true>(), e0_set_lds<2, 2, true>()})
+        if (e != hipSuccess) return e;
+    return hipSuccess;
 }
 
 hipError_t launch_conv_enc0_stem(const ConvArgs& a, const el16_t* wfrag, hipStream_t stream) {
-    const int tiles = a.n * a.ho * (a.wo / 32);
+    const int copies = e0_copies(a);
+    if (copies < 1 || copies > E0_MAX_COPIES) return hipErrorInvalidValue;
+    const int tiles = (a.n / copies) * a.ho * (a.wo / 32);
     int nwg = std::min(256, (tiles + 15) / 16);
     int per = (tiles + nwg - 1) / nwg;
     per = (per + 15) / 16 * 16;
     nwg = (tiles + per - 1) / per;
     dyf_form_note("conv_enc0_stem_kernel", a.n);
-    if (a.cout == 128)
-        hipLaunchKernelGGL(conv_enc0_stem_kernel<4>, dim3(nwg), dim3(E0_THREADS), e0_lds_bytes(4), stream, a, wfrag, tiles, per);
-    else
-        hipLaunchKernelGGL(conv_enc0_stem_kernel<2>, dim3(nwg), dim3(E0_THREADS), e0_lds_bytes(2), stream, a, wfrag, tiles, per);
+    if (a.cout == 128) e0_launch_nt<4>(a, wfrag, copies, nwg, tiles, per, stream);
+    else e0_launch_nt<2>(a, wfrag, copies, nwg, tiles, per, stream);
     return hipGetLastError();
 }
diff --git a/dyffusion_amd/csrc/engine.hip b/dyffusion_amd/csrc/engine.hip
--- a/dyffusion_amd/csrc/engine.hip
+++ b/dyffusion_amd/csrc/engine.hip
@@ -111,8 +111,8 @@
     return DYF_OK;
 }
 
-const ConvW* fused_enc0_args(const dyf_engine* e, const Net& n, ConvArgs& a) {
-    a.src0 = e->ws.stem16; a.c0 = 64; a.pix_pitch0 = 16;
+const ConvW* fused_enc0_args(const dyf_engine* e, const Net& n, ConvArgs& a, int pitch = 16) {
+    a.src0 = e->ws.stem16; a.c0 = 64; a.pix_pitch0 = pitch;
     a.h = n.uh + 2; a.w = n.uw + 2;
     a.kh = 4; a.kw = 1; a.stride = 2; a.pad = 0;
     return &n.enc0_fused_w;
@@ -164,8 +164,25 @@
     if (rng_in_stem) {
         sa.rng_state = e->rng_state; sa.rng_row_keys = e->row_keys; sa.rng_rows = nb; sa.rng_rows_per_fwd = o.src_rows > 0 ? o.src_rows : nb;
     }
+    bool pair_once = false;
+    int stem_pitch = 16;
+    if (fused_stem && !n.blk[0].gn) {
+        const int want_pitch = dyf_form_int("DYF_STEM_PITCH", 16) == 8 && n.cin_total <= 8 && n.enc0_fused_w.enc0_p8 ? 8 : 16;
+        const int want_rows = o.src_rows > 0 && o.src_rows < nb && dyf_form_int("DYF_STEM_PAIR_ONCE", 1) != 0 ? o.src_rows : 0;
+        if (want_pitch == 8 || want_rows > 0) {
+            ConvArgs a0 = block_conv_args(e, n, n.blk[0], nb);
+            const ConvW* w0 = fused_enc0_args(e, n, a0, want_pitch);
+            a0.src0_rows = want_rows; a0.wpk = w0->wpk; a0.out_el16 = ws.enc[0];
+            if (conv_choose_form(a0, *w0, conv_path(e, a0), ConvWant::Plain).form == ConvForm::Enc0Stem) {
+                stem_pitch = want_pitch;
+                pair_once = want_rows > 0;
+            }
+        }
+    }
     if (fused_stem) {
         sa.out = ws.stem16;
+        sa.out_pitch = ws.stem16_pitch = stem_pitch;
+        sa.distinct_only = pair_once ? 1 : 0;
         HIP_TRY(e, launch_stem16(sa, st));
     } else {
         sa.out = ws.stem;
@@ -177,7 +194,8 @@
         ConvArgs a = block_conv_args(e, n, b, nb);
         a.src0 = x; a.c0 = b.cin; a.src1 = nullptr; a.c1 = 0;
         const ConvW* w = &b.wpk;
-        if (i == 0 && fused_stem) w = fused_enc0_args(e, n, a);
+        if (i == 0 && fused_stem) w = fused_enc0_args(e, n, a, stem_pitch);
+        if (i == 0 && pair_once) a.src0_rows = o.src_rows;
         if (!b.gn) {
             a.coef_a = o.coef_a + b.film_off; a.coef_c = o.coef_c + b.film_off; a.coef_stride = o.coef_stride;
             a.coef_div = o.coef_div;
@@ -676,7 +694,7 @@
                             }
                         fw[((size_t)co * 16 + t) * 16 + c] = f32_to_el16((float)v);
                     }
-            { dyf_status _s = upload_conv_weights(e, &n.enc0_fused_w, fw, b.cout, 4, 64, true); if (_s != DYF_OK) return _s; }
+            { dyf_status _s = upload_conv_weights(e, &n.enc0_fused_w, fw, b.cout, 4, 64, true, n.cin_total); if (_s != DYF_OK) return _s; }
             n.stem_fused = true;
         }
         if (b.transposed && b.k == 3) {
@@ -1567,7 +1585,11 @@
     a.src0 = b.transposed ? e->ws.up : (layer == 0 ? e->ws.stem : e->ws.enc[layer - 1]);
     a.c0 = b.cin;
     const ConvW* w = &b.wpk;
-    if (layer == 0 && n.stem_fused && e->cfg.enable_mfma && e->fuse_stem && n.cfg.input_dropout == 0.0f) w = fused_enc0_args(e, n, a);
+    if (layer == 0 && n.stem_fused && e->cfg.enable_mfma && e->fuse_stem && n.cfg.input_dropout == 0.0f) {
+        w = fused_enc0_args(e, n, a, e->ws.stem16_pitch);
+        a.out_el16 = e->ws.enc[0];
+        if (a.pix_pitch0 != 16 && conv_choose_form(a, *w, conv_path(e, a), ConvWant::Plain).form != ConvForm::Enc0Stem) w = fused_enc0_args(e, n, a);
+    }
     if (b.transposed && layer > 6) {
         ConvArgs f = a;
         const UBlock& skipb = n.blk[11 - layer];
@@ -2043,7 +2065,7 @@
     if (!t.y) return bad("null output");
     if (d.k || d.pad || d.groups || d.act || d.film_stride || d.film_div || d.part_slots || t.residual || t.film_a || t.film_c || t.part)
         return bad("k / pad / groups / act / FiLM rows / residual / part belong to the kernels between the convs");
-    const int allowed = readout ? DYF_SOP_NO_TABLES : stem16 ? DYF_SOP_FOLD_RNG : clone ? DYF_SOP_COUNTERS_ONLY : 0;
+    const int allowed = readout ? DYF_SOP_NO_TABLES : stem16 ? (DYF_SOP_FOLD_RNG | DYF_SOP_PAIR_ONCE | DYF_SOP_STEM_PITCH8) : clone ? DYF_SOP_COUNTERS_ONLY : 0;
     if (d.flags & ~allowed) return bad("a flag the op does not take");
     const bool fold = stem16 && (d.flags & DYF_SOP_FOLD_RNG);
     if (!stem && (d.drop_mode != 0 || t.mask || d.drop_p != 0.0f || d.drop_site != 0)) return bad("the op has no dropout");
@@ -2082,6 +2104,8 @@
         for (int i = 0; i < 4; ++i)
             if ((i < d.nsrc) != (t.x[i] != nullptr)) return bad("STEM: sources and their channel counts go together");
         if (d.src_rows > d.nb) return bad("STEM: src_rows above nb");
+        if ((d.flags & DYF_SOP_STEM_PITCH8) && d.c > 8) return unsup("STEM16: the 8-channel stem takes at most 8 channels");
+        if ((d.flags & DYF_SOP_PAIR_ONCE) && d.src_rows < 1) return bad("STEM16: DYF_SOP_PAIR_ONCE writes the src_rows distinct rows");
         if (stem ? (d.c2 < 1 || d.c > DYF_MAX_IN_CH) : (d.c2 != 0 || d.c > 15)) return unsup("STEM: c2 = dim and c <= 32 (STEM); c <= 15 and no c2 (STEM16)");
         if ((long long)d.nb * (d.oh + 2) * (d.ow + 2) * std::max(d.c2, 16) >= 0x7F000000ll || hw * d.c * d.nb >= 0x7F000000ll)
             return unsup("tensor too large for the kernels' 32-bit indices");
@@ -2172,6 +2196,8 @@
             a.nsrc = d.nsrc; a.cin = d.c; a.n = d.nb; a.src_rows = d.src_rows; a.h = d.h; a.w = d.w; a.uh = d.oh; a.uw = d.ow;
             a.resample = (d.oh != d.h || d.ow != d.w) ? 1 : 0;
             a.nearest = d.nearest; a.dim = d.c2; a.out = (el16_t*)t.y;
+            a.distinct_only = (d.flags & DYF_SOP_PAIR_ONCE) ? 1 : 0;
+            a.out_pitch = (d.flags & DYF_SOP_STEM_PITCH8) ? 8 : 16;
             if (stem) {
                 rs = upf(&a.wgt, params_host[0], (size_t)d.c2 * d.c);
                 if (rs == DYF_OK) rs = upf(&a.bias, params_host[1], (size_t)d.c2);
diff --git a/dyffusion_amd/csrc/engine_internal.h b/dyffusion_amd/csrc/engine_internal.h
--- a/dyffusion_amd/csrc/engine_internal.h
+++ b/dyffusion_amd/csrc/engine_internal.h
@@ -75,6 +75,7 @@
 struct Workspace {
     el16_t* stem = nullptr;
     el16_t* stem16 = nullptr;
+    int stem16_pitch = 16;
     el16_t* enc[6] = {};
     float* enc5_raw = nullptr;
     el16_t* up = nullptr;
@@ -257,7 +258,7 @@
 }
 
 inline dyf_status upload_conv_weights(dyf_engine* e, ConvW* out, const std::vector<el16_t>& pk, int cout, int taps, int cin,
-                                      bool enc0_stem = false) {
+                                      bool enc0_stem = false, int enc0_stem_cin = 0) {
     *out = ConvW{};
     auto up = [&](const el16_t** dst, const std::vector<el16_t>& host) {
         el16_t* p = nullptr;
@@ -275,6 +276,12 @@
     }
     if (enc0_stem && (cout == 64 || cout == 128)) {
         pf.assign(pk.size(), el16_t{});
+        if (enc0_stem_cin >= 1 && enc0_stem_cin <= 8) {
+            pf.assign((size_t)9 * cout * 16, el16_t{});
+            pack_enc0_stem_frag8(pk.data(), cout, enc0_stem_cin, pf.data());
+            if ((st = up(&out->enc0_p8, pf)) != DYF_OK) return st;
+            pf.assign(pk.size(), el16_t{});
+        }
         pack_enc0_stem_frag(pk.data(), cout, pf.data());
         out->halo_order = HaloOrder::Enc0Stem;
     } else if (taps == 16 && cout % 128 == 0) {
diff --git a/dyffusion_amd/csrc/kernels.h b/dyffusion_amd/csrc/kernels.h
--- a/dyffusion_amd/csrc/kernels.h
+++ b/dyffusion_amd/csrc/kernels.h
@@ -40,6 +40,8 @@
     int nsrc, cin;
     int n, h, w;
     int src_rows;
+    int out_pitch;
+    int distinct_only;
     int uh, uw;
     int resample;
     int nearest;
@@ -54,6 +56,7 @@
 };
 hipError_t launch_stem(const StemArgs& a, hipStream_t s);
 hipError_t launch_stem16(const StemArgs& a, hipStream_t s);
+inline __host__ __device__ int stem16_out_rows(const StemArgs& a) { return a.distinct_only && a.src_rows > 0 ? a.src_rows : a.n; }
 
 struct Up2xArgs {
     const el16_t* src0;
diff --git a/dyffusion_amd/csrc/kernels.hip b/dyffusion_amd/csrc/kernels.hip
--- a/dyffusion_amd/csrc/kernels.hip
+++ b/dyffusion_amd/csrc/kernels.hip
@@ -182,7 +182,7 @@
     stem_rng_begin(a);
     const long long idx = (long long)blockIdx.x * 256 + threadIdx.x;
     const int ph = a.uh + 2, pw = a.uw + 2;
-    const long long total = (long long)a.n * ph * pw;
+    const long long total = (long long)stem16_out_rows(a) * ph * pw;
     if (idx >= total) return;
     const int n = (int)(idx / ((long long)ph * pw));
     const int rem = (int)(idx % ((long long)ph * pw));
@@ -210,13 +210,17 @@
                 const float top = p[o00] * (1.0f - lx) + p[o01] * lx;
                 const float bot = p[o10] * (1.0f - lx) + p[o11] * lx;
                 val = top * (1.0f - ly) + bot * ly;
-            } else if (k == a.cin) {
+            } else if (k == a.cin && a.out_pitch != 8) {
                 val = 1.0f;
             }
             v[k] = val;
         }
 #pragma unroll
         for (int k = 0; k < 8; ++k) w[k] = pack_el16x2(v[2 * k], v[2 * k + 1]);
+    }
+    if (a.out_pitch == 8) {
+        *(uint4*)(a.out + (size_t)idx * 8) = make_uint4(w[0], w[1], w[2], w[3]);
+        return;
     }
     uint4* o = (uint4*)(a.out + (size_t)idx * 16);
     o[0] = make_uint4(w[0], w[1], w[2], w[3]);
@@ -280,7 +284,8 @@
         }
     }
     __syncthreads();
-    uint4* oblk = (uint4*)(a.out + (((size_t)n * ph + py0) * pw) * 16);
+    const bool p8 = a.out_pitch == 8;
+    uint4* oblk = (uint4*)(a.out + (((size_t)n * ph + py0) * pw) * (p8 ? 8 : 16));
     if (a.cin <= 8 && (a.uw & 63) == 0) {
         const int lane = threadIdx.x & 63, wave = threadIdx.x >> 6;
         unsigned char* stg = (unsigned char*)(ytab + ST_ROWS) + wave * 2048;
@@ -288,7 +293,8 @@
         const uint4 half1 = a.cin == 8 ? make_uint4(pack_el16x2(1.0f, 0.0f), 0, 0, 0) : zero4;
         for (int i = threadIdx.x; i < (py1 - py0) * 4; i += 512) {
             const int rr = i >> 2, q = i & 3;
-            oblk[(size_t)rr * 2 * pw + (q < 2 ? q : 2 * pw - 4 + q)] = zero4;
+            if (!p8) oblk[(size_t)rr * 2 * pw + (q < 2 ? q : 2 * pw - 4 + q)] = zero4;
+            else if (q < 2) oblk[(size_t)rr * pw + (q ? pw - 1 : 0)] = zero4;
         }
         const int total_in = (py1 - py0) * a.uw;
         int r = 0, j = threadIdx.x;
@@ -319,11 +325,17 @@
                         const float top = t00[e] * (1.0f - lx) + t01[e] * lx;
                         const float bot = t10[e] * (1.0f - lx) + t11[e] * lx;
                         float val = top * (1.0f - ly) + bot * ly;
-                        if (k >= a.cin) val = k == a.cin ? 1.0f : 0.0f;
+                        if (k >= a.cin) val = k == a.cin && !p8 ? 1.0f : 0.0f;
                         v[k] = val;
                     }
                 }
                 w = make_uint4(pack_el16x2(v[0], v[1]), pack_el16x2(v[2], v[3]), pack_el16x2(v[4], v[5]), pack_el16x2(v[6], v[7]));
+            }
+            if (p8) {
+                oblk[(size_t)r * pw + 1 + j] = w;
+                j += 512;
+                while (j >= a.uw) { j -= a.uw; ++r; }
+                continue;
             }
             *(uint4*)(stg + lane * 32) = w;
             *(uint4*)(stg + lane * 32 + 16) = yt.w ? half1 : zero4;
@@ -335,10 +347,11 @@
         }
         return;
     }
-    const int total = (py1 - py0) * 2 * pw;
+    const int per_row = p8 ? pw : 2 * pw, total = (py1 - py0) * per_row;
     int r = 0, j = threadIdx.x;
+    while (j >= per_row) { j -= per_row; ++r; }
     for (int i = threadIdx.x; i < total; i += 512) {
-        const int px = j >> 1, half = j & 1;
+        const int px = p8 ? j : j >> 1, half = p8 ? 0 : j & 1;
         const int4 xt = xtab[px], yt = ytab[r];
         uint32_t w[4] = {0, 0, 0, 0};
         if (xt.w && yt.w) {
@@ -365,7 +378,7 @@
                     const float top = t00[e] * (1.0f - lx) + t01[e] * lx;
                     const float bot = t10[e] * (1.0f - lx) + t11[e] * lx;
                     float val = top * (1.0f - ly) + bot * ly;
-                    if (k >= a.cin) val = k == a.cin ? 1.0f : 0.0f;
+                    if (k >= a.cin) val = k == a.cin && !p8 ? 1.0f : 0.0f;
                     v[4 * q2 + e] = val;
                 }
             }
@@ -374,7 +387,7 @@
         }
         oblk[i] = make_uint4(w[0], w[1], w[2], w[3]);
         j += 512;
-        if (j >= 2 * pw) { j -= 2 * pw; ++r; }
+        while (j >= per_row) { j -= per_row; ++r; }
     }
 }
 
@@ -382,18 +395,20 @@
     const int cp = (a.cin + 3) / 4 * 4;
     const size_t lds = (size_t)(ST_ROWS + 2) * a.w * cp * sizeof(float) + (size_t)(a.uw + 2 + ST_ROWS) * 16 + 8 * 2048;
     const bool rows = dyf_form_int("DYF_STEM16_ROWS", 1) != 0;
+    const int rows_out = stem16_out_rows(a), pitch = a.out_pitch == 8 ? 8 : 16;
+    if ((a.out_pitch != 0 && a.out_pitch != 8 && a.out_pitch != 16) || (pitch == 8 && a.cin > 8)) return hipErrorInvalidValue;
     if (rows && lds <= 48 * 1024 && cp <= 16 && a.h <= a.uh && 2 * (a.uw + 2) >= 512) {
         const int nblk = (a.uh + 2 + ST_ROWS - 1) / ST_ROWS;
-        const dim3 grid((unsigned)(a.n * nblk)), block(512);
+        const dim3 grid((unsigned)(rows_out * nblk)), block(512);
         dyf_form_note("stem16_rows_kernel", a.n);
-        KernelProf kp("stem16_rows_kernel", s, (double)(a.src_rows ? a.src_rows : a.n) * a.h * a.w * a.cin * 4.0 + (double)a.n * (a.uh + 2) * (a.uw + 2) * 16 * 2.0);
+        KernelProf kp("stem16_rows_kernel", s, (double)(a.src_rows ? a.src_rows : a.n) * a.h * a.w * a.cin * 4.0 + (double)rows_out * (a.uh + 2) * (a.uw + 2) * pitch * 2.0);
         if (cp == 4) hipLaunchKernelGGL(stem16_rows_kernel<4>, grid, block, lds, s, a, nblk);
         else if (cp == 8) hipLaunchKernelGGL(stem16_rows_kernel<8>, grid, block, lds, s, a, nblk);
         else if (cp == 12) hipLaunchKernelGGL(stem16_rows_kernel<12>, grid, block, lds, s, a, nblk);
         else hipLaunchKernelGGL(stem16_rows_kernel<16>, grid, block, lds, s, a, nblk);
         return hipGetLastError();
     }
-    const long long total = (long long)a.n * (a.uh + 2) * (a.uw + 2);
+    const long long total = (long long)rows_out * (a.uh + 2) * (a.uw + 2);
     dyf_form_note("stem16_kernel", a.n);
     hipLaunchKernelGGL(stem16_kernel, dim3((unsigned)((total + 255) / 256)), dim3(256), 0, s, a);
     return hipGetLastError();
diff --git a/dyffusion_amd/engine.py b/dyffusion_amd/engine.py
--- a/dyffusion_amd/engine.py
+++ b/dyffusion_amd/engine.py
@@ -938,15 +938,16 @@
 
     def _op_sample_net(self, op, xs, params, *, mask=None, p=0.0, rng_site=None, rng_row_offset=0, rng_forward=0, out_hw=None, in_hw=None,
                        nearest=False, src_rows=0, nb=None, col_map=None, tables=True, fold_rng=False, counters_only=False, dst=None, tau=0.0,
-                       blocks=(), copy=False, iw_store=None):
+                       blocks=(), copy=False, iw_store=None, pair_once=False, pitch=16):
         given = {k for k, v, d in (("mask", mask, None), ("p", p, 0.0), ("rng_site", rng_site, None), ("rng_row_offset", rng_row_offset, 0),
                                    ("rng_forward", rng_forward, 0), ("out_hw", out_hw, None), ("in_hw", in_hw, None), ("nearest", nearest, False),
                                    ("src_rows", src_rows, 0), ("nb", nb, None), ("col_map", col_map, None), ("tables", tables, True),
                                    ("fold_rng", fold_rng, False), ("counters_only", counters_only, False), ("dst", dst, None), ("tau", tau, 0.0),
-                                   ("blocks", blocks, ()), ("copy", copy, False), ("iw_store", iw_store, None)) if v is not d and v != d}
+                                   ("blocks", blocks, ()), ("copy", copy, False), ("iw_store", iw_store, None),
+                                   ("pair_once", pair_once, False), ("pitch", pitch, 16)) if v is not d and v != d}
         takes = {"readout": {"out_hw", "nearest", "col_map", "tables"}, "readout_tables": {"in_hw", "out_hw", "nearest", "col_map", "iw_store"},
                  "stem": {"out_hw", "nearest", "src_rows", "nb", "mask", "p", "rng_site", "rng_row_offset", "rng_forward"},
-                 "stem16": {"out_hw", "nearest", "src_rows", "nb", "fold_rng", "rng_row_offset", "rng_forward"},
+                 "stem16": {"out_hw", "nearest", "src_rows", "nb", "fold_rng", "rng_row_offset", "rng_forward", "pair_once", "pitch"},
                  "rng_begin": {"nb", "src_rows", "rng_row_offset", "rng_forward"}, "rng_clone": {"dst", "rng_row_offset", "counters_only"},
                  "time_mlp": set(), "film": {"blocks", "nb"}, "cold_update": {"copy"}, "noisy_condition": {"tau", "rng_row_offset"}}[op]
         if given - takes:
@@ -1009,9 +1010,14 @@
                 elif rng_site is not None:
                     desc.drop_mode, desc.drop_site, desc.drop_row_offset, desc.drop_forward = 1, int(rng_site), int(rng_row_offset), int(rng_forward)
             else:
-                outs = [torch.empty((desc.nb, desc.oh + 2, desc.ow + 2, 16), dtype=dt, device=dev)]
+                if pair_once and desc.src_rows < 1:
+                    raise ValueError("stem16: pair_once writes the src_rows distinct rows: give src_rows")
+                if pitch not in (8, 16) or (pitch == 8 and desc.c > 8):
+                    raise ValueError("stem16: pitch is 16, or 8 for at most 8 channels")
+                outs = [torch.empty((desc.src_rows if pair_once else desc.nb, desc.oh + 2, desc.ow + 2, int(pitch)), dtype=dt, device=dev)]
+                desc.flags = (L.SOP_PAIR_ONCE if pair_once else 0) | (L.SOP_STEM_PITCH8 if pitch == 8 else 0)
                 if fold_rng:
-                    desc.flags, desc.drop_row_offset, desc.drop_forward = L.SOP_FOLD_RNG, int(rng_row_offset), int(rng_forward)
+                    desc.flags, desc.drop_row_offset, desc.drop_forward = desc.flags | L.SOP_FOLD_RNG, int(rng_row_offset), int(rng_forward)
                     outs += [i32(desc.nb, 2), i32(L.RNG_STATE_WORDS)]
         elif op == "rng_begin":
             desc.nb, desc.src_rows, desc.drop_row_offset, desc.drop_forward = int(nb), int(src_rows), int(rng_row_offset), int(rng_forward)
diff --git a/include/dyffusion_hip_testing.h b/include/dyffusion_hip_testing.h
--- a/include/dyffusion_hip_testing.h
+++ b/include/dyffusion_hip_testing.h
@@ -100,6 +100,8 @@
 #define DYF_SOP_NO_TABLES 2
 #define DYF_SOP_FOLD_RNG 4
 #define DYF_SOP_COUNTERS_ONLY 8
+#define DYF_SOP_PAIR_ONCE 16
+#define DYF_SOP_STEM_PITCH8 32
 typedef struct dyf_sample_op {
     int32_t op, nb, h, w, c, c2, k, pad, groups, act, flags;
     int32_t film_stride, film_div, part_slots;
```
